# Veason-silverbullet/DIGAT

Hardware: AMD Instinct MI355X
Metric: MIND dev impressions scored/sec (AUC match not run) (higher is better)
Workload: dtype f32; 1 GPU; MIND-small default: --graph_encoder=DIGAT neighbors=3 hops=2 (N=10, U=67), d=400, graph_depth=3, fp32 dev inference; projection=auto -> fp16x3, N=10, U=67, d=400, graph_depth=3, news_num=65238, parallelism=dp1 (row shards, no data-path collective), ranks_in_process_group=1

## Files before the change

digat_amd/_lib.py:

```python
from __future__ import annotations

import ctypes as C
import os
from typing import Optional

import torch

_HERE = os.path.dirname(os.path.abspath(__file__))
LIB_PATH = os.environ.get("DIGAT_HIP_LIB") or os.path.join(_HERE, "lib", "libdigat_hip.so")
DIGAT_MAX_DEPTH = 16
DIGAT_MAX_NODES = 128
GEMM_BF16X6, GEMM_F16X3 = 0, 1
GEMM_F16F8C = 2
PARAMS_GEMM_F16X3 = 64
PARAMS_BD_TILED = 128
PARAMS_PQ_FP8 = 256
PARAMS_SIDE_STREAM_OFF, PARAMS_SIDE_STREAM_ON = 512, 1024
PARAMS_NO_LIVE_ROWS = 2048
PARAMS_PROJ_F16F8C = 4096

_f = C.c_void_p


class LayerParams(C.Structure):
    _fields_ = [(k, _f) for k in ("W", "bW", "F1", "F2", "F3", "b3", "a", "wsplit", "f3_wsplit")]


class MsaParams(C.Structure):
    _fields_ = ([(k, C.c_int32) for k in ("word_embedding_dim", "head_num", "head_dim", "attention_dim")]
                + [(k, C.c_void_p) for k in ("word_embedding", "W_Q", "b_Q", "W_K", "W_V", "b_V", "A1", "b1", "a2",
                                             "qkv_wsplit", "a1_wsplit")])


class CnnParams(C.Structure):
    _fields_ = ([(k, C.c_int32) for k in ("word_embedding_dim", "kernel_num", "taps", "attention_dim")]
                + [(k, C.c_void_p) for k in ("word_embedding", "W", "b", "A1", "b1", "a2", "w_split", "a1_wsplit")])


class SplitJob(C.Structure):
    _fields_ = [("w0", C.c_void_p), ("w1", C.c_void_p), ("w2", C.c_void_p), ("rows", C.c_int32), ("cols", C.c_int32), ("layout", C.c_int32),
                ("reserved", C.c_int32), ("image", C.c_void_p)]


class GatherJob(C.Structure):
    _fields_ = [("src", C.c_void_p), ("dst", C.c_void_p), ("row_bytes", C.c_int64), ("rows", C.c_int64),
                ("idx", C.c_void_p), ("idx2", C.c_void_p), ("inner", C.c_int64)]


class Params(C.Structure):
    _fields_ = ([("d", C.c_int32), ("depth", C.c_int32), ("category_num", C.c_int32), ("flags", C.c_int32)]
                + [(k, _f) for k in ("topic_node_embedding", "cand_K", "cand_Q", "cand_bQ",
                                     "news_graph_W", "news_graph_b", "user_news_K", "user_news_Q",
                                     "user_news_bQ", "featureAffine_W", "featureAffine_b",
                                     "userAtt_K", "userAtt_Q", "userAtt_bQ")]
                + [("news", LayerParams * DIGAT_MAX_DEPTH), ("user", LayerParams * DIGAT_MAX_DEPTH)]
                + [(k, _f) for k in ("cand_fold_W", "cand_fold_b", "user_news_fold_W", "user_news_fold_b",
                                     "userAtt_fold_W", "userAtt_fold_b", "featureAffine_wsplit", "cand_fold_wsplit", "gate_wsplit")]
                + [("ctx_wsplit", _f * (DIGAT_MAX_DEPTH + 1)), ("range_flag", _f), ("featureAffine_fsplit", _f)])


class DigatHipError(RuntimeError):
    pass


_lib: Optional[C.CDLL] = None

_SIGNATURES = {
    "digat_version": (C.c_int, []),
    "digat_error_string": (C.c_char_p, [C.c_int]),
    "digat_linear_f32": (C.c_int, [_f, C.c_int64, _f, _f, _f, C.c_int64, C.c_int, C.c_int, C.c_int, _f]),
    "digat_xattn_workspace_bytes": (C.c_size_t, [C.c_int] * 3),
    "digat_xattn_fwd": (C.c_int, [_f] * 12 + [C.c_int] * 3 + [_f, C.c_size_t, _f]),
    "digat_xattn_fwd_mode": (C.c_int, [_f] * 11 + [C.c_int] * 4 + [_f, C.c_size_t, _f]),
    "digat_xattn_fwd_lowprec": (C.c_int, [_f] * 11 + [C.c_int, _f] + [C.c_int] * 4 + [_f, C.c_size_t, _f]),
    "digat_xattn_pairwise_fwd": (C.c_int, [_f] * 8 + [C.c_int] * 3 + [_f]),
    "digat_news_ctx_workspace_bytes": (C.c_size_t, [C.c_int] * 3),
    "digat_news_ctx_fwd": (C.c_int, [_f] * 9 + [C.c_int] * 3 + [_f, C.c_size_t, _f]),
    "digat_user_ctx_workspace_bytes": (C.c_size_t, [C.c_int] * 5),
    "digat_user_ctx_fwd": (C.c_int, [_f] * 14 + [C.c_int] * 5 + [_f, C.c_size_t, _f]),
    "digat_topic_pool_fwd": (C.c_int, [_f] * 4 + [C.c_int] * 5 + [_f]),
    "digat_encoder_workspace_bytes": (C.c_size_t, [C.c_int] * 6),
    "digat_encoder_fwd": (C.c_int, [C.POINTER(Params)] + [_f] * 10 + [C.c_int] * 3 + [_f, C.c_size_t, _f]),
    "digat_row_logits": (C.c_int, [_f] * 3 + [C.c_int] * 2 + [_f]),
    "digat_profile_pause": (C.c_int, [C.c_int]),
    "digat_set_train_precision": (C.c_int, [C.c_int]),
    "digat_gather_tables": (C.c_int, [C.POINTER(GatherJob), C.c_int, _f]),
    "digat_profile_live_row_fraction": (C.c_double, []),
    "digat_rank_metrics": (C.c_int, [_f] * 3 + [C.c_int] + [_f] * 4),
    "digat_format_rank_file": (C.c_int64, [_f, _f, C.c_int64, _f, C.c_int64]),
    "digat_gat_workspace_bytes": (C.c_size_t, [C.c_int] * 3),
    "digat_gat_fwd": (C.c_int, [_f] * 7 + [C.c_int] * 3 + [_f, C.c_size_t, _f]),
    "digat_gat_train_save_bytes": (C.c_size_t, [C.c_int] * 3),
    "digat_gat_train_workspace_bytes": (C.c_size_t, [C.c_int] * 3),
    "digat_gat_fwd_train": (C.c_int, [_f] * 7 + [C.c_float, C.c_uint32] + [C.c_int] * 3 + [_f, C.c_size_t, _f, C.c_size_t, _f]),
    "digat_gat_bwd": (C.c_int, [_f] * 7 + [C.c_float, _f, C.c_size_t] + [_f] * 5 + [C.c_int] * 3 + [_f, C.c_size_t, _f]),
    "digat_sag_cos_topk_workspace_bytes": (C.c_size_t, [C.c_int64, C.c_int64, C.c_int]),
    "digat_sag_cos_topk": (C.c_int, [_f, _f, C.c_int64, _f, _f, C.c_int64, C.c_int, C.c_int, _f, _f, _f, C.c_size_t, _f]),
    "digat_sag_news_graph": (C.c_int, [_f, _f, _f, C.c_int64, C.c_int, C.c_int, C.c_int, C.c_float] + [_f] * 5),
    "digat_msa_split_bytes": (C.c_size_t, [C.c_int] * 3),
    "digat_split_msa_weights": (C.c_int, [_f] * 3 + [C.c_int] * 2 + [_f, _f]),
    "digat_msa_workspace_bytes": (C.c_size_t, [C.c_int] * 6),
    "digat_msa_fwd": (C.c_int, [C.POINTER(MsaParams), _f, _f, _f, C.c_int, C.c_int, _f, C.c_size_t, _f]),
    "digat_msa_train_save_bytes": (C.c_size_t, [C.c_int] * 6),
    "digat_msa_train_workspace_bytes": (C.c_size_t, [C.c_int] * 6),
    "digat_msa_fwd_train": (C.c_int, [C.POINTER(MsaParams), _f, _f, _f, C.c_float, C.c_uint32, C.c_int, C.c_int, _f, C.c_size_t, _f,
                                      C.c_size_t, _f]),
    "digat_msa_bwd": (C.c_int, [C.POINTER(MsaParams), _f, _f, _f, C.c_float, _f, C.c_size_t, _f, C.c_int64] + [_f] * 8
                      + [C.c_int, C.c_int, _f, C.c_size_t, _f]),
    "digat_msa_row_grad_ld": (C.c_int64, [C.c_int] * 3),
    "digat_cnn_split_bytes": (C.c_size_t, [C.c_int] * 3),
    "digat_split_cnn_weights": (C.c_int, [_f] + [C.c_int] * 3 + [_f, _f]),
    "digat_cnn_merge_group3": (C.c_int, [_f] * 6 + [C.c_int] * 2 + [_f] * 3),
    "digat_cnn_workspace_bytes": (C.c_size_t, [C.c_int] * 6),
    "digat_cnn_fwd": (C.c_int, [C.POINTER(CnnParams), _f, _f, _f, C.c_int, C.c_int, _f, C.c_size_t, _f]),
    "digat_cnn_train_save_bytes": (C.c_size_t, [C.c_int] * 6),
    "digat_cnn_train_workspace_bytes": (C.c_size_t, [C.c_int] * 6),
    "digat_cnn_fwd_train": (C.c_int, [C.POINTER(CnnParams), _f, _f, _f, C.c_float, C.c_uint32, C.c_int, C.c_int, _f, C.c_size_t, _f,
                                      C.c_size_t, _f]),
    "digat_cnn_bwd": (C.c_int, [C.POINTER(CnnParams), _f, _f, _f, C.c_float, C.c_uint32, _f, C.c_size_t, _f, C.c_int64] + [_f] * 5
                      + [C.c_int, C.c_int, _f, C.c_size_t, _f]),
    "digat_embedding_bwd_workspace_bytes": (C.c_size_t, [C.c_int64, C.c_int]),
    "digat_embedding_bwd": (C.c_int, [_f, C.c_int64, _f, _f, C.c_int64, C.c_int, _f, _f, C.c_size_t, _f]),
    "digat_embedding_bwd_unsorted_workspace_bytes": (C.c_size_t, [C.c_int64, C.c_int, C.c_int64]),
    "digat_embedding_bwd_unsorted": (C.c_int, [_f, _f, C.c_int64, C.c_int64, _f, _f, C.c_int64, C.c_int64, C.c_int, C.c_int64, _f, _f, C.c_size_t,
                                               _f]),
    "digat_encoder_grouped_workspace_bytes": (C.c_size_t, [C.c_int] * 6),
    "digat_encoder_fwd_grouped": (C.c_int, [C.POINTER(Params)] + [_f] * 11 + [C.c_int] * 4 + [_f, C.c_size_t, _f]),
    "digat_encoder_fwd_grouped_cached": (C.c_int, [C.POINTER(Params)] + [_f] * 14 + [C.c_int64] + [_f] * 2 + [C.c_int] * 4 + [_f, C.c_size_t, _f]),
    "digat_news_context_queries": (C.c_int, [C.POINTER(Params), _f, _f, C.c_int, _f]),
    "digat_user_project0": (C.c_int, [C.POINTER(Params), _f, _f, C.c_int, _f]),
    "digat_news_project0": (C.c_int, [C.POINTER(Params), _f, _f, C.c_int, C.c_int, _f]),
    "digat_split_weights_bytes": (C.c_size_t, [C.c_int, C.c_int]),
    "digat_split_weights_bytes_format": (C.c_size_t, [C.c_int, C.c_int, C.c_int]),
    "digat_forget_split_image": (C.c_int, [_f]),
    "digat_split_proj_weights": (C.c_int, [_f, _f, _f, C.c_int, _f, C.c_int, _f]),
    "digat_split_weights": (C.c_int, [_f, C.c_int, C.c_int, _f, C.c_int, _f]),
    "digat_linear_f32x3": (C.c_int, [_f, C.c_int64, _f, _f, _f, C.c_int64, C.c_int, C.c_int, C.c_int, _f, C.c_int, _f]),
    "digat_fold_workspace_bytes": (C.c_size_t, [C.c_int]),
    "digat_fold_attention": (C.c_int, [_f] * 5 + [C.c_int, _f, C.c_size_t, _f]),
    "digat_linear_bwd_input": (C.c_int, [_f, C.c_int64, _f, _f, C.c_int64, C.c_int, C.c_int, C.c_int, C.c_int, _f]),
    "digat_linear_bwd_input_x3": (C.c_int, [_f, C.c_int64, _f, _f, C.c_int64, C.c_int, C.c_int, C.c_int, C.c_int, _f, _f]),
    "digat_linear_bwd_weight_workspace": (C.c_size_t, [C.c_int] * 3),
    "digat_linear_bwd_weight": (C.c_int, [_f, C.c_int64, _f, C.c_int64, _f, _f, C.c_int, C.c_int, C.c_int, C.c_int, _f,
                                          C.c_size_t, _f]),
    "digat_colsum": (C.c_int, [_f, C.c_int64, _f, C.c_int, C.c_int, C.c_int, _f]),
    "digat_dropout_fwd": (C.c_int, [_f, _f, _f, C.c_int64, C.c_float, C.c_uint32, _f]),
    "digat_dropout_bwd": (C.c_int, [_f, _f, _f, C.c_int64, C.c_float, _f]),
    "digat_gate_fwd": (C.c_int, [_f, _f, C.c_int64, _f, _f, C.c_int, C.c_int, _f]),
    "digat_gate_bwd": (C.c_int, [_f, _f, _f, C.c_int64, _f, _f, _f, _f, C.c_int, C.c_int, _f]),
    "digat_relu_res_fwd": (C.c_int, [_f, _f, _f, C.c_int64, _f]),
    "digat_relu_mask": (C.c_int, [_f, _f, _f, C.c_int64, _f]),
    "digat_attn_pool_fwd": (C.c_int, [_f, C.c_int64, _f, _f, _f, _f, C.c_int, C.c_int, C.c_int, _f]),
    "digat_attn_pool_bwd": (C.c_int, [_f, C.c_int64, _f, _f, _f, _f, _f, C.c_int64, _f, C.c_int, C.c_int, C.c_int,
                                      C.c_int, _f]),
    "digat_topic_pool_fwd_train": (C.c_int, [_f] * 5 + [C.c_int] * 5 + [_f]),
    "digat_topic_pool_bwd": (C.c_int, [_f] * 7 + [C.c_int] * 5 + [_f]),
    "digat_xattn_project": (C.c_int, [_f] * 9 + [C.c_int] * 3 + [_f]),
    "digat_xattn_project_x3": (C.c_int, [_f] * 9 + [C.c_int] * 3 + [_f, _f]),
    "digat_xattn_pairwise_fwd_train": (C.c_int, [_f] * 11 + [C.c_float, C.c_uint32, C.c_int, C.c_int, C.c_int, _f]),
    "digat_xattn_pairwise_bwd_workspace": (C.c_size_t, [C.c_int] * 3),
    "digat_xattn_pairwise_bwd": (C.c_int, [_f] * 11 + [C.c_float] + [_f] * 4 + [C.c_int] * 4 + [_f, C.c_size_t, _f]),
    "digat_sum_nodes": (C.c_int, [_f, _f, C.c_int, C.c_int, C.c_int, _f]),
    "digat_xattn_train_save_bytes": (C.c_size_t, [C.c_int] * 3),
    "digat_xattn_train_workspace_bytes": (C.c_size_t, [C.c_int] * 3),
    "digat_xattn_fwd_train": (C.c_int, [_f] * 11 + [C.c_float, C.c_uint32, C.c_float, C.c_uint32] + [C.c_int] * 3 + [_f, C.c_size_t, _f, C.c_size_t, _f, C.c_int,
                                        _f]),
    "digat_xattn_bwd": (C.c_int, [_f] * 10 + [C.c_float, C.c_float, _f, C.c_size_t] + [_f] * 9 + [C.c_int] * 3 + [_f, C.c_size_t, _f, C.c_int, _f]),
    "digat_opt_chunk": (C.c_int, []),
    "digat_clip_adam_step": (C.c_int, [_f, _f, _f, C.c_int, _f] + [C.c_float] * 5 + [C.c_int, _f]),
    "digat_row_logits_bwd": (C.c_int, [_f] * 5 + [C.c_int, C.c_int, _f]),
    "digat_click_loss": (C.c_int, [_f, C.c_int, C.c_int, _f, _f, _f]),
    "digat_split_job_bytes": (C.c_size_t, [C.c_int] * 4),
# ... 150 lines not shown
```

digat_amd/csrc/digat_context.inc:

```

struct PoolArgs {
    const float* feat; long ld_b;
    const float* kq; const uint8_t* mask; const float* addend; float* out;
    int B, n, d; float sqrt_d;
    float* alpha_out;
    long ld_out;
    float* node0; long ld_node0;
};

__global__ void __launch_bounds__(256) attn_pool_kernel(const PoolArgs g) {
    __shared__ float sc[DIGAT_MAX_NODES];
    const int b = blockIdx.x, tid = threadIdx.x, lane = tid & 63, wave = tid >> 6;
    const int d4 = g.d >> 2, n = g.n;
    const float4* F4 = reinterpret_cast<const float4*>(g.feat + (long)b * g.ld_b);
    const float4* K4 = reinterpret_cast<const float4*>(g.kq + (long)b * g.d);
    for (int j = wave; j < n; j += 4) {
        float part = 0.f;
        for (int c4 = lane; c4 < d4; c4 += 64) {
            const float4 x = F4[(long)j * d4 + c4], k = K4[c4];
            part = fmaf(x.w, k.w, fmaf(x.z, k.z, fmaf(x.y, k.y, fmaf(x.x, k.x, part))));
        }
        part = wave_sum(part);
        if (lane == 0) sc[j] = g.mask[(long)b * n + j] == 0 ? -1e9f : part / g.sqrt_d;
    }
    __syncthreads();
    if (wave == 0) {
        const float v0 = lane < n ? sc[lane] : -INFINITY;
        const float v1 = lane + 64 < n ? sc[lane + 64] : -INFINITY;
        const float m = wave_max(fmaxf(v0, v1));
        const float e0 = lane < n ? expf(v0 - m) : 0.f;
        const float e1 = lane + 64 < n ? expf(v1 - m) : 0.f;
        const float s = wave_sum(e0 + e1);
        if (lane < n) sc[lane] = e0 / s;
        if (lane + 64 < n) sc[lane + 64] = e1 / s;
        if (g.alpha_out) {
            if (lane < n) g.alpha_out[(long)b * n + lane] = e0 / s;
            if (lane + 64 < n) g.alpha_out[(long)b * n + lane + 64] = e1 / s;
        }
    }
    __syncthreads();
    for (int c4 = tid; c4 < d4; c4 += 256) {
        float4 o = f4_zero();
        for (int j = 0; j < n; ++j) {
            const float al = sc[j];
            if (al == 0.f) continue;
            const float4 x = F4[(long)j * d4 + c4];
            o.x = fmaf(al, x.x, o.x); o.y = fmaf(al, x.y, o.y); o.z = fmaf(al, x.z, o.z); o.w = fmaf(al, x.w, o.w);
        }
        if (g.addend) o = f4_add(reinterpret_cast<const float4*>(g.addend + (long)b * g.d)[c4], o);
        reinterpret_cast<float4*>(g.out + (long)b * (g.ld_out ? g.ld_out : (long)g.d))[c4] = o;
        if (g.node0) reinterpret_cast<float4*>(g.node0 + (long)b * g.ld_node0)[c4] = F4[c4];
    }
}

template <int NPW, int U>
__global__ void __launch_bounds__(256) attn_pool_resident_kernel(const PoolArgs g) {
    __shared__ float sc[DIGAT_MAX_NODES];
    __shared__ float4 part[4][64 * U];
    const int b = blockIdx.x, tid = threadIdx.x, lane = tid & 63, wave = tid >> 6;
    const int d4 = g.d >> 2, n = g.n;
    const float4* F4 = reinterpret_cast<const float4*>(g.feat + (long)b * g.ld_b);
    const float4* K4 = reinterpret_cast<const float4*>(g.kq + (long)b * g.d);
    float4 x[NPW][U], k[U];
#pragma unroll
    for (int u = 0; u < U; ++u) {
        const int c4 = min(lane + 64 * u, d4 - 1);
        const float4 kv = K4[c4];
        k[u] = lane + 64 * u < d4 ? kv : f4_zero();
    }
    const unsigned long long mb0 = __ballot(lane < n && g.mask[(long)b * n + min(lane, n - 1)] != 0);
    const unsigned long long mb1 = __ballot(lane + 64 < n && g.mask[(long)b * n + min(lane + 64, n - 1)] != 0);
    const bool none = (mb0 | mb1) == 0ull;
#pragma unroll
    for (int t = 0; t < NPW; ++t) {
        const int j = min(wave + 4 * t, n - 1);
        const bool want = none || (((j < 64 ? mb0 : mb1) >> (j & 63)) & 1ull);
#pragma unroll
        for (int u = 0; u < U; ++u) x[t][u] = want ? F4[(long)j * d4 + min(lane + 64 * u, d4 - 1)] : f4_zero();
    }
#pragma unroll
    for (int t = 0; t < NPW; ++t) {
        const int j = wave + 4 * t;
        float p = 0.f;
#pragma unroll
        for (int u = 0; u < U; ++u) p = fmaf(x[t][u].w, k[u].w, fmaf(x[t][u].z, k[u].z, fmaf(x[t][u].y, k[u].y, fmaf(x[t][u].x, k[u].x, p))));
        p = wave_sum(p);
        if (lane == 0 && j < n) sc[j] = g.mask[(long)b * n + j] == 0 ? -1e9f : p / g.sqrt_d;
    }
    __syncthreads();
    {
        const float v0 = lane < n ? sc[lane] : -INFINITY;
        const float v1 = lane + 64 < n ? sc[lane + 64] : -INFINITY;
        const float m = wave_max(fmaxf(v0, v1));
        const float e0 = lane < n ? expf(v0 - m) : 0.f;
        const float e1 = lane + 64 < n ? expf(v1 - m) : 0.f;
        const float s = wave_sum(e0 + e1);
        const float a0 = e0 / s, a1 = e1 / s;
        if (wave == 0 && g.alpha_out) {
            if (lane < n) g.alpha_out[(long)b * n + lane] = a0;
            if (lane + 64 < n) g.alpha_out[(long)b * n + lane + 64] = a1;
        }
        float4 o[U];
#pragma unroll
        for (int u = 0; u < U; ++u) o[u] = f4_zero();
#pragma unroll
        for (int t = 0; t < NPW; ++t) {
            const int j = wave + 4 * t;
            const float al = j < n ? (j < 64 ? lane_bcast(a0, j & 63) : lane_bcast(a1, j & 63)) : 0.f;
            if (al != 0.f) {
#pragma unroll
                for (int u = 0; u < U; ++u) {
                    o[u].x = fmaf(al, x[t][u].x, o[u].x); o[u].y = fmaf(al, x[t][u].y, o[u].y);
                    o[u].z = fmaf(al, x[t][u].z, o[u].z); o[u].w = fmaf(al, x[t][u].w, o[u].w);
                }
            }
        }
#pragma unroll
        for (int u = 0; u < U; ++u) part[wave][lane + 64 * u] = o[u];
    }
    __syncthreads();
    for (int c4 = tid; c4 < d4; c4 += 256) {
        float4 o = f4_add(f4_add(part[0][c4], part[1][c4]), f4_add(part[2][c4], part[3][c4]));
        if (g.addend) o = f4_add(reinterpret_cast<const float4*>(g.addend + (long)b * g.d)[c4], o);
        reinterpret_cast<float4*>(g.out + (long)b * g.d)[c4] = o;
    }
}

static int launch_pool(const float* feat, long ld_b, const float* kq, const uint8_t* mask, const float* addend,
                       float* out, int B, int n, int d, hipStream_t st) {
    if (n > DIGAT_MAX_NODES || d % 4) return DIGAT_ERR_SHAPE;
    if (B == 0) return DIGAT_OK;
    PoolArgs g{feat, ld_b, kq, mask, addend, out, B, n, d, sqrtf((float)d), nullptr};
    ProfScope prof(DIGAT_KERNEL_POOL, (double)B * ((double)n * d * 4 + 2.0 * d * 4 + n), st);
    const int d4 = d / 4;
    if (d4 <= 128 && n <= 68) {
        if (d4 <= 64) {
            if (n <= 12) hipLaunchKernelGGL((attn_pool_resident_kernel<3, 1>), dim3(B), dim3(256), 0, st, g);
            else if (n <= 20) hipLaunchKernelGGL((attn_pool_resident_kernel<5, 1>), dim3(B), dim3(256), 0, st, g);
            else if (n <= 28) hipLaunchKernelGGL((attn_pool_resident_kernel<7, 1>), dim3(B), dim3(256), 0, st, g);
            else hipLaunchKernelGGL((attn_pool_resident_kernel<17, 1>), dim3(B), dim3(256), 0, st, g);
        } else {
            if (n <= 12) hipLaunchKernelGGL((attn_pool_resident_kernel<3, 2>), dim3(B), dim3(256), 0, st, g);
            else if (n <= 20) hipLaunchKernelGGL((attn_pool_resident_kernel<5, 2>), dim3(B), dim3(256), 0, st, g);
            else if (n <= 28) hipLaunchKernelGGL((attn_pool_resident_kernel<7, 2>), dim3(B), dim3(256), 0, st, g);
            else hipLaunchKernelGGL((attn_pool_resident_kernel<17, 2>), dim3(B), dim3(256), 0, st, g);
        }
        DIGAT_CHECK_LAUNCH();
        return DIGAT_OK;
    }
    hipLaunchKernelGGL(attn_pool_kernel, dim3(B), dim3(256), 0, st, g);
    DIGAT_CHECK_LAUNCH();
    return DIGAT_OK;
}

struct TopicArgs {
    const float* Xu; long ld_b; const float* kq; const int64_t* idx; float* out;
    int B, H, C1, d; float sqrt_d;
    float* alpha_out;
    const int* group;
    const uint8_t* live; int live_ld;
    const int* hlast;
};
constexpr int TOPIC_MAX_H = 256;
constexpr int TOPIC_MAX_CT = 4;

__global__ void __launch_bounds__(1024) topic_pool_kernel(const TopicArgs g) {
    extern __shared__ __attribute__((aligned(16))) unsigned char smem[];
    const int H = g.H, hs = H | 1;
    const int ct = (g.C1 + 15) >> 4;
    float* M = reinterpret_cast<float*>(smem);
    float* sa = M + ct * 16 * hs;
    int* sidx = reinterpret_cast<int*>(sa + H);
    const int b = blockIdx.x, tid = threadIdx.x, lane = tid & 63, wave = tid >> 6;
    const int nthreads = blockDim.x, nw = nthreads >> 6;
    const int d4 = g.d >> 2;
    const float* Xb = g.Xu + (long)(g.group ? g.group[b] : b) * g.ld_b;
    const float4* F4 = reinterpret_cast<const float4*>(Xb);
    const float4* K4 = reinterpret_cast<const float4*>(g.kq + (long)b * g.d);
    unsigned char* slive = reinterpret_cast<unsigned char*>(sidx + H);
    for (int t = tid; t < H; t += nthreads) {
        const long v = g.idx[(long)b * H + t];
        sidx[t] = (v >= 0 && v < g.C1) ? (int)v : -1;
        slive[t] = g.live ? g.live[(long)b * g.live_ld + t] : 1;
    }
    for (int i = tid; i < ct * 16 * hs; i += nthreads) M[i] = 0.f;
    __syncthreads();
    for (int t0 = wave; t0 < H; t0 += 4 * nw) {
        float part[4] = {0.f, 0.f, 0.f, 0.f};
        for (int c4 = lane; c4 < d4; c4 += 64) {
            const float4 k = K4[c4];
#pragma unroll
            for (int r = 0; r < 4; ++r) {
                const int t = t0 + r * nw;
                if (t < H && slive[t]) {
                    const float4 x = F4[(long)t * d4 + c4];
                    part[r] = fmaf(x.w, k.w, fmaf(x.z, k.z, fmaf(x.y, k.y, fmaf(x.x, k.x, part[r]))));
                }
            }
        }
#pragma unroll
        for (int r = 0; r < 4; ++r) {
            const int t = t0 + r * nw;
            const float s = wave_sum(part[r]);
            if (lane == 0 && t < H) sa[t] = s / g.sqrt_d;
        }
    }
    __syncthreads();
    for (int t = tid; t < H; t += nthreads) {
        const int s = sidx[t];
        float m = -INFINITY;
        for (int u = 0; u < H; ++u) if (sidx[u] == s) m = fmaxf(m, sa[u]);
        float den = 0.f;
        for (int u = 0; u < H; ++u) if (sidx[u] == s) den += expf(sa[u] - m);
        const float al = s >= 0 ? expf(sa[t] - m) / den : 0.f;
        if (s >= 0) M[s * hs + t] = al;
        if (g.alpha_out) g.alpha_out[(long)b * H + t] = al;
    }
    __syncthreads();

    const int lr = lane & 15, lq = lane >> 4;
    const int ch = wave * 64 + 4 * lr;
    const bool ch_ok = ch < g.d;
    const int nsteps = (H + 3) >> 2;
    auto load_x = [&](int step) -> float4 {
        const int j = step * 4 + lq;
        return (j < H && ch_ok && slive[j]) ? *reinterpret_cast<const float4*>(Xb + (long)j * g.d + ch) : f4_zero();
    };
    constexpr int PF = 4;
    v4f acc[TOPIC_MAX_CT][4];
#pragma unroll
    for (int it = 0; it < TOPIC_MAX_CT; ++it)
#pragma unroll
        for (int s = 0; s < 4; ++s) acc[it][s] = (v4f){0.f, 0.f, 0.f, 0.f};
    float4 xq[PF];
#pragma unroll
    for (int u = 0; u < PF; ++u) xq[u] = load_x(u);
    for (int step = 0; step < nsteps; step += PF) {
#pragma unroll
        for (int u = 0; u < PF; ++u) {
            const int st = step + u;
            if (st < nsteps) {
                const float4 xc = xq[u];
                xq[u] = load_x(st + PF);
                const int j = st * 4 + lq;
#pragma unroll
                for (int it = 0; it < TOPIC_MAX_CT; ++it) {
                    if (it < ct) {
                        const float av = j < H ? M[(it * 16 + lr) * hs + j] : 0.f;
                        acc[it][0] = __builtin_amdgcn_mfma_f32_16x16x4f32(av, xc.x, acc[it][0], 0, 0, 0);
                        acc[it][1] = __builtin_amdgcn_mfma_f32_16x16x4f32(av, xc.y, acc[it][1], 0, 0, 0);
                        acc[it][2] = __builtin_amdgcn_mfma_f32_16x16x4f32(av, xc.z, acc[it][2], 0, 0, 0);
                        acc[it][3] = __builtin_amdgcn_mfma_f32_16x16x4f32(av, xc.w, acc[it][3], 0, 0, 0);
                    }
                }
            }
        }
    }
    float* Ob = g.out + (long)b * g.C1 * g.d;
#pragma unroll
    for (int it = 0; it < TOPIC_MAX_CT; ++it) {
        if (it < ct) {
#pragma unroll
            for (int r = 0; r < 4; ++r) {
                const int c = it * 16 + 4 * lq + r;
                if (c < g.C1 && ch_ok)
                    *reinterpret_cast<float4*>(Ob + (long)c * g.d + ch) =
                        make_float4(acc[it][0][r], acc[it][1][r], acc[it][2][r], acc[it][3][r]);
            }
        }
    }
}


template <int TOPIC_RES_STEPS>
__global__ void __launch_bounds__(TOPIC_RES_STEPS > 13 ? 512 : 1024) topic_pool_resident_kernel(const TopicArgs g) {
    extern __shared__ __attribute__((aligned(16))) unsigned char smem[];
    const int H = g.H, hs = H | 1;
    const int ct = (g.C1 + 15) >> 4;
    const int tid = threadIdx.x, lane = tid & 63, wave = tid >> 6;
    const int nthreads = blockDim.x, nw = nthreads >> 6;
    float* M = reinterpret_cast<float*>(smem);
    float* part = M + ct * 16 * hs;
    float* sa = part + nw * 64;
    int* sidx = reinterpret_cast<int*>(sa + 64);
    int* slive = sidx + 64;
    int* cslot = slive + 64;
    int* scat = cslot + 64;
    const int b = blockIdx.x;
    const float* Xb = g.Xu + (long)(g.group ? g.group[b] : b) * g.ld_b;
    const int lr = lane & 15, lq = lane >> 4;
    const int ch = wave * 64 + 4 * lr;
    const bool ch_ok = ch < g.d;
    const int nsteps = (H + 3) >> 2;
    const int nl = (g.live && g.hlast) ? min(g.hlast[b], H) : H;

    float4 xq[TOPIC_RES_STEPS];
#pragma unroll
    for (int s = 0; s < TOPIC_RES_STEPS; ++s) {
        const int j = s * 4 + lq;
        const int jr = min(j, nl > 0 ? nl - 1 : 0);
        xq[s] = (s < nsteps && j < H && ch_ok) ? *reinterpret_cast<const float4*>(Xb + (long)jr * g.d + ch) : f4_zero();
    }
    const float4 k4 = ch_ok ? *reinterpret_cast<const float4*>(g.kq + (long)b * g.d + ch) : f4_zero();
    if (tid < 64) {
        long v = -1;
        if (tid < H) v = g.idx[(long)b * H + tid];
        const int cat = (v >= 0 && v < g.C1) ? (int)v : -1;
        sidx[tid] = cat;
        slive[tid] = (g.live && tid < H) ? (int)g.live[(long)b * g.live_ld + tid] : 1;
        unsigned long long present = 0ull;
        for (int c = 0; c < g.C1; ++c) present |= __ballot(cat == c) ? (1ull << c) : 0ull;
        const bool has = tid < g.C1 && ((present >> tid) & 1ull);
        const int slot = __popcll(present & ((1ull << tid) - 1ull));
        cslot[tid] = has ? slot : -1;
        if (has) scat[slot] = tid;
        if (tid == 0) scat[64] = __popcll(present);
    }
    for (int i = tid; i < ct * 16 * hs; i += nthreads) M[i] = 0.f;
    if (g.live) {
        __syncthreads();
#pragma unroll
        for (int s = 0; s < TOPIC_RES_STEPS; ++s) xq[s] = slive[min(s * 4 + lq, 63)] ? xq[s] : f4_zero();
    }

#pragma unroll
    for (int s = 0; s < TOPIC_RES_STEPS; ++s) {
        float p = fmaf(xq[s].w, k4.w, fmaf(xq[s].z, k4.z, fmaf(xq[s].y, k4.y, xq[s].x * k4.x)));
        p += dpp_mov<0xB1>(p); p += dpp_mov<0x4E>(p); p += dpp_mov<0x141>(p); p += dpp_mov<0x140>(p);
        if (lr == 0) part[wave * 64 + s * 4 + lq] = p;
    }
    __syncthreads();
    if (tid < 64) {
        float a = 0.f;
        for (int w = 0; w < nw; ++w) a += part[w * 64 + tid];
        sa[tid] = a / g.sqrt_d;
    }
    __syncthreads();
    {
        const int my = lane < H ? sidx[lane] : -2;
        const float v = lane < H ? sa[lane] : 0.f;
        const int nslots = scat[64];
        for (int sl = wave; sl < nslots; sl += nw) {
            const int c = scat[sl];
            const bool in = my == c;
            const float m = wave_max(in ? v : -INFINITY);
            const float e = in ? expf(v - m) : 0.f;
            const float den = wave_sum(e);
            if (in) {
                const float al = e / den;
                M[sl * hs + lane] = al;
                if (g.alpha_out) g.alpha_out[(long)b * H + lane] = al;
            }
        }
        if (wave == 0 && g.alpha_out && lane < H && my < 0) g.alpha_out[(long)b * H + lane] = 0.f;
    }
    __syncthreads();

    const int ct_eff = __builtin_amdgcn_readfirstlane((scat[64] + 15) >> 4);
    const int nslots_all = scat[64];
    float* Ob = g.out + (long)b * g.C1 * g.d;
    for (int it = 0; it < ct_eff; ++it) {
        v4f acc[4];
#pragma unroll
        for (int s = 0; s < 4; ++s) acc[s] = (v4f){0.f, 0.f, 0.f, 0.f};
#pragma unroll
        for (int s = 0; s < TOPIC_RES_STEPS; ++s) {
            if (s * 4 < nl) {
                const int j = s * 4 + lq;
                const float4 xc = xq[s];
                const float av = j < H ? M[(it * 16 + lr) * hs + j] : 0.f;
                acc[0] = __builtin_amdgcn_mfma_f32_16x16x4f32(av, xc.x, acc[0], 0, 0, 0);
                acc[1] = __builtin_amdgcn_mfma_f32_16x16x4f32(av, xc.y, acc[1], 0, 0, 0);
                acc[2] = __builtin_amdgcn_mfma_f32_16x16x4f32(av, xc.z, acc[2], 0, 0, 0);
                acc[3] = __builtin_amdgcn_mfma_f32_16x16x4f32(av, xc.w, acc[3], 0, 0, 0);
            }
        }
#pragma unroll
        for (int r = 0; r < 4; ++r) {
            const int sl = it * 16 + 4 * lq + r;
            if (sl < nslots_all && ch_ok)
                *reinterpret_cast<float4*>(Ob + (long)scat[sl] * g.d + ch) = make_float4(acc[0][r], acc[1][r], acc[2][r], acc[3][r]);
        }
    }
    for (int c = lq; c < g.C1; c += 4)
        if (cslot[c] < 0 && ch_ok) *reinterpret_cast<float4*>(Ob + (long)c * g.d + ch) = f4_zero();
}

static int launch_topic_args(TopicArgs g, hipStream_t st) {
    const int groups = (g.d + 63) / 64;
    const int ct = (g.C1 + 15) / 16;
    if (g.H > TOPIC_MAX_H || g.d % 4 || groups > 16 || ct > TOPIC_MAX_CT) return DIGAT_ERR_SHAPE;
    const size_t lds = ((size_t)ct * 16 * (g.H | 1) + 2 * (size_t)g.H) * 4 + align_up((size_t)g.H, 16);
    if (lds > 64 * 1024) {
        static int raised = 0;
        if (!raised) {
            if (hipFuncSetAttribute((const void*)topic_pool_kernel, hipFuncAttributeMaxDynamicSharedMemorySize,
                                    160 * 1024) != hipSuccess) return DIGAT_ERR_LAUNCH;
            raised = 1;
        }
    }
    if (g.H <= 64 && (g.H <= 52 || groups <= 8)) {
        const size_t ldsr = ((size_t)ct * 16 * (g.H | 1) + (size_t)groups * 64 + 192 + 64 + 68) * 4;
        if (g.H <= 52) hipLaunchKernelGGL(topic_pool_resident_kernel<13>, dim3(g.B), dim3(64 * groups), ldsr, st, g);
        else hipLaunchKernelGGL(topic_pool_resident_kernel<16>, dim3(g.B), dim3(64 * groups), ldsr, st, g);
    } else {
        hipLaunchKernelGGL(topic_pool_kernel, dim3(g.B), dim3(64 * groups), lds, st, g);
    }
    DIGAT_CHECK_LAUNCH();
    return DIGAT_OK;
}

static int launch_topic(const float* Xu, long ld_b, const float* kq, const int64_t* idx, float* out,
                        int B, int H, int C1, int d, hipStream_t st, const int* group = nullptr,
                        const uint8_t* live = nullptr, int live_ld = 0, const int* hlast = nullptr) {
    if (B == 0) return DIGAT_OK;
    TopicArgs g{Xu, ld_b, kq, idx, out, B, H, C1, d, sqrtf((float)d), nullptr, group, live, live_ld, hlast};
    ProfScope prof(DIGAT_KERNEL_TOPIC, (double)B * ((double)H * d * 4 + d * 4.0 + H * 8.0 + (double)C1 * d * 4), st);
    return launch_topic_args(g, st);
}
```

digat_amd/csrc/digat_gemm.inc:

```

#include "digat_gemm_plan.h"

template <int BM, int BN, int WAVES_M, int WAVES_N, int PF, int TAG>
__global__ void __launch_bounds__(256) gemm_f32_kernel(const GemmArgs g) {
    constexpr int BK4 = 8;
    constexpr int MT = BM / WAVES_M / 16;
    constexpr int NT = BN / WAVES_N / 16;
    static_assert(WAVES_M * WAVES_N == 4, "4 waves per workgroup");
    static_assert(BM % (WAVES_M * 16) == 0 && BN % (WAVES_N * 16) == 0, "wave tile");
    static_assert(BM % 8 == 0 && BN % 8 == 0, "xor swizzle needs 8-row groups");
    constexpr int A_PER_T = (BM * BK4 + 255) / 256;
    constexpr int B_PER_T = (BN * BK4 + 255) / 256;
    __shared__ float4 As[BK4 * BM];
    __shared__ float4 Bs[BK4 * BN];

    const int total = g.mtiles * g.ntiles;
    const int chunk = (total + 7) >> 3;
    const int tile = (int)(blockIdx.x & 7) * chunk + (int)(blockIdx.x >> 3);
    if (tile >= total) return;
    const int mtile = tile / g.ntiles, ntile = tile - mtile * g.ntiles;

    const int tid = threadIdx.x, lane = tid & 63, wave = tid >> 6;
    const int wm = wave / WAVES_N, wn = wave % WAVES_N;
    const int m0 = mtile * BM, n0 = ntile * BN;
// ... 43 lines not shown
        }
    };
    auto store_tiles = [&](const float4* ra, const float4* rb) {
#pragma unroll
        for (int u = 0; u < A_PER_T; ++u) {
            const int i = tid + u * 256;
            if (i < BM * BK4) {
                const int r = i / BK4, c4 = i % BK4;
                As[c4 * BM + (r ^ c4)] = ra[u];
            }
        }
#pragma unroll
        for (int u = 0; u < B_PER_T; ++u) {
            const int i = tid + u * 256;
            if (i < BN * BK4) {
                const int r = g.transW ? i % BN : i / BK4;
                const int c4 = g.transW ? i / BN : i % BK4;
                Bs[c4 * BN + (r ^ c4)] = rb[u];
            }
        }
    };

    v4f acc[MT][NT];
#pragma unroll
    for (int mt = 0; mt < MT; ++mt)
#pragma unroll
        for (int nt = 0; nt < NT; ++nt) acc[mt][nt] = (v4f){0.f, 0.f, 0.f, 0.f};

    auto compute_tile = [&]() {
#pragma unroll
        for (int kk = 0; kk < 2; ++kk) {
            const int k4 = kk * 4 + (lane >> 4);
            float4 af[MT], bf[NT];
#pragma unroll
            for (int mt = 0; mt < MT; ++mt) {
                const int r = wm * (MT * 16) + mt * 16 + (lane & 15);
                af[mt] = As[k4 * BM + (r ^ k4)];
            }
#pragma unroll
            for (int nt = 0; nt < NT; ++nt) {
                const int r = wn * (NT * 16) + nt * 16 + (lane & 15);
                bf[nt] = Bs[k4 * BN + (r ^ k4)];
            }
#pragma unroll
            for (int s = 0; s < 4; ++s)
#pragma unroll
                for (int mt = 0; mt < MT; ++mt)
#pragma unroll
                    for (int nt = 0; nt < NT; ++nt)
                        acc[mt][nt] = __builtin_amdgcn_mfma_f32_16x16x4f32(
                            f4_comp(af[mt], s), f4_comp(bf[nt], s), acc[mt][nt], 0, 0, 0);
        }
    };

    if (PF == 1) {
        load_tiles(0, ra0, rb0);
        store_tiles(ra0, rb0);
        __syncthreads();
        for (int kt = 0; kt < ktiles; ++kt) {
            const bool more = kt + 1 < ktiles;
            if (more) load_tiles(kt + 1, ra0, rb0);
            compute_tile();
            __syncthreads();
            if (more) {
                store_tiles(ra0, rb0);
                __syncthreads();
            }
        }
    } else {
        load_tiles(0, ra0, rb0);
        if (ktiles > 1) load_tiles(1, ra1, rb1);
        store_tiles(ra0, rb0);
        __syncthreads();
        for (int kt = 0; kt < ktiles; kt += 2) {
            if (kt + 2 < ktiles) load_tiles(kt + 2, ra0, rb0);
            compute_tile();
            __syncthreads();
            if (kt + 1 >= ktiles) break;
            store_tiles(ra1, rb1);
            __syncthreads();
            if (kt + 3 < ktiles) load_tiles(kt + 3, ra1, rb1);
            compute_tile();
            __syncthreads();
            if (kt + 2 < ktiles) {
                store_tiles(ra0, rb0);
                __syncthreads();
            }
        }
    }

#pragma unroll
    for (int mt = 0; mt < MT; ++mt) {
#pragma unroll
        for (int nt = 0; nt < NT; ++nt) {
            const int nn = nbase + wn * (NT * 16) + nt * 16 + (lane & 15);
            if (nn >= g.nseg) continue;
            const float* bp = g.bias[seg];
            float* yp = g.y[seg];
            const float bv = bp ? bp[nn] : 0.f;
            const float* radd = seg == g.radd_seg ? g.radd : nullptr;
#pragma unroll
            for (int r = 0; r < 4; ++r) {
                const int gm = m0 + wm * (MT * 16) + mt * 16 + (lane >> 4) * 4 + r;
                if (gm >= g.M) continue;
                float v = acc[mt][nt][r] + bv;
                if (radd) v = radd[(long)(gm / g.rows_per_b) * g.nseg + nn] + v;
                if (g.epi == EPI_RELU_RES) {
                    v = fmaxf(v, 0.f) + g.e0[(long)gm * g.lde0 + nn];
                } else if (g.epi == EPI_GATE) {
                    const float gate = 1.f / (1.f + expf(-v));
                    const float loc = g.e0[(long)gm * g.lde0 + nn];
                    const float glo = g.e1[(long)gm * g.lde1 + nn];
                    v = gate * loc + (1.f - gate) * glo;
                    if (g.e2) v = g.e2[(long)gm * g.lde2 + nn] + v;
                } else if (g.epi == EPI_ACCUM) {
                    v = yp[(long)gm * g.ldy + nn] + v;
                }
                yp[(long)gm * g.ldy + nn] = v;
            }
        }
    }
}

typedef __bf16 bf16x8 __attribute__((ext_vector_type(8)));

struct Split3f { float a, b, c; };
__device__ __forceinline__ Split3f split3f(float v) {
    Split3f o;
    o.a = __builtin_bit_cast(float, __builtin_bit_cast(unsigned, v) & 0xffff0000u);
    const float r1 = v - o.a;
    o.b = __builtin_bit_cast(float, __builtin_bit_cast(unsigned, r1) & 0xffff0000u);
    o.c = r1 - o.b;
    return o;
}
__device__ __forceinline__ unsigned pack_bf16_rne(float lo, float hi) {
    unsigned a = __builtin_bit_cast(unsigned, lo), b = __builtin_bit_cast(unsigned, hi);
    a += 0x7fffu + ((a >> 16) & 1u);
    b += 0x7fffu + ((b >> 16) & 1u);
    return (a >> 16) | (b & 0xffff0000u);
}
__device__ __forceinline__ unsigned pack_hi16(float lo, float hi) {
    return __builtin_amdgcn_perm(__builtin_bit_cast(unsigned, hi), __builtin_bit_cast(unsigned, lo), 0x07060302u);
}
constexpr float F16_WEIGHT_SCALE = 1024.f;
constexpr float F16_ACT_SCALE = 16.f;
typedef _Float16 half8 __attribute__((ext_vector_type(8)));
typedef __fp16 fp16x2 __attribute__((ext_vector_type(2)));
__device__ __forceinline__ unsigned pack_half_rtz(float lo, float hi) { return __builtin_bit_cast(unsigned, __builtin_amdgcn_cvt_pkrtz(lo, hi)); }
__device__ __forceinline__ unsigned half_bits_rtz(float v) { return pack_half_rtz(v, 0.f) & 0xffffu; }
__device__ __forceinline__ float half_bits_to_float(unsigned bits) {
    const fp16x2 h = __builtin_bit_cast(fp16x2, bits);
    return (float)h[0];
}
struct Split3 { unsigned short a, b, c; };
__device__ __forceinline__ Split3 split3(float v) {
    const Split3f f = split3f(v);
    Split3 o;
    o.a = (unsigned short)(__builtin_bit_cast(unsigned, f.a) >> 16);
    o.b = (unsigned short)(__builtin_bit_cast(unsigned, f.b) >> 16);
    o.c = (unsigned short)(__builtin_bit_cast(unsigned, f.c) >> 16);
    return o;
}

constexpr int WS_SLOTS = 960;

__device__ __forceinline__ void split_weights_tiled_body(const float* w0, const float* w1, const float* w2,
                                                         int nseg, int nsegs, int K, unsigned short* out, int transposed, int planes) {
    const int KT = (K + 31) >> 5, Kp = KT * 32;
    const int Ntot = nseg * nsegs;
    const int strips = (Ntot + 79) / 80;
    const long total = (long)strips * 80 * Kp;
    for (long i = (long)blockIdx.x * 256 + threadIdx.x; i < total; i += (long)gridDim.x * 256) {
        const int n = (int)(i / Kp), k = (int)(i - (long)n * Kp);
        float v = 0.f;
        if (n < Ntot && k < K) {
            const int seg = n / nseg;
            const float* w = seg == 0 ? w0 : (seg == 1 ? w1 : w2);
            if (transposed == 2) {
                const int kseg = K / 3, ks = k / kseg;
                const float* wk = ks == 0 ? w0 : (ks == 1 ? w1 : w2);
                v = wk[(long)(k - ks * kseg) * nseg + n];
            } else
            v = transposed ? w[(long)k * nseg + n] : w[(long)(n - seg * nseg) * K + k];
        }
        const int strip = n / 80, r = n - strip * 80, kt = k >> 5, kq = (k >> 3) & 3, e = k & 7;
        const long base = ((long)strip * KT + kt) * (planes * 320) * 8;
        if (planes == 3) {
            const Split3 sp = split3(v);
            out[base + ((0 * 4 + kq) * 80 + r) * 8 + e] = sp.a;
            out[base + ((1 * 4 + kq) * 80 + r) * 8 + e] = sp.b;
            out[base + ((2 * 4 + kq) * 80 + r) * 8 + e] = sp.c;
        } else {
            const float vs = v * F16_WEIGHT_SCALE;
            const _Float16 h = (_Float16)vs;
            const _Float16 l = (_Float16)(vs - (float)h);
            const unsigned hi = __builtin_bit_cast(unsigned short, h), lo = __builtin_bit_cast(unsigned short, l);
            out[base + ((0 * 4 + kq) * 80 + r) * 8 + e] = (unsigned short)hi;
            out[base + ((1 * 4 + kq) * 80 + r) * 8 + e] = (unsigned short)lo;
        }
    }
}
__global__ void __launch_bounds__(256) split_weights_tiled_kernel(const float* w0, const float* w1, const float* w2,
                                                                  int nseg, int nsegs, int K, unsigned short* out, int transposed, int planes) {
    split_weights_tiled_body(w0, w1, w2, nseg, nsegs, K, out, transposed, planes);
}
constexpr int SPLIT_MAX_JOBS = 24;
struct SplitJobDev { const float *w0, *w1, *w2; unsigned short* out; int nseg, nsegs, K, transposed; };
struct SplitJobsDev { SplitJobDev j[SPLIT_MAX_JOBS]; };
__device__ __forceinline__ void split_weights_slots_body(const float* w0, const float* w1, const float* w2, int nseg, int nsegs, int K,
                                                         unsigned short* out, int transposed) {
    const int KT = (K + 31) >> 5;
    const int Ntot = nseg * nsegs;
    const int strips = (Ntot + 79) / 80;
    const int k8s = KT * 4;
    const long total = (long)strips * 80 * k8s;
    for (long i = (long)blockIdx.x * 256 + threadIdx.x; i < total; i += (long)gridDim.x * 256) {
        const int n = transposed ? (int)(i % (strips * 80)) : (int)(i / k8s);
        const int k8 = transposed ? (int)(i / (strips * 80)) : (int)(i - (long)n * k8s);
        const int k0 = k8 * 8;
        float v[8];
#pragma unroll
        for (int e = 0; e < 8; ++e) v[e] = 0.f;
        if (n < Ntot) {
            if (!transposed) {
                const int seg = n / nseg;
                const float* row = (seg == 0 ? w0 : (seg == 1 ? w1 : w2)) + (long)(n - seg * nseg) * K;
                if (k0 + 8 <= K && ((uintptr_t)(row + k0) & 15) == 0) {
                    const float4 a = *reinterpret_cast<const float4*>(row + k0), b = *reinterpret_cast<const float4*>(row + k0 + 4);
                    v[0] = a.x; v[1] = a.y; v[2] = a.z; v[3] = a.w; v[4] = b.x; v[5] = b.y; v[6] = b.z; v[7] = b.w;
                } else {
#pragma unroll
                    for (int e = 0; e < 8; ++e) if (k0 + e < K) v[e] = row[k0 + e];
                }
            } else if (transposed == 2) {
                const int kseg = K / 3;
#pragma unroll
                for (int e = 0; e < 8; ++e) {
                    const int k = k0 + e;
                    if (k < K) {
                        const int ks = k / kseg;
                        v[e] = (ks == 0 ? w0 : (ks == 1 ? w1 : w2))[(long)(k - ks * kseg) * nseg + n];
                    }
                }
            } else {
#pragma unroll
                for (int e = 0; e < 8; ++e) if (k0 + e < K) v[e] = w0[(long)(k0 + e) * nseg + n];
            }
        }
        const int strip = n / 80, r = n - strip * 80, kt = k8 >> 2, kq = k8 & 3;
        const long base = ((long)strip * KT + kt) * (3 * 320) * 8;
        unsigned pa[4], pb[4], pc[4];
#pragma unroll
        for (int h = 0; h < 4; ++h) {
            const Split3 s0 = split3(v[2 * h]), s1 = split3(v[2 * h + 1]);
            pa[h] = (unsigned)s0.a | ((unsigned)s1.a << 16);
            pb[h] = (unsigned)s0.b | ((unsigned)s1.b << 16);
            pc[h] = (unsigned)s0.c | ((unsigned)s1.c << 16);
        }
        *reinterpret_cast<uint4*>(out + base + ((0 * 4 + kq) * 80 + r) * 8) = make_uint4(pa[0], pa[1], pa[2], pa[3]);
        *reinterpret_cast<uint4*>(out + base + ((1 * 4 + kq) * 80 + r) * 8) = make_uint4(pb[0], pb[1], pb[2], pb[3]);
        *reinterpret_cast<uint4*>(out + base + ((2 * 4 + kq) * 80 + r) * 8) = make_uint4(pc[0], pc[1], pc[2], pc[3]);
    }
}
__global__ void __launch_bounds__(256) split_weights_jobs_kernel(const SplitJobsDev a) {
    const SplitJobDev& j = a.j[blockIdx.y];
    split_weights_slots_body(j.w0, j.w1, j.w2, j.nseg, j.nsegs, j.K, j.out, j.transposed);
}

#ifdef DIGAT_GEMM_TIMERS
__device__ unsigned long long g_gemm_timers[8];
#define GT_NOW() __builtin_amdgcn_s_memtime()
#else
#define GT_NOW() 0ull
#endif
template <int NSUB, bool F16, int MT, bool FULL>
__global__ void __launch_bounds__(256, MT == 1 ? 3 : 2) gemm_bf16x6s_kernel(const GemmArgs g) {
    static_assert(MT == 1 || MT == 2, "wave tiles of 16 or 32 rows");
    constexpr int NT = 5;
    constexpr int WROWS = 16 * MT, TROWS = 4 * WROWS;
    constexpr int APW = 2 * MT;
    constexpr int RING = 3;
    constexpr int ABUF = NSUB == 1 ? 2 : 1;
    constexpr int PL = F16 ? 2 : 3;
    constexpr int WS_SLOTS = PL * 320;
    constexpr int PIECES = WS_SLOTS / 64;
    constexpr int IMG_I = (PIECES + 3) / 4;
    __shared__ uint4 Bs[RING][WS_SLOTS];
    __shared__ uint4 As[ABUF][TROWS * 8];

    const int Mv = g.nrows_dev ? __builtin_amdgcn_readfirstlane(*g.nrows_dev) : g.M;
    if (g.exec_rows && blockIdx.x == 0 && threadIdx.x == 0) atomicAdd(g.exec_rows, (unsigned long long)Mv);
    const int total = ((Mv + TROWS - 1) / TROWS) * g.ntiles;
    const int chunk = (total + 7) >> 3;
    if ((int)(blockIdx.x >> 3) >= chunk) return;
    const int tile = (int)(blockIdx.x & 7) * chunk + (int)(blockIdx.x >> 3);
    if (tile >= total) return;
    const int mtile = tile / g.ntiles, ntile = tile - mtile * g.ntiles;

    const int tid = threadIdx.x, lane = tid & 63, wm = tid >> 6;
    const int kg = lane >> 4, lr = lane & 15;
    const int m0 = mtile * TROWS;
    const int strip0 = ntile * NSUB;
#ifdef DIGAT_GEMM_TIMERS
    const unsigned long long gt_enter = GT_NOW();
    unsigned long long gt_wait = 0, gt_bar = 0, gt_body = 0, gt_steps = 0, gt_last = 0;
#endif
    const int KT = (g.K + 31) >> 5;
    const int nsteps = KT * NSUB;
    const unsigned ldsB = (unsigned)(uintptr_t)(__attribute__((address_space(3))) unsigned char*)&Bs[0][0];
    const unsigned ldsA = (unsigned)(uintptr_t)(__attribute__((address_space(3))) unsigned char*)&As[0][0];
    const char* const wimg = reinterpret_cast<const char*>(g.wsplit);
    const unsigned wlane = (unsigned)lane * 16u;
    const int wu = __builtin_amdgcn_readfirstlane(wm);

    auto issue_b = [&](int step) {
        const int kt = step / NSUB, s = step - kt * NSUB;
        const int buf = step % RING;
        const char* src = wimg + ((long)(strip0 + s) * KT + kt) * (WS_SLOTS * 16);
#pragma unroll
        for (int k = 0; k < IMG_I; ++k) {
            int q = wu + 4 * k;
            q = q < PIECES ? q : PIECES - 1;
            lds_dma16_s(src + q * 1024, wlane, ldsB + (unsigned)((buf * WS_SLOTS + q * 64) * 16));
        }
    };
    const long arow0 = g.rowidx ? 0 : (long)(m0 < Mv ? m0 : Mv - 1);
    const char* const abase = reinterpret_cast<const char*>(g.a0 + arow0 * g.lda0);
    unsigned aoff[APW];
    int ac4[APW];
#pragma unroll
    for (int k = 0; k < APW; ++k) {
        const int sl = (wm + 4 * k) * 64 + lane;
        const int r = sl >> 3, c4 = (sl & 7) ^ ((r >> 1) & 7);
        int gm = m0 + r;
        gm = gm < Mv ? gm : Mv - 1;
        if (g.rowidx) gm = g.rowidx[gm];
        aoff[k] = (unsigned)((((long)gm - arow0) * g.lda0 + c4 * 4) * 4);
        ac4[k] = c4 * 4;
    }
    auto issue_a_piece = [&](int kt, int abuf, int k) {
        unsigned vo = aoff[k];
        long sk = (long)kt * 128;
        if (kt * 32 + 32 > g.K) { vo += kt * 32 + ac4[k] < g.K ? (unsigned)kt * 128u : 0u; sk = 0; }
        lds_dma16_s(abase + sk, vo, ldsA + (unsigned)((abuf * (TROWS * 8) + (wu + 4 * k) * 64) * 16));
    };
    auto issue_a = [&](int kt, int abuf) {
#pragma unroll
        for (int k = 0; k < APW; ++k) issue_a_piece(kt, abuf, k);
    };
    auto split_half = [&](const float4& v, unsigned (&o)[3][2]) {
        const Split3f s0 = split3f(v.x), s1 = split3f(v.y), s2 = split3f(v.z), s3 = split3f(v.w);
        o[0][0] = pack_hi16(s0.a, s1.a); o[0][1] = pack_hi16(s2.a, s3.a);
        o[1][0] = pack_hi16(s0.b, s1.b); o[1][1] = pack_hi16(s2.b, s3.b);
        o[2][0] = pack_hi16(s0.c, s1.c); o[2][1] = pack_hi16(s2.c, s3.c);
    };
    float amax = 0.f;
    auto split_mt = [&](int mt, int abuf, bf16x8 (&dst)[3][MT]) {
        const int r = wm * WROWS + mt * 16 + lr;
        const int sw = (r >> 1) & 7;
        const float4 v0 = __builtin_bit_cast(float4, As[abuf][r * 8 + ((kg * 2) ^ sw)]);
        const float4 v1 = __builtin_bit_cast(float4, As[abuf][r * 8 + ((kg * 2 + 1) ^ sw)]);
        if constexpr (F16) {
            constexpr float xs = F16_ACT_SCALE;
            const float raw[8] = {v0.x, v0.y, v0.z, v0.w, v1.x, v1.y, v1.z, v1.w};
            const float v[8] = {v0.x * xs, v0.y * xs, v0.z * xs, v0.w * xs, v1.x * xs, v1.y * xs, v1.z * xs, v1.w * xs};
            amax = fmaxf(fmaxf(amax, fabsf(v[0])), fabsf(v[1])); amax = fmaxf(fmaxf(amax, fabsf(v[2])), fabsf(v[3]));
            amax = fmaxf(fmaxf(amax, fabsf(v[4])), fabsf(v[5])); amax = fmaxf(fmaxf(amax, fabsf(v[6])), fabsf(v[7]));
            unsigned hi[4], lo[4];
#pragma unroll
            for (int e = 0; e < 4; ++e) {
                hi[e] = pack_half_rtz(v[2 * e], v[2 * e + 1]);
                const fp16x2 h = __builtin_bit_cast(fp16x2, hi[e]);
                const _Float16 l0 = (_Float16)__builtin_fmaf(raw[2 * e], xs, -(float)h[0]), l1 = (_Float16)__builtin_fmaf(raw[2 * e + 1], xs, -(float)h[1]);
                lo[e] = (unsigned)__builtin_bit_cast(unsigned short, l0) | ((unsigned)__builtin_bit_cast(unsigned short, l1) << 16);
            }
            dst[0][mt] = __builtin_bit_cast(bf16x8, make_uint4(hi[0], hi[1], hi[2], hi[3]));
            dst[1][mt] = __builtin_bit_cast(bf16x8, make_uint4(lo[0], lo[1], lo[2], lo[3]));
        } else {
            unsigned lo[3][2], hi[3][2];
            split_half(v0, lo);
            split_half(v1, hi);
#pragma unroll
            for (int p = 0; p < 3; ++p) dst[p][mt] = __builtin_bit_cast(bf16x8, make_uint4(lo[p][0], lo[p][1], hi[p][0], hi[p][1]));
        }
    };
    auto mma = [&](const bf16x8 w, const bf16x8 a, const v4f c) -> v4f {
        if constexpr (F16) return __builtin_amdgcn_mfma_f32_16x16x32_f16(__builtin_bit_cast(half8, w), __builtin_bit_cast(half8, a), c, 0, 0, 0);
        else return __builtin_amdgcn_mfma_f32_16x16x32_bf16(w, a, c, 0, 0, 0);
    };

    int lite[NSUB];
#pragma unroll
    for (int s = 0; s < NSUB; ++s) {
        const int seg = ((strip0 + s) * 80) / g.nseg;
        lite[s] = FULL ? 0 : __builtin_amdgcn_readfirstlane(((g.x1_segs >> seg) & 1) ? 2 : ((g.x3_segs >> seg) & 1));
    }
    v4f acc[NSUB][MT][NT];
#pragma unroll
    for (int s = 0; s < NSUB; ++s)
#pragma unroll
        for (int mt = 0; mt < MT; ++mt)
#pragma unroll
            for (int nt = 0; nt < NT; ++nt) acc[s][mt][nt] = (v4f){0.f, 0.f, 0.f, 0.f};

    bf16x8 af[3][MT], afn[3][MT];
    if constexpr (NSUB == 1) {
#pragma unroll
        for (int j = 0; j < ABUF; ++j) if (j < KT) issue_a(j, j);
#pragma unroll
        for (int j = 0; j < RING - 1; ++j) if (j < nsteps) issue_b(j);
    } else {
        issue_a(0, 0);
        issue_b(0);
        if (nsteps > 1) issue_b(1);
    }
    asm volatile("s_waitcnt vmcnt(0)" ::: "memory");
    __builtin_amdgcn_s_barrier();
#pragma unroll
    for (int mt = 0; mt < MT; ++mt) split_mt(mt, 0, af);

    for (int kt = 0; kt < KT; ++kt) {
        const bool more = kt + 1 < KT;
#pragma unroll
        for (int s = 0; s < NSUB; ++s) {
            const int step = kt * NSUB + s;
            const int buf = step % RING;
#ifdef DIGAT_GEMM_TIMERS
            const unsigned long long gt0 = GT_NOW();
            if (step > 0) gt_body += gt0 - gt_last;
#endif
            if constexpr (NSUB == 1) {
                constexpr int L = (RING - 1 < ABUF - 1 ? RING - 1 : ABUF - 1) - 1;
                constexpr int KEEP = (APW + IMG_I) * (L < 0 ? 0 : L) + ((ABUF - 1 < RING - 1) ? IMG_I : 0);
                static_assert(KEEP <= 63, "vmcnt is six bits");
                if (kt + (RING - 1 > ABUF ? RING - 1 : ABUF) < KT) wait_vmcnt_imm<KEEP>();
                else asm volatile("s_waitcnt vmcnt(0)" ::: "memory");
            } else if (step + 1 < nsteps) {
                if constexpr (IMG_I == 4) asm volatile("s_waitcnt vmcnt(4)" ::: "memory");
                else asm volatile("s_waitcnt vmcnt(3)" ::: "memory");
            } else asm volatile("s_waitcnt vmcnt(0)" ::: "memory");
#ifdef DIGAT_GEMM_TIMERS
            const unsigned long long gt1 = GT_NOW();
#endif
            __builtin_amdgcn_s_barrier();
#ifdef DIGAT_GEMM_TIMERS
            gt_last = GT_NOW();
            gt_wait += gt1 - gt0; gt_bar += gt_last - gt1; ++gt_steps;
#endif
            if (NSUB == 1) {
                if (kt + ABUF < KT) issue_a(kt + ABUF, kt % ABUF);
                if (step + RING - 1 < nsteps) issue_b(step + RING - 1);
            } else {
                if (s == 0 && more) issue_a(kt + 1, 0);
                if (step + 2 < nsteps) issue_b(step + 2);
            }
            const uint4* Bi = Bs[buf];
            const int lslot = kg * 80 + lr;
            bf16x8 bq[2][3];
#pragma unroll
            for (int p = 0; p < PL; ++p) bq[0][p] = __builtin_bit_cast(bf16x8, Bi[p * 320 + lslot]);
#pragma unroll
            for (int nt = 0; nt < NT; ++nt) {
                if (nt + 1 < NT) {
#pragma unroll
                    for (int p = 0; p < PL; ++p) bq[(nt + 1) & 1][p] = __builtin_bit_cast(bf16x8, Bi[p * 320 + lslot + (nt + 1) * 16]);
                }
                const bf16x8 b1 = bq[nt & 1][0], b2 = bq[nt & 1][1], b3 = bq[nt & 1][PL - 1];
                v4f c[MT];
#pragma unroll
                for (int mt = 0; mt < MT; ++mt) c[mt] = acc[s][mt][nt];
                if (!F16 && (FULL || !lite[s])) {
#pragma unroll
                    for (int mt = 0; mt < MT; ++mt) c[mt] = mma(b1, af[2][mt], c[mt]);
#pragma unroll
                    for (int mt = 0; mt < MT; ++mt) c[mt] = mma(b2, af[1][mt], c[mt]);
#pragma unroll
                    for (int mt = 0; mt < MT; ++mt) c[mt] = mma(b3, af[0][mt], c[mt]);
                }
                if (FULL || lite[s] < 2) {
#pragma unroll
                    for (int mt = 0; mt < MT; ++mt) c[mt] = mma(b1, af[1][mt], c[mt]);
#pragma unroll
                    for (int mt = 0; mt < MT; ++mt) c[mt] = mma(b2, af[0][mt], c[mt]);
                }
#pragma unroll
                for (int mt = 0; mt < MT; ++mt) c[mt] = mma(b1, af[0][mt], c[mt]);
#pragma unroll
                for (int mt = 0; mt < MT; ++mt) acc[s][mt][nt] = c[mt];
                if (NSUB > 1) {
                    if (s == 1 && nt == 0) split_mt(0, 0, afn);
                    if constexpr (MT > 1) { if (s == 1 && nt == 2) split_mt(1, 0, afn); }
                } else {
                    if (nt == 0) split_mt(0, (kt + 1) % ABUF, afn);
                    if constexpr (MT > 1) { if (nt == 2) split_mt(1, (kt + 1) % ABUF, afn); }
                }
            }
            if (NSUB == 1 || s == 1) {
#pragma unroll
                for (int i = 0; i < 56; ++i) {
                    __builtin_amdgcn_sched_group_barrier(0x008, 1, 0);
                    __builtin_amdgcn_sched_group_barrier(0x002, 2, 0);
                }
            }
        }
        if (more) {
#pragma unroll
            for (int p = 0; p < 3; ++p)
#pragma unroll
                for (int mt = 0; mt < MT; ++mt) af[p][mt] = afn[p][mt];
        }
    }

#ifdef DIGAT_GEMM_TIMERS
    const unsigned long long gt_loop_end = GT_NOW();
    gt_body += gt_loop_end - gt_last;
#endif
    if constexpr (F16) {
        if (g.range_flag && __builtin_amdgcn_ballot_w64(!(amax < 65504.f)) != 0 && lane == 0) atomicOr(g.range_flag, 1u);
    }
    int gmv[MT];
    bool rok[MT];
    {
        const int* const ri = (g.rowidx && !g.gather_only) ? g.rowidx : nullptr;
#pragma unroll
        for (int mt = 0; mt < MT; ++mt) {
            const int gv = m0 + wm * WROWS + mt * 16 + lr;
            rok[mt] = gv < Mv;
            const int gvc = rok[mt] ? gv : Mv - 1;
            gmv[mt] = ri ? ri[gvc] : gvc;
        }
    }
    const bool has_e0 = g.epi == EPI_RELU_RES || g.epi == EPI_ADD_E0;
#pragma unroll
    for (int s = 0; s < NSUB; ++s) {
        const int ncol0 = (strip0 + s) * 80;
        const int seg = ncol0 / g.nseg;
        const int nbase = ncol0 - seg * g.nseg + kg * 4;
        const float* const bp = g.bias[seg];
        const bool radd_here = g.radd && seg == g.radd_seg;
        const bool y16 = (g.bf16_segs >> seg) & 1;
        const bool y8 = (g.fp8_segs >> seg) & 1;
        float4 bv[NT];
        if (bp) {
#pragma unroll
            for (int nt = 0; nt < NT; ++nt) bv[nt] = *reinterpret_cast<const float4*>(bp + nbase + nt * 16);
        }
#pragma unroll
        for (int mt = 0; mt < MT; ++mt) {
            const int gm = gmv[mt];
            float* const yrow = g.y[seg] + (long)gm * g.ldy;
            float4 rv[NT], ev[NT];
            if (radd_here) {
                const float* rrow = g.radd + (long)(gm / g.rows_per_b) * g.nseg + nbase;
#pragma unroll
                for (int nt = 0; nt < NT; ++nt) rv[nt] = *reinterpret_cast<const float4*>(rrow + nt * 16);
            }
            if (y8) {
                float4 vv[NT];
                float amx = 0.f;
#pragma unroll
                for (int nt = 0; nt < NT; ++nt) {
                    const v4f a = acc[s][mt][nt];
                    float4 v = make_float4(a[0], a[1], a[2], a[3]);
                    if constexpr (F16) {
                        constexpr float u = 1.f / (F16_WEIGHT_SCALE * F16_ACT_SCALE);
                        v = make_float4(v.x * u, v.y * u, v.z * u, v.w * u);
                    }
                    if (bp) v = f4_add(v, bv[nt]);
                    if (radd_here) v = f4_add(rv[nt], v);
                    vv[nt] = v;
                    amx = fmaxf(fmaxf(amx, fmaxf(fabsf(v.x), fabsf(v.y))), fmaxf(fabsf(v.z), fabsf(v.w)));
                }
                amx = fmaxf(amx, __shfl_xor(amx, 16, 64));
                amx = fmaxf(amx, __shfl_xor(amx, 32, 64));
                const float scale = amx > 0.f ? amx * (1.f / 448.f) : 1.f;
                const float inv = 1.f / scale;
                unsigned char* const row8 = reinterpret_cast<unsigned char*>(g.y[seg]) + (long)gm * g.ldy8;
                if (rok[mt]) {
#pragma unroll
                    for (int nt = 0; nt < NT; ++nt) {
                        int w = 0;
                        w = __builtin_amdgcn_cvt_pk_fp8_f32(vv[nt].x * inv, vv[nt].y * inv, w, false);
                        w = __builtin_amdgcn_cvt_pk_fp8_f32(vv[nt].z * inv, vv[nt].w * inv, w, true);
                        *reinterpret_cast<int*>(row8 + nbase + nt * 16) = w;
                    }
                    if (kg == 0) *reinterpret_cast<float*>(row8 + g.nseg + 4 * ((ncol0 - seg * g.nseg) / 80)) = scale;
                }
                continue;
            }
            if (has_e0) {
                const float* erow = g.e0 + (long)gm * g.lde0 + nbase;
#pragma unroll
                for (int nt = 0; nt < NT; ++nt) ev[nt] = *reinterpret_cast<const float4*>(erow + nt * 16);
            } else if (g.epi == EPI_ACCUM) {
#pragma unroll
                for (int nt = 0; nt < NT; ++nt) ev[nt] = *reinterpret_cast<const float4*>(yrow + nbase + nt * 16);
            }
#pragma unroll
            for (int nt = 0; nt < NT; ++nt) {
                const int nn = nbase + nt * 16;
                const v4f a = acc[s][mt][nt];
                float4 v = make_float4(a[0], a[1], a[2], a[3]);
                if constexpr (F16) {
                    constexpr float u = 1.f / (F16_WEIGHT_SCALE * F16_ACT_SCALE);
                    v = make_float4(v.x * u, v.y * u, v.z * u, v.w * u);
                }
                if (bp) v = f4_add(v, bv[nt]);
                if (radd_here) v = f4_add(rv[nt], v);
                if (y16) {
                    if (rok[mt])
                        *reinterpret_cast<uint2*>(reinterpret_cast<unsigned short*>(g.y[seg]) + (long)gm * g.ldy + nn) =
                            make_uint2(pack_bf16_rne(v.x, v.y), pack_bf16_rne(v.z, v.w));
                    continue;
                }
                if (g.epi == EPI_RELU_RES) {
                    const float4 x = ev[nt];
                    v = make_float4(fmaxf(v.x, 0.f) + x.x, fmaxf(v.y, 0.f) + x.y, fmaxf(v.z, 0.f) + x.z, fmaxf(v.w, 0.f) + x.w);
                }
                if (g.epi == EPI_ACCUM || g.epi == EPI_ADD_E0) v = f4_add(ev[nt], v);
                if constexpr (!F16) {
                    if (g.dmask && rok[mt] && (g.dmask_cols == 0 || nn < g.dmask_cols)) {
                        const unsigned mk = *reinterpret_cast<const unsigned*>(g.dmask + (long)gm * g.lddm + nn);
                        v = make_float4((mk & 0xffu) ? v.x * g.dscale : 0.f, (mk & 0xff00u) ? v.y * g.dscale : 0.f,
                                        (mk & 0xff0000u) ? v.z * g.dscale : 0.f, (mk & 0xff000000u) ? v.w * g.dscale : 0.f);
                    }
                }
                if (rok[mt]) *reinterpret_cast<float4*>(yrow + nn) = v;
            }
        }
    }
#ifdef DIGAT_GEMM_TIMERS
    if (lane == 0 && (blockIdx.x & 15) < 8) {
        const unsigned long long gt_end = GT_NOW();
        atomicAdd(&g_gemm_timers[0], gt_wait); atomicAdd(&g_gemm_timers[1], gt_bar); atomicAdd(&g_gemm_timers[2], gt_body);
        atomicAdd(&g_gemm_timers[3], gt_steps); atomicAdd(&g_gemm_timers[5], gt_end - gt_loop_end);
        atomicAdd(&g_gemm_timers[6], 1ull); atomicAdd(&g_gemm_timers[7], gt_end - gt_enter);
    }
#endif
}

template <int MT, bool KTAIL, bool TW = false>
__global__ void __launch_bounds__(256) gemm_skinny_kernel(const GemmArgs g) {
    __shared__ float red[4][MT * 20][64];
    const int tile = blockIdx.x;
    const int mtile = tile / g.ntiles, ntile = tile - mtile * g.ntiles;
    const int tid = threadIdx.x, lane = tid & 63, wave = tid >> 6;
    const int lr = lane & 15, lq = lane >> 4;
    const int m0 = mtile * (MT * 16), n0 = ntile * 80;
    const int seg = n0 / g.nseg;
    const int nbase = n0 - seg * g.nseg;
    const float* const wseg = g.w[seg];
    const int nkb = (g.K + 15) >> 4;

    const float* arow[MT][2];
    bool aok[MT];
#pragma unroll
    for (int mt = 0; mt < MT; ++mt) {
        const int gm = m0 + mt * 16 + lr;
        aok[mt] = gm < g.M;
        arow[mt][0] = g.a0 + (long)(aok[mt] ? gm : 0) * g.lda0;
        arow[mt][1] = g.a1 ? g.a1 + (long)(aok[mt] ? gm : 0) * g.lda1 : arow[mt][0];
    }
    const float* brow[5];
    bool bok[5];
#pragma unroll
    for (int nt = 0; nt < 5; ++nt) {
        const int nn = nbase + nt * 16 + lr;
        bok[nt] = nn < g.nseg;
        brow[nt] = TW ? wseg + (bok[nt] ? nn : 0) : wseg + (long)(bok[nt] ? nn : 0) * g.K;
    }
    auto load_block = [&](int kb, float4* a, float4* b) {
        const int k = kb * 16 + 4 * lq;
        const int kc = (KTAIL && k >= g.K) ? g.K - 4 : k;
        const float mk = (KTAIL && k >= g.K) ? 0.f : 1.f;
#pragma unroll
        for (int mt = 0; mt < MT; ++mt) {
            const float* p = kc < g.k0 ? arow[mt][0] + kc : arow[mt][1] + (kc - g.k0);
            const float4 v = *reinterpret_cast<const float4*>(p);
            a[mt] = KTAIL ? make_float4(v.x * mk, v.y * mk, v.z * mk, v.w * mk) : v;
        }
#pragma unroll
        for (int nt = 0; nt < 5; ++nt) {
            float4 v;
            if constexpr (TW) {
                const float* c = brow[nt] + (long)kc * g.nseg;
                v = make_float4(c[0], c[g.nseg], c[2 * (long)g.nseg], c[3 * (long)g.nseg]);
            } else {
                v = *reinterpret_cast<const float4*>(brow[nt] + kc);
            }
            b[nt] = KTAIL ? make_float4(v.x * mk, v.y * mk, v.z * mk, v.w * mk) : v;
        }
    };

    v4f acc[MT][5];
#pragma unroll
    for (int mt = 0; mt < MT; ++mt)
#pragma unroll
        for (int nt = 0; nt < 5; ++nt) acc[mt][nt] = (v4f){0.f, 0.f, 0.f, 0.f};

    auto blk = [&](int q) { return 8 * (q >> 1) + 2 * wave + (q & 1); };
    float4 a0[MT], b0[5], a1[MT], b1[5];
    int q = 0;
    if (blk(0) < nkb) load_block(blk(0), a0, b0);
    while (blk(q) < nkb) {
        if (blk(q + 1) < nkb) load_block(blk(q + 1), a1, b1);
#pragma unroll
        for (int s = 0; s < 4; ++s)
#pragma unroll
            for (int mt = 0; mt < MT; ++mt)
#pragma unroll
                for (int nt = 0; nt < 5; ++nt)
                    acc[mt][nt] = __builtin_amdgcn_mfma_f32_16x16x4f32(f4_comp(a0[mt], s), f4_comp(b0[nt], s), acc[mt][nt], 0, 0, 0);
        ++q;
        if (blk(q) >= nkb) break;
        if (blk(q + 1) < nkb) load_block(blk(q + 1), a0, b0);
#pragma unroll
        for (int s = 0; s < 4; ++s)
#pragma unroll
            for (int mt = 0; mt < MT; ++mt)
#pragma unroll
                for (int nt = 0; nt < 5; ++nt)
                    acc[mt][nt] = __builtin_amdgcn_mfma_f32_16x16x4f32(f4_comp(a1[mt], s), f4_comp(b1[nt], s), acc[mt][nt], 0, 0, 0);
        ++q;
    }
#pragma unroll
    for (int mt = 0; mt < MT; ++mt)
#pragma unroll
        for (int nt = 0; nt < 5; ++nt)
#pragma unroll
            for (int r = 0; r < 4; ++r) red[wave][(mt * 5 + nt) * 4 + r][lane] = acc[mt][nt][r];
    __syncthreads();
    const float* bp = g.bias[seg];
    float* yp = g.y[seg];
    for (int q = 0; q < MT * 5; ++q) {
        const int reg = wave * (MT * 5) + q;
        const int mt = reg / 20, nt = (reg / 4) % 5, r = reg & 3;
        const int gm = m0 + mt * 16 + lq * 4 + r;
        const int nn = nbase + nt * 16 + lr;
        if (gm >= g.M || nn >= g.nseg) continue;
        float v = ((red[0][reg][lane] + red[1][reg][lane]) + red[2][reg][lane]) + red[3][reg][lane];
        v += bp ? bp[nn] : 0.f;
        if (g.epi == EPI_RELU_RES) {
            v = fmaxf(v, 0.f) + g.e0[(long)gm * g.lde0 + nn];
        } else if (g.epi == EPI_GATE) {
            const float gate = 1.f / (1.f + expf(-v));
            const float loc = g.e0[(long)gm * g.lde0 + nn];
            const float glo = g.e1[(long)gm * g.lde1 + nn];
            v = gate * loc + (1.f - gate) * glo;
            if (g.e2) v = g.e2[(long)gm * g.lde2 + nn] + v;
        } else if (g.epi == EPI_ACCUM) {
            v = yp[(long)gm * g.ldy + nn] + v;
        }
        yp[(long)gm * g.ldy + nn] = v;
    }
}

template <int MT, bool F16>
__global__ void __launch_bounds__(256) gemm_skinny_split_kernel(const GemmArgs g) {
    constexpr int PL = F16 ? 2 : 3;
    constexpr int IMG_BYTES = PL * 320 * 16;
    __shared__ v4f red[4][MT * 5][64];
    const int tile = blockIdx.x;
    const int mtile = tile / g.ntiles, strip = tile - mtile * g.ntiles;
    const int tid = threadIdx.x, lane = tid & 63, wave = tid >> 6;
    const int kg = lane >> 4, lr = lane & 15;
    const int m0 = mtile * (MT * 16), n0 = strip * 80;
    const int seg = n0 / g.nseg;
    const int nbase = n0 - seg * g.nseg;
    const int KT = (g.K + 31) >> 5;
    const char* const wimg = reinterpret_cast<const char*>(g.wsplit) + (long)strip * KT * IMG_BYTES + (long)(kg * 80 + lr) * 16;

    const float* arow[MT][2];
#pragma unroll
    for (int mt = 0; mt < MT; ++mt) {
        const int gm = min(m0 + mt * 16 + lr, g.M - 1);
        arow[mt][0] = g.a0 + (long)gm * g.lda0;
        arow[mt][1] = g.a1 ? g.a1 + (long)gm * g.lda1 : arow[mt][0];
    }
    auto load_tile = [&](int kt, uint4 (&b)[PL][5], float4 (&a)[MT][2]) {
        const char* src = wimg + (long)kt * IMG_BYTES;
#pragma unroll
        for (int p = 0; p < PL; ++p)
#pragma unroll
            for (int nt = 0; nt < 5; ++nt) b[p][nt] = *reinterpret_cast<const uint4*>(src + (p * 320 + nt * 16) * 16);
        const int k = kt * 32 + kg * 8;
        const bool in = k < g.K;
#pragma unroll
        for (int mt = 0; mt < MT; ++mt) {
            const float* pa = !in ? arow[mt][0] : (k < g.k0 ? arow[mt][0] + k : arow[mt][1] + (k - g.k0));
            a[mt][0] = *reinterpret_cast<const float4*>(pa);
            a[mt][1] = *reinterpret_cast<const float4*>(pa + (in ? 4 : 0));
// ... 316 lines not shown
        xsc = ((w >> sh) & 0xff) | (((w >> (16 + sh)) & 0xff) << 8);
    };

    v4f acc[NSUB][NT];
#pragma unroll
    for (int s = 0; s < NSUB; ++s)
#pragma unroll
        for (int nt = 0; nt < NT; ++nt) acc[s][nt] = (v4f){0.f, 0.f, 0.f, 0.f};

    load_x(0);
    issue_b(0);
    for (int kt = 0; kt < KT; ++kt) {
        const int krel = g.K - kt * 128;
        const int nks = krel >= 32 ? 4 : (krel + 7) >> 3;
#pragma unroll
        for (int s = 0; s < NSUB; ++s) {
            const int step = kt * NSUB + s;
            asm volatile("s_waitcnt vmcnt(0)" ::: "memory");
            __builtin_amdgcn_s_barrier();
            if (s == 0) split_x();
            if (step + 1 < nsteps) issue_b(step + 1);
            if (s == NSUB - 1 && kt + 1 < KT) load_x(kt + 1);
            const uint4* Bi = Bs[step & 1];
            const int lslot = kg * 80 + lr;
            const uint2 sch = *reinterpret_cast<const uint2*>(reinterpret_cast<const unsigned char*>(Bi) + 40960 + ((0 * 4 + kg) * 16 + lr) * 8);
            const uint2 scl = *reinterpret_cast<const uint2*>(reinterpret_cast<const unsigned char*>(Bi) + 40960 + ((1 * 4 + kg) * 16 + lr) * 8);
#pragma unroll
            for (int nt = 0; nt < NT; ++nt) {
                const int sl = lslot + nt * 16;
                const uint4 q1a = Bi[1280 + sl], q1b = Bi[1280 + 320 + sl];
                const uint4 q2a = Bi[1920 + sl], q2b = Bi[1920 + 320 + sl];
                const v8i wq1 = (v8i){(int)q1a.x, (int)q1a.y, (int)q1a.z, (int)q1a.w, (int)q1b.x, (int)q1b.y, (int)q1b.z, (int)q1b.w};
                const v8i wq2 = (v8i){(int)q2a.x, (int)q2a.y, (int)q2a.z, (int)q2a.w, (int)q2b.x, (int)q2b.y, (int)q2b.z, (int)q2b.w};
                const int sh = (int)(nt < 4 ? sch.x : sch.y), sl8 = (int)(nt < 4 ? scl.x : scl.y);
                v4f c = acc[s][nt];
                c = f8c_mma<0>(nt & 3, wq2, xq1, c, sl8, xsc);
                c = f8c_mma<1>(nt & 3, wq1, xq2, c, sh, xsc);
#pragma unroll
                for (int ks = 0; ks < 4; ++ks) {
                    if (ks < nks) {
                        const bf16x8 wh = __builtin_bit_cast(bf16x8, Bi[ks * 320 + sl]);
                        c = __builtin_amdgcn_mfma_f32_16x16x32_f16(__builtin_bit_cast(half8, wh), __builtin_bit_cast(half8, xh[ks]), c, 0, 0, 0);
                    }
                }
                acc[s][nt] = c;
            }
        }
    }

    if (g.range_flag && __builtin_amdgcn_ballot_w64(!(amax < 65504.f)) != 0 && lane == 0) atomicOr(g.range_flag, 1u);
    const int gv = m0 + wm * 16 + lr;
    const bool rok = gv < Mv;
    const int gvc = rok ? gv : Mv - 1;
    const int gm = (g.rowidx && !g.gather_only) ? g.rowidx[gvc] : gvc;
    const bool has_e0 = g.epi == EPI_RELU_RES || g.epi == EPI_ADD_E0;
    constexpr float u = 1.f / (F16_WEIGHT_SCALE * F16_ACT_SCALE);
#pragma unroll
    for (int s = 0; s < NSUB; ++s) {
        const int ncol0 = (strip0 + s) * 80;
        const int seg = ncol0 / g.nseg;
        const int nbase = ncol0 - seg * g.nseg + kg * 4;
        const float* const bp = g.bias[seg];
        const bool radd_here = g.radd && seg == g.radd_seg;
        float* const yrow = g.y[seg] + (long)gm * g.ldy;
        float4 bv[NT], rv[NT], ev[NT];
        if (bp) {
#pragma unroll
            for (int nt = 0; nt < NT; ++nt) bv[nt] = *reinterpret_cast<const float4*>(bp + nbase + nt * 16);
        }
        if (radd_here) {
            const float* rrow = g.radd + (long)(gm / g.rows_per_b) * g.nseg + nbase;
#pragma unroll
            for (int nt = 0; nt < NT; ++nt) rv[nt] = *reinterpret_cast<const float4*>(rrow + nt * 16);
        }
        if (has_e0) {
            const float* erow = g.e0 + (long)gm * g.lde0 + nbase;
#pragma unroll
            for (int nt = 0; nt < NT; ++nt) ev[nt] = *reinterpret_cast<const float4*>(erow + nt * 16);
        } else if (g.epi == EPI_ACCUM) {
#pragma unroll
            for (int nt = 0; nt < NT; ++nt) ev[nt] = *reinterpret_cast<const float4*>(yrow + nbase + nt * 16);
        }
#pragma unroll
        for (int nt = 0; nt < NT; ++nt) {
            const v4f a = acc[s][nt];
            float4 v = make_float4(a[0] * u, a[1] * u, a[2] * u, a[3] * u);
            if (bp) v = f4_add(v, bv[nt]);
            if (radd_here) v = f4_add(rv[nt], v);
            if (g.epi == EPI_RELU_RES) {
                const float4 x = ev[nt];
                v = make_float4(fmaxf(v.x, 0.f) + x.x, fmaxf(v.y, 0.f) + x.y, fmaxf(v.z, 0.f) + x.z, fmaxf(v.w, 0.f) + x.w);
            }
            if (g.epi == EPI_ACCUM || g.epi == EPI_ADD_E0) v = f4_add(ev[nt], v);
            if (rok) *reinterpret_cast<float4*>(yrow + nbase + nt * 16) = v;
        }
    }
}

static std::mutex g_wsplit_mu;
static std::unordered_map<const void*, int> g_wsplit_format;
static void wsplit_note(const void* image, int format) {
    std::lock_guard<std::mutex> lock(g_wsplit_mu);
    g_wsplit_format[image] = format;
}
static int wsplit_forget(const void* image) {
    std::lock_guard<std::mutex> lock(g_wsplit_mu);
    return g_wsplit_format.erase(image) ? 1 : 0;
}
static int wsplit_format_of(const void* image) {
    std::lock_guard<std::mutex> lock(g_wsplit_mu);
    const auto it = g_wsplit_format.find(image);
    return it == g_wsplit_format.end() ? -1 : it->second;
}
static double gemm_row_bytes(const GemmArgs& g) {
    double out = 0.0;
    for (int sgm = 0; sgm < g.nsegs; ++sgm)
        out += ((g.fp8_segs >> sgm) & 1) ? (double)g.nseg + 4.0 * (g.nseg / 80) : (((g.bf16_segs >> sgm) & 1) ? 2.0 * g.nseg : 4.0 * g.nseg);
    double in = 4.0 * g.K;
    if (g.epi == EPI_RELU_RES || g.epi == EPI_ADD_E0 || g.epi == EPI_ACCUM) in += 4.0 * g.nseg;
    if (g.epi == EPI_GATE) in += 4.0 * g.nseg * (g.e2 ? 3 : 2);
    if (g.radd) in += 4.0 * g.nseg / (g.rows_per_b > 0 ? g.rows_per_b : 1);
    return in + out;
}

static int launch_gemm(GemmArgs g, hipStream_t st, int kind = DIGAT_KERNEL_LINEAR) {
    if (g.M <= 0) return DIGAT_OK;
    const GemmPlan p = gemm_plan(g, kind);
    if (p.status) return p.status;
    if (p.kernel == GEMM_PER_SEGMENT) {
        for (int sgm = 0; sgm < g.nsegs; ++sgm) {
            GemmArgs one = g;
            one.w[0] = g.w[sgm]; one.bias[0] = g.bias[sgm]; one.y[0] = g.y[sgm]; one.nsegs = 1;
            if (sgm == g.radd_seg) one.radd_seg = 0; else one.radd = nullptr;
            const int rc = launch_gemm(one, st, kind);
            if (rc) return rc;
        }
        return DIGAT_OK;
    }
    if (p.image_format >= 0) {
        const int made_as = wsplit_format_of(g.wsplit);
        if (made_as >= 0 && made_as != p.image_format) return DIGAT_ERR_ARG;
    }
    const int Ntot = g.nseg * g.nsegs;
    const bool listed = g.rowidx != nullptr && !g.gather_only;
    if (listed && g_prof.enabled) {
        g.exec_rows = g_prof.rows_dev + kind;
        g_prof.flops_per_row[kind] = 2.0 * (double)Ntot * g.K; g_prof.rows_nominal[kind] += g.M;
        g_prof.bytes_per_row[kind] = gemm_row_bytes(g);
    }
    ProfScope prof(kind, listed ? 0.0 : 2.0 * g.M * (double)Ntot * g.K, st, listed ? 0.0 : (double)g.M * gemm_row_bytes(g));
    g.mtiles = p.mtiles; g.ntiles = p.ntiles;
    switch (p.kernel) {
#define DIGAT_GEMM_LAUNCH(id, ...) case GEMM_##id: hipLaunchKernelGGL((__VA_ARGS__), dim3(p.grid), dim3(p.block), 0, st, g); break;
        DIGAT_GEMM_KERNELS(DIGAT_GEMM_LAUNCH)
#undef DIGAT_GEMM_LAUNCH
        default: return DIGAT_ERR_ARG;
    }
    DIGAT_CHECK_LAUNCH();
    return DIGAT_OK;
}

static GemmArgs gemm_plain(const float* x, long ldx, const float* w, const float* b, float* y, long ldy,
                           int M, int N, int K, int transW) {
    GemmArgs g;
    memset(&g, 0, sizeof(g));
    g.a0 = x; g.lda0 = ldx; g.k0 = K; g.a1 = nullptr; g.lda1 = 0;
    g.w[0] = w; g.bias[0] = b; g.y[0] = y; g.ldy = ldy;
    g.nseg = N; g.nsegs = 1; g.M = M; g.K = K; g.transW = transW; g.epi = EPI_NONE;
    return g;
}
```

digat_amd/csrc/digat_gemm_plan.h:

```cpp
#pragma once
#include <stdint.h>
#include "../../include/digat_hip.h"

enum { EPI_NONE = 0, EPI_RELU_RES = 1, EPI_GATE = 2, EPI_ACCUM = 3,
       EPI_ADD_E0 = 4 };

struct GemmArgs {
    const float* a0; long lda0; int k0;
    const float* a1; long lda1;
    const float* w[3]; const float* bias[3]; float* y[3]; long ldy;
    int nseg, nsegs, M, K, transW;
    int epi;
    const float* e0; long lde0; const float* e1; long lde1; const float* e2; long lde2;
    int mtiles, ntiles;
    const unsigned short* wsplit;
    const float* radd; int radd_seg, rows_per_b;
    unsigned long long* exec_rows;
    const int* rowidx; const int* nrows_dev;
    int gather_only;
    int m_dispatch;
    int x3_segs;
    int x1_segs;
    int bf16_segs;
    int fp8_segs; long ldy8;
    int format;
    unsigned* range_flag;
    const uint8_t* dmask; long lddm; float dscale;
    int dmask_cols;
};

#define DIGAT_GEMM_KERNELS(X)                                        \
    X(F16F8C_3, gemm_f16f8c_kernel<3>)                               \
    X(F16F8C_1, gemm_f16f8c_kernel<1>)                               \
    X(SKINNY_TW_2, gemm_skinny_kernel<2, false, true>)               \
    X(SKINNY_TW_1, gemm_skinny_kernel<1, false, true>)               \
    X(SKINNY_SPLIT_F16_2, gemm_skinny_split_kernel<2, true>)         \
    X(SKINNY_SPLIT_F16_1, gemm_skinny_split_kernel<1, true>)         \
    X(SKINNY_SPLIT_BF16_2, gemm_skinny_split_kernel<2, false>)       \
    X(SKINNY_SPLIT_BF16_1, gemm_skinny_split_kernel<1, false>)       \
    X(SKINNY_2_KTAIL, gemm_skinny_kernel<2, true, false>)            \
    X(SKINNY_2, gemm_skinny_kernel<2, false, false>)                 \
    X(SKINNY_1_KTAIL, gemm_skinny_kernel<1, true, false>)            \
    X(SKINNY_1, gemm_skinny_kernel<1, false, false>)                 \
    X(STRIP_3_F16_64, gemm_bf16x6s_kernel<3, true, 1, false>)        \
    X(STRIP_1_F16_64, gemm_bf16x6s_kernel<1, true, 1, false>)        \
    X(STRIP_3_BF16_64, gemm_bf16x6s_kernel<3, false, 1, false>)      \
    X(STRIP_1_BF16_64, gemm_bf16x6s_kernel<1, false, 1, false>)      \
    X(STRIP_3_F16_FULL, gemm_bf16x6s_kernel<3, true, 2, true>)       \
    X(STRIP_3_F16, gemm_bf16x6s_kernel<3, true, 2, false>)           \
    X(STRIP_3_BF16, gemm_bf16x6s_kernel<3, false, 2, false>)         \
    X(STRIP_1_F16, gemm_bf16x6s_kernel<1, true, 2, false>)           \
    X(STRIP_1_BF16, gemm_bf16x6s_kernel<1, false, 2, false>)         \
    X(F32_128_PROJ, gemm_f32_kernel<128, 80, 4, 1, 1, 1>)            \
    X(F32_128, gemm_f32_kernel<128, 80, 4, 1, 1, 0>)                 \
    X(F32_64, gemm_f32_kernel<64, 80, 4, 1, 2, 0>)                   \
    X(F32_32, gemm_f32_kernel<32, 64, 1, 4, 2, 0>)

enum GemmKernel {
    GEMM_NONE,
    GEMM_PER_SEGMENT,
#define DIGAT_GEMM_ENUM(id, ...) GEMM_##id,
    DIGAT_GEMM_KERNELS(DIGAT_GEMM_ENUM)
#undef DIGAT_GEMM_ENUM
};

static inline const char* gemm_kernel_name(int kernel) {
#define DIGAT_GEMM_NAME(id, ...) if (kernel == GEMM_##id) return #__VA_ARGS__;
    DIGAT_GEMM_KERNELS(DIGAT_GEMM_NAME)
#undef DIGAT_GEMM_NAME
    return kernel == GEMM_PER_SEGMENT ? "per segment" : "none";
}

struct GemmPlan {
    int status;
    int kernel;
    int mtiles, ntiles;
    unsigned grid, block;
    int image_format;
};

static inline bool gemm_kernel_takes_row_list(int kernel) {
    return kernel == GEMM_F16F8C_3 || kernel == GEMM_F16F8C_1 || (kernel >= GEMM_STRIP_3_F16_64 && kernel <= GEMM_STRIP_1_BF16);
}

static inline GemmPlan gemm_plan(const GemmArgs& g, int kind = DIGAT_KERNEL_LINEAR) {
    GemmPlan p = {DIGAT_OK, GEMM_NONE, 0, 0, 0, 256, -1};
    const int Ntot = g.nseg * g.nsegs;
    const int Md = g.m_dispatch > 0 ? g.m_dispatch : g.M;
    const auto tiles = [&](int kernel, int mtiles, int ntiles, bool round8) {
        p.kernel = kernel; p.mtiles = mtiles; p.ntiles = ntiles;
        p.grid = round8 ? (unsigned)(((mtiles * ntiles + 7) / 8) * 8) : (unsigned)(mtiles * ntiles);
        if (g.rowidx && !gemm_kernel_takes_row_list(kernel)) p.status = DIGAT_ERR_ARG;
        return p;
    };

    if (g.format == DIGAT_GEMM_F16F8C && g.wsplit) {
        const bool ok = g.nseg % 80 == 0 && g.K % 4 == 0 && g.k0 == g.K && !g.a1 && !g.transW && g.lda0 % 4 == 0 &&
                        ((uintptr_t)g.a0 & 15) == 0 && g.ldy % 4 == 0 && g.lde0 % 4 == 0 &&
                        (g.epi == EPI_NONE || g.epi == EPI_RELU_RES || g.epi == EPI_ACCUM || g.epi == EPI_ADD_E0) &&
                        !g.x1_segs && !g.x3_segs && !g.bf16_segs && !g.fp8_segs && !g.dmask;
        if (!ok) { p.status = DIGAT_ERR_ARG; return p; }
        const int strips = Ntot / 80;
        p.image_format = DIGAT_GEMM_F16F8C;
        p.block = 512;
        return strips % 3 == 0 ? tiles(GEMM_F16F8C_3, (g.M + 127) / 128, strips / 3, true)
                               : tiles(GEMM_F16F8C_1, (g.M + 127) / 128, strips, true);
    }
    if (Md < 2048 && g.nseg % 80 == 0 && g.transW && g.nsegs == 1 && g.K % 16 == 0 && g.k0 == g.K && !g.radd && !g.a1) {
        const int ntiles = Ntot / 80;
        if (((g.M + 31) / 32) * ntiles >= 480 || g.K >= 800) return tiles(GEMM_SKINNY_TW_2, (g.M + 31) / 32, ntiles, false);
        return tiles(GEMM_SKINNY_TW_1, (g.M + 15) / 16, ntiles, false);
    }
    if (Md < 2048 && g.wsplit && g.nseg % 80 == 0 && !g.transW && g.K % 8 == 0 && g.k0 % 8 == 0 && !g.radd && !g.rowidx &&
        g.ldy % 4 == 0 && g.lda0 % 4 == 0 && (!g.a1 || g.lda1 % 4 == 0) && g.lde0 % 4 == 0 && g.lde1 % 4 == 0 && g.lde2 % 4 == 0 &&
        (g.epi == EPI_NONE || g.epi == EPI_RELU_RES || g.epi == EPI_GATE || g.epi == EPI_ACCUM)) {
        if (g.format != DIGAT_GEMM_BF16X6 && g.format != DIGAT_GEMM_F16X3) p.status = DIGAT_ERR_ARG;
        p.image_format = g.format;
        const int ntiles = Ntot / 80;
        const bool mt2 = ((g.M + 31) / 32) * ntiles >= 320;
        const bool f16 = g.format == DIGAT_GEMM_F16X3;
        return tiles(mt2 ? (f16 ? GEMM_SKINNY_SPLIT_F16_2 : GEMM_SKINNY_SPLIT_BF16_2) : (f16 ? GEMM_SKINNY_SPLIT_F16_1 : GEMM_SKINNY_SPLIT_BF16_1),
                     mt2 ? (g.M + 31) / 32 : (g.M + 15) / 16, ntiles, false);
    }
    if (Md < 2048 && g.nseg % 80 == 0 && !g.transW && g.K % 4 == 0 && g.k0 % 16 == 0 && !g.radd) {
        const int ntiles = Ntot / 80;
        const bool ktail = (g.K & 15) != 0;
        if (((g.M + 31) / 32) * ntiles >= 480 || g.K >= 800)
            return tiles(ktail ? GEMM_SKINNY_2_KTAIL : GEMM_SKINNY_2, (g.M + 31) / 32, ntiles, false);
        return tiles(ktail ? GEMM_SKINNY_1_KTAIL : GEMM_SKINNY_1, (g.M + 15) / 16, ntiles, false);
    }
    const int cfg = Md >= 2048 ? 0 : ((g.nsegs > 1 && g.nseg % 80 == 0) ? 1 : 2);
    const int bn = cfg == 2 ? 64 : 80;
    if (g.nsegs > 1 && g.nseg % bn != 0) return tiles(GEMM_PER_SEGMENT, 0, 0, false);
    if (g.wsplit && cfg == 0 && g.nseg % 80 == 0 && g.K % 4 == 0 && g.K >= 32 && g.ldy % 4 == 0 && g.lde0 % 4 == 0 &&
        (g.epi == EPI_NONE || g.epi == EPI_RELU_RES || g.epi == EPI_ACCUM || g.epi == EPI_ADD_E0) && g.k0 == g.K && !g.transW) {
        if (g.format != DIGAT_GEMM_BF16X6 && g.format != DIGAT_GEMM_F16X3) p.status = DIGAT_ERR_ARG;
        else if (g.rowidx && (unsigned long long)g.M * (unsigned long long)g.lda0 * 4ull >= (1ull << 32)) p.status = DIGAT_ERR_SHAPE;
        p.image_format = g.format;
        const bool f16 = g.format == DIGAT_GEMM_F16X3;
        const int strips = Ntot / 80;
        const bool three = strips % 3 == 0;
        const int ntiles = three ? strips / 3 : strips;
        if (((g.M + 127) / 128) * ntiles < 400 && (f16 || !g.rowidx)) {
            const int k = f16 ? (three ? GEMM_STRIP_3_F16_64 : GEMM_STRIP_1_F16_64) : (three ? GEMM_STRIP_3_BF16_64 : GEMM_STRIP_1_BF16_64);
            return tiles(k, (g.M + 63) / 64, ntiles, true);
        }
        const int k = three ? (f16 ? (!g.x1_segs && !g.x3_segs ? GEMM_STRIP_3_F16_FULL : GEMM_STRIP_3_F16) : GEMM_STRIP_3_BF16)
                            : (f16 ? GEMM_STRIP_1_F16 : GEMM_STRIP_1_BF16);
        return tiles(k, (g.M + 127) / 128, ntiles, true);
    }
    const int bm = cfg == 0 ? 128 : (cfg == 1 ? 64 : 32);
    const int k = cfg == 0 ? (kind == DIGAT_KERNEL_PROJ ? GEMM_F32_128_PROJ : GEMM_F32_128) : (cfg == 1 ? GEMM_F32_64 : GEMM_F32_32);
    return tiles(k, (g.M + bm - 1) / bm, (Ntot + bn - 1) / bn, true);
}

static inline bool gemm_takes_row_list(const GemmArgs& g) { return gemm_kernel_takes_row_list(gemm_plan(g).kernel); }
```

digat_amd/csrc/digat_kernels.hip:

```cpp
#include <hip/hip_runtime.h>
#include <stdint.h>
#include <string.h>
#include <stdlib.h>
#include <atomic>
#include <initializer_list>
#include <mutex>
#include <unordered_map>
#include <utility>

#include "../../include/digat_hip.h"

typedef float v4f __attribute__((ext_vector_type(4)));

#define DIGAT_CHECK_LAUNCH()                                   \
    do {                                                       \
        if (hipGetLastError() != hipSuccess) return DIGAT_ERR_LAUNCH; \
    } while (0)

static inline size_t align_up(size_t v, size_t a) { return (v + a - 1) / a * a; }
struct Arena {
    char* base; size_t cap, used; bool ok;
    Arena() : base(nullptr), cap(SIZE_MAX), used(0), ok(true) {}
    Arena(void* p, size_t n) : base((char*)p), cap(n), used(0), ok(p != nullptr) {}
    template <class T> T* take(size_t count) {
// ... 414 lines not shown

int digat_split_weights(const float* W, int N, int K, void* wsplit, int format, void* stream) {
    if (!W || !wsplit || N <= 0 || K <= 0) return DIGAT_ERR_ARG;
    return launch_split(W, W, W, N, 1, K, wsplit, (hipStream_t)stream, 0, format);
}

#ifdef DIGAT_CF_TIMERS
extern "C" int digat_debug_cf_timers(double* out16) {
    unsigned long long h[16];
    if (hipDeviceSynchronize() != hipSuccess || hipMemcpyFromSymbol(h, HIP_SYMBOL(g_cf_timers), sizeof(h)) != hipSuccess) return DIGAT_ERR_LAUNCH;
    for (int k = 0; k < 16; ++k) { out16[k] = (double)h[k]; h[k] = 0; }
    return hipMemcpyToSymbol(HIP_SYMBOL(g_cf_timers), h, sizeof(h)) == hipSuccess ? DIGAT_OK : DIGAT_ERR_LAUNCH;
}
#endif
#ifdef DIGAT_GEMM_TIMERS
int digat_debug_gemm_timers(double* out8) {
    unsigned long long h[8];
    if (hipDeviceSynchronize() != hipSuccess || hipMemcpyFromSymbol(h, HIP_SYMBOL(g_gemm_timers), sizeof(h)) != hipSuccess) return DIGAT_ERR_LAUNCH;
    for (int k = 0; k < 8; ++k) { out8[k] = (double)h[k]; h[k] = 0; }
    return hipMemcpyToSymbol(HIP_SYMBOL(g_gemm_timers), h, sizeof(h)) == hipSuccess ? DIGAT_OK : DIGAT_ERR_LAUNCH;
}
#endif

static std::atomic<int> g_train_bf16{0};
int digat_set_train_precision(int bf16) { return g_train_bf16.exchange(bf16 ? 1 : 0); }

int digat_linear_f32x3(const float* x, int64_t ldx, const float* w, const float* b, float* y, int64_t ldy,
                       int M, int N, int K, void* wsplit, int format, void* stream) {
    if (!x || !w || !y || !wsplit || M < 0 || N <= 0 || K <= 0) return DIGAT_ERR_ARG;
    if (K % 8 || ldx % 4 || N % 80) return DIGAT_ERR_SHAPE;
    const int rcs = launch_split(w, w, w, N, 1, K, wsplit, (hipStream_t)stream, 0, format);
    if (rcs) return rcs;
    GemmArgs g = gemm_plain(x, ldx, w, b, y, ldy, M, N, K, 0);
    g.wsplit = (const unsigned short*)wsplit; g.format = format;
    if (g_train_bf16 && format != DIGAT_GEMM_F16F8C) g.x1_segs = 7;
    return launch_gemm(g, (hipStream_t)stream, DIGAT_KERNEL_PROJ);
}

struct NewsCtxWs { float *qv, *kq, *glob; };
static NewsCtxWs news_ctx_carve(Arena& a, int B, int d) {
    const size_t bd = (size_t)B * d;
    return NewsCtxWs{a.take<float>(bd), a.take<float>(bd), a.take<float>(bd)};
}
size_t digat_news_ctx_workspace_bytes(int B, int N, int d) { (void)N; Arena a; news_ctx_carve(a, B, d); return a.used; }

int digat_news_ctx_fwd(const float* X, const uint8_t* mask, const float* Kc, const float* Qc, const float* bQc,
                       const float* Wg, const float* bg, const float* addend, float* out, int B, int N, int d,
                       void* workspace, size_t workspace_bytes, void* stream) {
    if (!X || !mask || !Kc || !Qc || !Wg || !out || !workspace || B < 0 || N <= 0 || d <= 0) return DIGAT_ERR_ARG;
    if (d % 4 || N > DIGAT_MAX_NODES) return DIGAT_ERR_SHAPE;
    Arena ar(workspace, workspace_bytes);
    const NewsCtxWs w = news_ctx_carve(ar, B, d);
    if (!ar.ok) return DIGAT_ERR_WORKSPACE;
    if (B == 0) return DIGAT_OK;
    hipStream_t st = (hipStream_t)stream;
    float *qv = w.qv, *kq = w.kq, *glob = w.glob;
    const long ldx = (long)N * d;
    int rc;
    rc = launch_gemm(gemm_plain(X, ldx, Qc, bQc, qv, d, B, d, d, 0), st);
    if (rc) return rc;
    rc = launch_gemm(gemm_plain(qv, d, Kc, nullptr, kq, d, B, d, d, 1), st);
    if (rc) return rc;
    rc = launch_pool(X, ldx, kq, mask, nullptr, glob, B, N, d, st);
    if (rc) return rc;
    GemmArgs g = gemm_plain(X, ldx, Wg, bg, out, d, B, d, 2 * d, 0);
    g.k0 = d; g.a1 = glob; g.lda1 = d;
    g.epi = EPI_GATE; g.e0 = X; g.lde0 = ldx; g.e1 = glob; g.lde1 = d; g.e2 = addend; g.lde2 = d;
    return launch_gemm(g, st);
}

struct UserCtxWs { float *qv, *kq, *T, *T2; };
static UserCtxWs user_ctx_carve(Arena& a, int B, int C1, int d) {
    const size_t bd = (size_t)B * d, bcd = (size_t)B * C1 * d;
    return UserCtxWs{a.take<float>(bd), a.take<float>(bd), a.take<float>(bcd), a.take<float>(bcd)};
}
size_t digat_user_ctx_workspace_bytes(int B, int U, int H, int C1, int d) { (void)U; (void)H; Arena a; user_ctx_carve(a, B, C1, d); return a.used; }

int digat_topic_pool_fwd(const float* Xu, const float* kq, const int64_t* cat_idx, float* out,
                         int B, int U, int H, int C1, int d, void* stream) {
    if (!Xu || !kq || !cat_idx || !out || B < 0 || H < 0 || U < H || C1 <= 0 || d <= 0) return DIGAT_ERR_ARG;
    return launch_topic(Xu, (long)U * d, kq, cat_idx, out, B, H, C1, d, (hipStream_t)stream);
}

int digat_user_ctx_fwd(const float* Xu, const uint8_t* cat_mask, const int64_t* cat_idx, const float* c_n,
                       const float* Ku, const float* Qu, const float* bQu, const float* Fa, const float* bFa,
                       const float* Kua, const float* Qua, const float* bQua, const float* addend, float* out,
                       int B, int U, int H, int C1, int d, void* workspace, size_t workspace_bytes, void* stream) {
    if (!Xu || !cat_mask || !cat_idx || !c_n || !Ku || !Qu || !Fa || !Kua || !Qua || !out || !workspace)
        return DIGAT_ERR_ARG;
    if (B < 0 || H < 0 || U < H || C1 <= 0 || d <= 0) return DIGAT_ERR_ARG;
    if (d % 4 || C1 > DIGAT_MAX_NODES || H > TOPIC_MAX_H) return DIGAT_ERR_SHAPE;
    Arena ar(workspace, workspace_bytes);
    const UserCtxWs w = user_ctx_carve(ar, B, C1, d);
    if (!ar.ok) return DIGAT_ERR_WORKSPACE;
    if (B == 0) return DIGAT_OK;
    hipStream_t st = (hipStream_t)stream;
    float *qv = w.qv, *kq = w.kq, *T = w.T, *T2 = w.T2;
    int rc;
    rc = launch_gemm(gemm_plain(c_n, d, Qu, bQu, qv, d, B, d, d, 0), st);
    if (rc) return rc;
    rc = launch_gemm(gemm_plain(qv, d, Ku, nullptr, kq, d, B, d, d, 1), st);
    if (rc) return rc;
    rc = launch_topic(Xu, (long)U * d, kq, cat_idx, T, B, H, C1, d, st);
    if (rc) return rc;
    GemmArgs g = gemm_plain(T, d, Fa, bFa, T2, d, B * C1, d, d, 0);
    g.epi = EPI_RELU_RES; g.e0 = T; g.lde0 = d;
    rc = launch_gemm(g, st);
    if (rc) return rc;
    rc = launch_gemm(gemm_plain(c_n, d, Qua, bQua, qv, d, B, d, d, 0), st);
    if (rc) return rc;
    rc = launch_gemm(gemm_plain(qv, d, Kua, nullptr, kq, d, B, d, d, 1), st);
    if (rc) return rc;
    return launch_pool(T2, (long)C1 * d, kq, cat_mask, addend, out, B, C1, d, st);
}

__global__ void __launch_bounds__(256) transpose_kernel(const float* __restrict__ in, float* __restrict__ out, int d) {
    __shared__ float tile[32][33];
    const int bx = blockIdx.x * 32, by = blockIdx.y * 32;
    for (int r = threadIdx.y; r < 32; r += 8) {
        const int y = by + r, x = bx + threadIdx.x;
        if (y < d && x < d) tile[r][threadIdx.x] = in[(long)y * d + x];
    }
    __syncthreads();
    for (int r = threadIdx.y; r < 32; r += 8) {
        const int y = bx + r, x = by + threadIdx.x;
        if (y < d && x < d) out[(long)y * d + x] = tile[threadIdx.x][r];
    }
}

size_t digat_fold_workspace_bytes(int d) { return 2 * align_up((size_t)d * d * 4, 256); }

int digat_fold_attention(const float* K, const float* Q, const float* bQ, float* Wf, float* bf, int d,
                         void* workspace, size_t workspace_bytes, void* stream) {
    if (!K || !Q || !Wf || !bf || !workspace || d <= 0) return DIGAT_ERR_ARG;
    if (d % 4) return DIGAT_ERR_SHAPE;
    if (workspace_bytes < digat_fold_workspace_bytes(d)) return DIGAT_ERR_WORKSPACE;
    hipStream_t st = (hipStream_t)stream;
    float* Kt = (float*)workspace;
    float* Qt = (float*)((char*)workspace + align_up((size_t)d * d * 4, 256));
    const dim3 grid((d + 31) / 32, (d + 31) / 32), block(32, 8);
    hipLaunchKernelGGL(transpose_kernel, grid, block, 0, st, K, Kt, d);
    hipLaunchKernelGGL(transpose_kernel, grid, block, 0, st, Q, Qt, d);
    DIGAT_CHECK_LAUNCH();
    int rc = launch_gemm(gemm_plain(Kt, d, Qt, nullptr, Wf, d, d, d, d, 0), st);
    if (rc) return rc;
    if (bQ) return launch_gemm(gemm_plain(bQ, d, Kt, nullptr, bf, d, 1, d, d, 0), st);
    return hipMemsetAsync(bf, 0, (size_t)d * 4, st) == hipSuccess ? DIGAT_OK : DIGAT_ERR_LAUNCH;
}

static size_t max_sz(size_t a, size_t b) { return a > b ? a : b; }


enum { ENC_PLAIN, ENC_GROUPED, ENC_SHARED };
struct FoldCtxWs { float *T, *T2, *glob; };
struct EncoderWs {
    float *Xu[2], *Xn[2];
    char* xws; size_t xws_bytes;
    XattnWs xu;
    char* cws; size_t cws_bytes;
    FoldCtxWs fc;
    float *kq_t, *kq_u, *r_user[2], *r_news;
    char* xws_news; size_t xws_news_bytes;
    XattnWs xn;
    int *cnt, *off, *idx, *cnt2, *off2, *idx2, *entries, *flag, *hlast;
    uint8_t *flags1, *flags2;
    int *cnt_n, *off_n, *idx_n; uint8_t* flags_n;
    int *l0_gs, *l0_off; uint8_t* l0_lead; int* l0_idx;
    unsigned* tw_word; int* tw_list; uint8_t* tw_flags; int *tw_cnt, *tw_off;
    int *gl_off, *gl_idx;
    int* idx32;
    uint8_t *Au, *cm; int64_t* ci;
    uint8_t *fg, *tfg; unsigned* twg; uint8_t* bfg; int *cg, *eg, *hg, *bcg, *tcg;
    uint8_t *same, *is_leader, *lead; int* leader_of;
};
static bool encoder_carve(Arena& a, int B, int N, int H, int C, int d, int variant, EncoderWs& e) {
    const int U = H + C, C1 = C + 1, nmax = N > U ? N : U;
    const size_t b = (size_t)B, bd = b * d, bu = b * U;
    e = EncoderWs();
    for (float*& x : e.Xu) x = a.take<float>(bu * d);
    for (float*& x : e.Xn) x = a.take<float>(b * N * d);
    Arena xa = a.sub(digat_xattn_workspace_bytes(B, nmax, d));
    e.xws = xa.base; e.xws_bytes = xa.cap;
    e.xu = xattn_carve(xa, B, U, d);
    Arena ca = a.sub(max_sz(digat_news_ctx_workspace_bytes(B, N, d), digat_user_ctx_workspace_bytes(B, U, H, C1, d)));
    e.cws = ca.base; e.cws_bytes = ca.cap;
    e.fc = FoldCtxWs{ca.take<float>(b * C1 * d), ca.take<float>(b * C1 * d), ca.take<float>(bd)};
    e.kq_t = a.take<float>(bd); e.kq_u = a.take<float>(bd);
    e.r_user[0] = a.take<float>(bd); e.r_news = a.take<float>(bd); e.r_user[1] = a.take<float>(bd);
    Arena na = a.sub(digat_xattn_workspace_bytes(B, N, d));
    e.xws_news = na.base; e.xws_news_bytes = na.cap;
    e.xn = xattn_carve(na, B, N, d);
    e.cnt = a.take<int>(b); e.off = a.take<int>(b + 1); e.idx = a.take<int>(bu);
    e.cnt2 = a.take<int>(b); e.off2 = a.take<int>(b + 1); e.idx2 = a.take<int>(b * C1);
    e.entries = a.take<int>(b); e.flag = a.take<int>(64); e.hlast = a.take<int>(b);
    e.flags1 = a.take<uint8_t>(bu); e.flags2 = a.take<uint8_t>(b * C1);
    e.cnt_n = a.take<int>(b); e.off_n = a.take<int>(b + 1); e.idx_n = a.take<int>(b * N); e.flags_n = a.take<uint8_t>(b * N);
    e.l0_gs = a.take<int>(b + 64); e.l0_off = a.take<int>(b + 64); e.l0_lead = a.take<uint8_t>(b); e.l0_idx = a.take<int>(bu);
    e.tw_word = a.take<unsigned>(bu); e.tw_list = a.take<int>(bu); e.tw_flags = a.take<uint8_t>(bu);
    e.tw_cnt = a.take<int>(b + 64); e.tw_off = a.take<int>(b + 64);
    e.gl_off = a.take<int>(b + 64); e.gl_idx = a.take<int>(bu);
    e.idx32 = a.take<int>(b);
    if (variant == ENC_GROUPED) {
        const size_t g = b / 4 + 1;
        e.Au = a.take<uint8_t>(bu * U); e.cm = a.take<uint8_t>(b * C1); e.ci = a.take<int64_t>(b * H);
        e.fg = a.take<uint8_t>(g * U); e.tfg = a.take<uint8_t>(g * U); e.twg = a.take<unsigned>(g * U); e.bfg = a.take<uint8_t>(g * C1);
        for (int** x : {&e.cg, &e.eg, &e.hg, &e.bcg, &e.tcg}) *x = a.take<int>(g);
    } else if (variant == ENC_SHARED) {
        e.same = a.take<uint8_t>(b); e.is_leader = a.take<uint8_t>(b); e.lead = a.take<uint8_t>(b); e.leader_of = a.take<int>(b);
    }
    return a.ok && xa.ok && ca.ok && na.ok;
}
static size_t encoder_ws_bytes(int B, int N, int H, int C, int d, int variant) { Arena a; EncoderWs e; encoder_carve(a, B, N, H, C, d, variant, e); return a.used; }

struct EncoderCall {
    const digat_params* p;
    const float* Xn_in; const uint8_t *An, *Mn;
    const float* ue;
    const uint8_t *Au, *cat_mask; const int64_t* cat_idx;
    const float* c_n0; float *out_news, *out_user;
    int B, N, H;
    void* workspace; size_t workspace_bytes; hipStream_t st;
    int variant;
    const int* row_group; int G;
    const uint8_t *Au_g, *cm_g; const int64_t* ci_g;
    const float *news_hpq0, *hist_hpq0, *topic_hpq0, *ctxq0; const int64_t* news_index; int64_t news_rows;
    const uint8_t *run_leader, *run_lead;
    EncoderWs ws;
};
struct SideStream { hipStream_t s; hipEvent_t fork, join, early; int ok; };
constexpr int SPARSE_PER_NODE = 20;
static SideStream* side_stream(hipStream_t caller) {
    struct Entry { int dev; hipStream_t caller; SideStream side; int state; };
    static Entry tab[64];
    static int used = 0;
    static std::mutex mu;
    int dev = 0;
    if (hipGetDevice(&dev) != hipSuccess) return nullptr;
    std::lock_guard<std::mutex> lock(mu);
    for (int i = 0; i < used; ++i)
        if (tab[i].dev == dev && tab[i].caller == caller) return tab[i].state == 1 ? &tab[i].side : nullptr;
    if (used == 64) return nullptr;
    Entry& e = tab[used++];
    e.dev = dev; e.caller = caller;
    SideStream& x = e.side;
    const bool ok = hipStreamCreateWithFlags(&x.s, hipStreamNonBlocking) == hipSuccess &&
                    hipEventCreateWithFlags(&x.fork, hipEventDisableTiming) == hipSuccess &&
                    hipEventCreateWithFlags(&x.join, hipEventDisableTiming) == hipSuccess &&
                    hipEventCreateWithFlags(&x.early, hipEventDisableTiming) == hipSuccess;
    e.state = ok ? 1 : -1;
    return ok ? &x : nullptr;
}

static int encoder_fwd_folded(const EncoderCall& c, const float* Xg0) {
    const digat_params* p = c.p;
    const EncoderWs& w = c.ws;
    const int B = c.B, N = c.N, H = c.H, G = c.G;
    const uint8_t *An = c.An, *Mn = c.Mn, *Au = c.Au, *cat_mask = c.cat_mask, *run_leader = c.run_leader, *run_lead = c.run_lead;
    const int64_t* cat_idx = c.cat_idx;
    const int* row_group = c.row_group;
    const float *news_hpq0 = c.news_hpq0, *ctxq0 = c.ctxq0;
    float *c_n = c.out_news, *c_u = c.out_user;
    hipStream_t st = c.st;
    const bool shared = run_leader != nullptr && run_lead != nullptr && row_group != nullptr;
    const float* c_n_src = c.c_n0 && p->depth > 0 ? c.c_n0 : c_n;
    const bool xu0_grouped = Xg0 != nullptr;
    const int d = p->d, C = p->category_num, L = p->depth, U = H + C, C1 = C + 1;
    const int fmt = (p->flags & DIGAT_PARAMS_GEMM_F16X3) ? 1 : 0;
    unsigned* const rflag = fmt ? (unsigned*)p->range_flag : nullptr;
    const int lfmt = (p->flags & DIGAT_PARAMS_PROJ_F16F8C) ? DIGAT_GEMM_F16F8C : fmt;
    const int bd_disp = (p->flags & DIGAT_PARAMS_BD_TILED) ? (1 << 30) : 1;
    float *T = w.fc.T, *T2 = w.fc.T2, *glob = w.fc.glob;
    const int* bucket_idx = nullptr;
    const int* nbuckets_dev = nullptr;
    const int* hist_last = nullptr;
    int rc;
    auto from_c_n = [&](int next_layer, hipStream_t sq) -> int {
        GemmArgs g = gemm_plain(next_layer == 0 ? c_n_src : c_n, d, p->user_news_fold_W, p->user_news_fold_b, w.kq_t, d, B, d, d, 0);
        g.w[1] = p->userAtt_fold_W; g.bias[1] = p->userAtt_fold_b; g.y[1] = w.kq_u;
        g.nsegs = 2;
        if (next_layer < L) {
            g.w[2] = p->user[next_layer].F3; g.bias[2] = p->user[next_layer].b3; g.y[2] = w.r_user[next_layer & 1];
            g.nsegs = 3;
        }
        g.wsplit = (const unsigned short*)p->ctx_wsplit[next_layer]; g.format = fmt; g.range_flag = rflag;
        g.m_dispatch = bd_disp;
        return launch_gemm(g, sq);
    };
    auto user_ctx_tail = [&](const float* Xu_cur, const float* addend, hipStream_t sq, const int* xgroup = nullptr,
                             const uint8_t* live = nullptr, const float* kq_topic = nullptr, const float* kq_user = nullptr) -> int {
        if (!kq_topic) { kq_topic = w.kq_t; kq_user = w.kq_u; }
        if (p->featureAffine_fsplit && fmt == 1 && ctxfused_ok(H, C1, d)) {
            const CtxFusedArgs fa{Xu_cur, (long)U * d, xgroup, live, U, live ? hist_last : nullptr, kq_topic, kq_user, cat_idx, cat_mask, addend, c_u,
                                  (const uint4*)p->featureAffine_fsplit, p->featureAffine_b, rflag, B, H, C1, d, sqrtf((float)d)};
            return launch_user_ctx_fused(fa, sq);
        }
        int e = launch_topic(Xu_cur, (long)U * d, kq_topic, cat_idx, T, B, H, C1, d, sq, xgroup, live, U, live ? hist_last : nullptr);
        if (e) return e;
        GemmArgs g = gemm_plain(T, d, p->featureAffine_W, p->featureAffine_b, T2, d, B * C1, d, d, 0);
        g.epi = EPI_RELU_RES; g.e0 = T; g.lde0 = d;
        g.wsplit = (const unsigned short*)p->featureAffine_wsplit;
        g.format = fmt; g.range_flag = rflag;
        if (bucket_idx && gemm_takes_row_list(g)) { g.rowidx = bucket_idx; g.nrows_dev = nbuckets_dev; }
        e = launch_gemm(g, sq);
        if (e) return e;
        return launch_pool(T2, (long)C1 * d, kq_user, cat_mask, addend, c_u, B, C1, d, sq);
    };
    auto news_ctx = [&](const float* Xn_cur, hipStream_t sq, bool first) -> int {
        const long ldx = (long)N * d;
        float* kq = w.kq_t;
        GemmArgs gq = gemm_plain(Xn_cur, ldx, p->cand_fold_W, p->cand_fold_b, kq, d, B, d, d, 0);
        gq.wsplit = (const unsigned short*)p->cand_fold_wsplit; gq.format = fmt; gq.range_flag = rflag;
        gq.m_dispatch = bd_disp;
        int e = launch_gemm(gq, sq);
        if (e) return e;
        e = launch_pool(Xn_cur, ldx, kq, Mn, nullptr, glob, B, N, d, sq);
        if (e) return e;
        GemmArgs g = gemm_plain(Xn_cur, ldx, p->news_graph_W, p->news_graph_b, c_n, d, B, d, 2 * d, 0);
        g.k0 = d; g.a1 = glob; g.lda1 = d;
        g.epi = EPI_GATE; g.e0 = Xn_cur; g.lde0 = ldx; g.e1 = glob; g.lde1 = d; g.e2 = first ? c_n_src : c_n; g.lde2 = d;
        g.wsplit = (const unsigned short*)p->gate_wsplit; g.format = fmt; g.range_flag = rflag;
        g.m_dispatch = 1;
        return launch_gemm(g, sq);
    };

    const bool want_live = L > 0 && !(p->flags & DIGAT_PARAMS_NO_LIVE_ROWS);
    int sparse_mode = p->flags & 3;
    if (sparse_mode == 3 || (sparse_mode == DIGAT_XATTN_AUTO && L == 0)) sparse_mode = DIGAT_XATTN_DENSE;
    const int* sparse_flag = nullptr;
    const int pq_x3 = (p->flags & DIGAT_PROJ_PQ_X3) ? 1 : 0;
    const int pq_mode = ((p->flags & DIGAT_PQ_BF16) ? 1 : 0) | ((p->flags & DIGAT_PQ_X1) ? 2 : 0) | ((p->flags & DIGAT_PQ_FP8) ? 4 : 0);
    const bool want_scan = want_live || sparse_mode == DIGAT_XATTN_AUTO;
    const int* rowidx = nullptr;
    const int* nrows_dev = nullptr;
    uint8_t* live_flags = nullptr;
    const int *pend_rowidx = nullptr, *pend_nrows = nullptr, *pend_bidx = nullptr, *pend_nb = nullptr, *pend_hlast = nullptr;

    uint8_t* pend_flags = nullptr;
    const bool l0_chunked = row_group && (Xg0 || shared) && want_live &&
                            sparse_mode == DIGAT_XATTN_SPARSE && d / 4 <= 128 && U <= 128;
    const uint8_t* const l0_lead = shared ? run_lead : w.l0_lead;
    const bool twins = want_live && sparse_mode == DIGAT_XATTN_SPARSE && d / 4 <= 128 && U <= 128 && L > 1;
    unsigned* const tw_word = w.tw_word; uint8_t* const tw_flags = w.tw_flags;
    int *const tw_list = w.tw_list, *const tw_cnt = w.tw_cnt, *const tw_off = w.tw_off;
    int *const gl_off = w.gl_off, *const gl_idx = w.gl_idx, *const l0_gs = w.l0_gs, *const l0_off = w.l0_off, *const l0_idx = w.l0_idx;
    TwinLists tw_pub{nullptr, nullptr, nullptr};
    auto find_live_rows = [&](hipStream_t sq) -> int {
        int *cnt = w.cnt, *off = w.off, *idx = w.idx, *cnt2 = w.cnt2, *off2 = w.off2, *idx2 = w.idx2, *entries = w.entries, *flag = w.flag;
        int* hlast = w.hlast; uint8_t *flags1 = w.flags1, *flags2 = w.flags2;
        ProfScope prof(DIGAT_KERNEL_GLUE, (double)B * ((double)U * U + 2.0 * C1 + H * 8.0) + (double)B * (U + C1) * 6, sq);
        if (l0_chunked && !shared) {
            hipLaunchKernelGGL(sparse_l0_chunks_kernel, dim3(1), dim3(1024), 0, sq, row_group, B, G, SPARSE_L0_ROWS, l0_gs, w.l0_lead);
            DIGAT_CHECK_LAUNCH();
        }
        if (shared) {
            const bool want_entries = sparse_mode == DIGAT_XATTN_AUTO;
            hipLaunchKernelGGL(user_live_flags_kernel, dim3((B + 3) / 4), dim3(256), (size_t)4 * ((U * U + 63) & ~63), sq, Au, cat_mask, cat_idx, B, U, H, C1,
                               flags1, cnt, want_entries ? entries : (int*)nullptr, hlast, flags2, cnt2,
                               twins ? tw_word : (unsigned*)nullptr, twins ? tw_flags : (uint8_t*)nullptr, twins ? tw_cnt : (int*)nullptr,
                               run_leader);
            DIGAT_CHECK_LAUNCH();
            const LiveExpand le{flags1, twins ? tw_word : nullptr, tw_flags, flags2, cnt, entries, hlast, cnt2, tw_cnt,
                                flags1, twins ? tw_word : nullptr, tw_flags, flags2,
                                cnt, want_entries ? entries : nullptr, hlast, cnt2, twins ? tw_cnt : nullptr};
            hipLaunchKernelGGL(live_expand_kernel, dim3((B + 3) / 4), dim3(256), 0, sq, le, row_group, B, U, C1);
            DIGAT_CHECK_LAUNCH();
        } else if (c.variant == ENC_GROUPED) {
            uint8_t *fg = w.fg, *tfg = w.tfg, *bfg = w.bfg; unsigned* twg = w.twg;
            int *cg = w.cg, *eg = w.eg, *hg = w.hg, *bcg = w.bcg, *tcg = w.tcg;
            const bool want_entries = sparse_mode == DIGAT_XATTN_AUTO;
            hipLaunchKernelGGL(user_live_flags_kernel, dim3((G + 3) / 4), dim3(256), (size_t)4 * ((U * U + 63) & ~63), sq, c.Au_g, c.cm_g, c.ci_g, G, U, H, C1,
                               fg, cg, want_entries ? eg : (int*)nullptr, hg, bfg, bcg,
                               twins ? twg : (unsigned*)nullptr, twins ? tfg : (uint8_t*)nullptr, twins ? tcg : (int*)nullptr);
            DIGAT_CHECK_LAUNCH();
            const LiveExpand le{fg, twins ? twg : nullptr, tfg, bfg, cg, eg, hg, bcg, tcg,
                                flags1, twins ? tw_word : nullptr, tw_flags, flags2,
                                cnt, want_entries ? entries : nullptr, hlast, cnt2, twins ? tw_cnt : nullptr};
            hipLaunchKernelGGL(live_expand_kernel, dim3((B + 3) / 4), dim3(256), 0, sq, le, row_group, B, U, C1);
            DIGAT_CHECK_LAUNCH();
        } else {
            hipLaunchKernelGGL(user_live_flags_kernel, dim3((B + 3) / 4), dim3(256), (size_t)4 * ((U * U + 63) & ~63), sq, Au, cat_mask, cat_idx, B, U, H, C1,
                               flags1, cnt, sparse_mode == DIGAT_XATTN_AUTO ? entries : (int*)nullptr, hlast, flags2, cnt2,
                               twins ? tw_word : (unsigned*)nullptr, twins ? tw_flags : (uint8_t*)nullptr, twins ? tw_cnt : (int*)nullptr);
            DIGAT_CHECK_LAUNCH();
        }
        if (sparse_mode == DIGAT_XATTN_AUTO) {
            hipLaunchKernelGGL(sparse_decide_kernel, dim3(1), dim3(1024), 0, sq, (const int*)entries, B, U, SPARSE_PER_NODE, flag);
            DIGAT_CHECK_LAUNCH();
            sparse_flag = flag;
        }
        ScanPair sp{{cnt, cnt2}, {off, off2}, {nullptr, nullptr}};
        ListPair lp{{flags1, flags2}, {off, off2}, {U, C1, U, U, U, U}, {idx, idx2}, {nullptr, nullptr}};
        int jobs = 2;
        if (l0_chunked) {
            sp.cnt[jobs] = cnt; sp.off[jobs] = l0_off; sp.rowmask[jobs] = l0_lead;
            lp.flags[jobs] = flags1; lp.off[jobs] = l0_off; lp.out[jobs] = l0_idx; lp.rowmask[jobs] = l0_lead;
            ++jobs;
        }
        if (twins) {
            sp.cnt[jobs] = tw_cnt; sp.off[jobs] = tw_off;
            lp.flags[jobs] = tw_flags; lp.off[jobs] = tw_off; lp.out[jobs] = tw_list;
            lp.width[jobs] = U;
            ++jobs;
        }
        if (shared) {
            sp.cnt[jobs] = cnt; sp.off[jobs] = gl_off; sp.rowmask[jobs] = run_leader;
            lp.flags[jobs] = flags1; lp.off[jobs] = gl_off; lp.out[jobs] = gl_idx; lp.rowmask[jobs] = run_leader;
            lp.width[jobs] = U;
            ++jobs;
        }
        hipLaunchKernelGGL(exclusive_scan2_kernel, dim3(jobs), dim3(1024), 0, sq, sp, B);
        DIGAT_CHECK_LAUNCH();
        hipLaunchKernelGGL(live_list2_kernel, dim3((B + 3) / 4, jobs), dim3(256), 0, sq, lp, B);
        DIGAT_CHECK_LAUNCH();
        pend_rowidx = idx; pend_nrows = off + B; pend_bidx = idx2; pend_nb = off2 + B; pend_flags = flags1; pend_hlast = hlast;
        return DIGAT_OK;
    };
    auto publish_live_rows = [&]() {
        rowidx = pend_rowidx; nrows_dev = pend_nrows; bucket_idx = pend_bidx; nbuckets_dev = pend_nb; live_flags = pend_flags;
        hist_last = pend_hlast;
        if (twins) tw_pub = TwinLists{tw_word, tw_list, tw_off + B};
    };
    const int side_mode = (p->flags & DIGAT_PARAMS_SIDE_STREAM_OFF) ? 0 : ((p->flags & DIGAT_PARAMS_SIDE_STREAM_ON) ? 1 : 2);
    SideStream* side = (side_mode == 0 || (side_mode == 2 && B >= 2048)) ? nullptr : side_stream(st);
    const bool news_early = L > 0 && N <= 16 && d / 4 <= 256;
    const bool news_lists_on = L > 0 && d / 4 <= 256 && !(p->flags & DIGAT_PARAMS_NO_LIVE_ROWS);
    const bool news_lists = news_lists_on && ((!news_early && (p->flags & DIGAT_NEWS_XATTN_SPARSE) && N > 16) || (news_early && L > 1 && B >= 2048));
    const int* news_rowidx = nullptr; const int* news_nrows = nullptr; const uint8_t* news_flags = nullptr;
    auto news_project = [&](int layer, const float* Xn_cur, hipStream_t sq) -> int {
        const digat_layer_params& ln = p->news[layer];
        GemmArgs gp = gemm_plain(Xn_cur, d, ln.W, ln.bW, w.xn.h, d, B * N, d, d, 0);
        gp.w[1] = ln.F1; gp.bias[1] = nullptr; gp.y[1] = w.xn.P;
        gp.w[2] = ln.F2; gp.bias[2] = nullptr; gp.y[2] = w.xn.Q;
        gp.nsegs = 3;
        gp.x3_segs = pq_x3 ? 6 : 0;
        gp.m_dispatch = 1 << 30;
        gp.wsplit = (const unsigned short*)ln.wsplit;
        gp.format = lfmt; gp.range_flag = rflag;
        if (news_rowidx && gemm_takes_row_list(gp)) { gp.rowidx = news_rowidx; gp.nrows_dev = news_nrows; }
        return launch_gemm(gp, sq, DIGAT_KERNEL_PROJ);
    };
    auto group_project = [&](hipStream_t sq) -> int {
        const digat_layer_params& lu = p->user[0];
        if (shared) {
            GemmArgs gs = gemm_plain(w.Xu[0], d, lu.W, lu.bW, w.xu.h, d, B * U, d, d, 0);
            gs.w[1] = lu.F1; gs.bias[1] = nullptr; gs.y[1] = w.xu.P;
            gs.w[2] = lu.F2; gs.bias[2] = nullptr; gs.y[2] = w.xu.Q;
            gs.nsegs = 3;
            gs.x3_segs = pq_x3 ? 6 : 0;
            gs.wsplit = (const unsigned short*)lu.wsplit;
            gs.format = lfmt; gs.range_flag = rflag;
            gs.m_dispatch = B * U;
            if (want_live && gemm_takes_row_list(gs)) { gs.rowidx = gl_idx; gs.nrows_dev = gl_off + B; }
            return launch_gemm(gs, sq, DIGAT_KERNEL_PROJ);
        }
        const size_t ndg = (size_t)G * U * d;
        float* Xg = xu0_grouped ? const_cast<float*>(Xg0) : w.Xu[1];
        float* h0 = w.xu.h;
        float* P0 = h0 + ndg;
        float* Q0 = w.xu.Q;
        const long total4 = (long)ndg / 4;
        int blocks = (int)((total4 + 255) / 256);
        if (blocks > 2048) blocks = 2048;
        if (!xu0_grouped) {
            hipLaunchKernelGGL(build_user_nodes_kernel, dim3(blocks), dim3(256), 0, sq, (const float4*)c.ue,
                               (const float4*)p->topic_node_embedding, (float4*)Xg, (long)G, H, C, d / 4, (const int*)nullptr);
            DIGAT_CHECK_LAUNCH();
        }
        if (c.hist_hpq0 && c.topic_hpq0 && (long)B * U >= 2048) {
            float* dst[3] = {h0, P0, Q0};
            UserNodes3 un3;
            for (int t = 0; t < 3; ++t) {
                un3.hist[t] = (const float4*)(c.hist_hpq0 + (size_t)t * G * H * d);
                un3.topic[t] = (const float4*)(c.topic_hpq0 + (size_t)t * C * d);
                un3.dst[t] = (float4*)dst[t];
            }
            hipLaunchKernelGGL(build_user_nodes3_kernel, dim3(blocks, 3), dim3(256), 0, sq, un3, (long)G, H, C, d / 4);
            DIGAT_CHECK_LAUNCH();
            return DIGAT_OK;
        }
        GemmArgs gg = gemm_plain(Xg, d, lu.W, lu.bW, h0, d, G * U, d, d, 0);
        gg.w[1] = lu.F1; gg.bias[1] = nullptr; gg.y[1] = P0;
        gg.w[2] = lu.F2; gg.bias[2] = nullptr; gg.y[2] = Q0;
        gg.nsegs = 3;
        gg.x3_segs = pq_x3 ? 6 : 0;
        gg.wsplit = (const unsigned short*)lu.wsplit;
        gg.format = lfmt; gg.range_flag = rflag;
        gg.m_dispatch = B * U;
        return launch_gemm(gg, sq, DIGAT_KERNEL_PROJ);
    };
    const bool group_early = side && L > 0 && row_group;
    const bool live_early = side && want_scan;
    if (side && (news_early || group_early || live_early)) {
        if (hipEventRecord(side->fork, st) != hipSuccess || hipStreamWaitEvent(side->s, side->fork, 0) != hipSuccess)
            return DIGAT_ERR_LAUNCH;
    }
    if (live_early) {
        rc = find_live_rows(side->s);
        if (rc) return rc;
    }
    if (group_early) {
        rc = group_project(side->s);
        if (rc) return rc;
    }
    if (group_early || live_early) {
        if (hipEventRecord(side->early, side->s) != hipSuccess) return DIGAT_ERR_LAUNCH;
    }
    if (news_early && !news_hpq0) {
        rc = news_project(0, c.Xn_in, side ? side->s : st);
        if (rc) return rc;
    }
    const size_t bd = (size_t)B * d;
    if (!ctxq0) {
        rc = from_c_n(0, st);
        if (rc) return rc;
    }
    const bool xu0_shared = shared && sparse_mode == DIGAT_XATTN_SPARSE;
    rc = user_ctx_tail(xu0_grouped ? Xg0 : w.Xu[0], nullptr, st, (xu0_grouped || xu0_shared) ? row_group : nullptr, nullptr,
                       ctxq0 ? ctxq0 : nullptr, ctxq0 ? ctxq0 + bd : nullptr);
    if (rc) return rc;
    const float* xn_cur = c.Xn_in;
    int un = 0, nn = 0;
    for (int i = 0; i < L; ++i) {
        const digat_layer_params& ln = p->news[i];
        const digat_layer_params& lu = p->user[i];
        const float* r_user = (i == 0 && ctxq0 && L > 0) ? ctxq0 + 2 * bd : w.r_user[i & 1];
        hipStream_t sn = side ? side->s : st;
        if (side && i == 0) {
            if (hipEventRecord(side->fork, st) != hipSuccess || hipStreamWaitEvent(sn, side->fork, 0) != hipSuccess)
                return DIGAT_ERR_LAUNCH;
        }
        if (side && i > 0) {
            if (hipStreamWaitEvent(st, side->join, 0) != hipSuccess) return DIGAT_ERR_LAUNCH;
        }
        if (i == 0 && want_scan && !live_early) {
            rc = find_live_rows(st);
            if (rc) return rc;
        }
        if (i == 0 && side && (group_early || live_early)) {
            if (hipStreamWaitEvent(st, side->early, 0) != hipSuccess) return DIGAT_ERR_LAUNCH;
        }
        if (i == 0 && want_live) publish_live_rows();
        if (i == 0 && row_group) {
            const size_t ndg = shared ? (size_t)B * U * d : (size_t)G * U * d;
            float* h0 = w.xu.h;
            float* P0 = h0 + ndg;
            float* P = w.xu.P;
            float* Q0 = w.xu.Q;
            if (!group_early) {
                rc = group_project(st);
                if (rc) return rc;
            }
            rc = DIGAT_OK;
            if (sparse_mode != DIGAT_XATTN_DENSE && d / 4 <= 256) {
                const bool l0_live = want_live && live_flags;
                SparseArgs sg{P0, Q0, h0, xu0_grouped ? Xg0 : w.Xu[0], lu.a, Au, w.Xu[1], r_user, row_group, l0_live ? live_flags : nullptr,
                                    sparse_mode == DIGAT_XATTN_AUTO ? sparse_flag : nullptr, B, U, d / 4, (xu0_grouped || xu0_shared) ? 1 : 0,
                                    (!l0_live && xu0_grouped && want_live) ? (const uint8_t*)pend_flags : nullptr, w.Xu[0],
                                    l0_live ? rowidx : nullptr, l0_live ? nrows_dev : nullptr, G, nullptr, 0, 0};
                if (l0_chunked && l0_live && sparse_l0_ok(sg)) {
                    rc = launch_sparse_l0(sg, l0_lead, l0_idx, l0_off + B, shared ? (B + SPARSE_L0_ROWS - 1) / SPARSE_L0_ROWS : G, st);
                } else
                rc = launch_sparse(sg, st);
            }
            if (!rc && !(sparse_mode == DIGAT_XATTN_SPARSE && d / 4 <= 256)) {
                const int* skip_if = sparse_mode == DIGAT_XATTN_AUTO && d / 4 <= 256 ? sparse_flag : nullptr;
                const size_t nd = (size_t)B * U * d;
                float* alpha = w.xu.alpha;
                {
                    const long total4 = (long)nd / 4;
                    int blocks = (int)((total4 + 255) / 256);
                    if (blocks > 4096) blocks = 4096;
                    ProfScope prof(DIGAT_KERNEL_GLUE, skip_if ? 0.0 : (double)nd * 4, st);
                    hipLaunchKernelGGL(expand_proj_kernel, dim3(blocks), dim3(256), 0, st, (const float4*)P0, (const float4*)r_user,
                                       row_group, (float4*)P, (long)B, U, d / 4, skip_if);
                    DIGAT_CHECK_LAUNCH();
                }
                rc = launch_xattn_pairwise(P, Q0, h0, w.Xu[0], lu.a, Au, w.Xu[1], alpha, B, U, d, st, nullptr, row_group, nullptr, true,
                                           skip_if);
            }
        } else {
            XattnOpts o;
            o.wsplit = lu.wsplit; o.rowidx = rowidx; o.nrows_dev = nrows_dev; o.live = live_flags;
            o.sparse_mode = sparse_mode; o.sparse_flag = sparse_flag; o.pq_x3 = pq_x3; o.pq_mode = i > 0 ? pq_mode : 0;
            o.centre_limit = (i > 0 && i == L - 1 && sparse_mode == DIGAT_XATTN_SPARSE) ? H : 0;
            o.gemm_format = lfmt; o.range_flag = rflag;
            o.tw = (i > 0 && tw_pub.word) ? &tw_pub : nullptr;
            rc = xattn_core(w.Xu[un], Au, r_user, lu.W, lu.bW, lu.F1, lu.F2, lu.a, w.Xu[un ^ 1], nullptr, B, U, d, w.xws, w.xws_bytes, st, o);
        }
        if (rc) return rc;
        if (side && hipEventRecord(side->fork, st) != hipSuccess) return DIGAT_ERR_LAUNCH;
        {
            GemmArgs g3 = gemm_plain(c_u, d, ln.F3, ln.b3, w.r_news, d, B, d, d, 0);
            g3.wsplit = (const unsigned short*)ln.f3_wsplit; g3.format = fmt; g3.range_flag = rflag;
            g3.m_dispatch = bd_disp;
            rc = launch_gemm(g3, sn);
        }
        if (rc) return rc;
        if (i == 0 && news_lists) {
            int *cnt_n = w.cnt_n, *off_n = w.off_n, *idx_n = w.idx_n; uint8_t* flags_n = w.flags_n;
            ProfScope prof(DIGAT_KERNEL_GLUE, (double)B * ((double)N * N + 6.0 * N), sn);
            hipLaunchKernelGGL(news_live_flags_kernel, dim3((B + 3) / 4), dim3(256), (size_t)4 * ((N * N + 15) & ~15), sn, An, Mn, B, N, flags_n, cnt_n);
            DIGAT_CHECK_LAUNCH();
            ScanPair sp{{cnt_n}, {off_n}, {nullptr}};
            ListPair lp{{flags_n}, {off_n}, {N, N, N, N, N, N}, {idx_n}, {nullptr}};
            hipLaunchKernelGGL(exclusive_scan2_kernel, dim3(1), dim3(1024), 0, sn, sp, B);
            DIGAT_CHECK_LAUNCH();
            hipLaunchKernelGGL(live_list2_kernel, dim3((B + 3) / 4, 1), dim3(256), 0, sn, lp, B);
            DIGAT_CHECK_LAUNCH();
            news_rowidx = idx_n; news_nrows = off_n + B; news_flags = flags_n;
        }
        if (news_early) {
            const size_t ndn = (size_t)B * N * d;
            const float* hn = (i == 0 && news_hpq0) ? news_hpq0 : w.xn.h;
            const bool tab = i == 0 && news_hpq0 && c.news_index;
            const size_t plane = tab ? (size_t)c.news_rows * N * d : ndn;
            rc = launch_xattn_pairwise(hn + plane, hn + 2 * plane, hn, xn_cur, ln.a, An, w.Xn[nn], w.xn.alpha, B, N, d, sn, nullptr, nullptr,
                                       w.r_news, false, nullptr, tab ? c.news_index : nullptr);
        } else if (i == 0 && news_hpq0 && c.news_index) {
            const size_t plane = (size_t)c.news_rows * N * d;
            hipLaunchKernelGGL(index_to_i32_kernel, dim3((B + 255) / 256), dim3(256), 0, sn, c.news_index, w.idx32, B);
            DIGAT_CHECK_LAUNCH();
            SparseArgs sgn{news_hpq0 + plane, news_hpq0 + 2 * plane, news_hpq0, xn_cur, ln.a, An, w.Xn[nn], w.r_news, w.idx32, news_flags,
                           nullptr, B, N, d / 4, 1, nullptr, nullptr, news_rowidx, news_nrows, B, nullptr, 0, 0};
            if (news_rowidx) sgn.prof_part = XPART_NEWS + 1;
            rc = launch_sparse(sgn, sn);
        } else {
            XattnOpts o;
            o.wsplit = ln.wsplit; o.rowidx = news_rowidx; o.nrows_dev = news_nrows; o.live = news_flags;
            o.sparse_mode = (p->flags & DIGAT_NEWS_XATTN_SPARSE) ? DIGAT_XATTN_SPARSE : DIGAT_XATTN_DENSE;
            o.pq_x3 = pq_x3;
            o.pq_mode = pq_mode;
            o.gemm_format = lfmt; o.range_flag = rflag;
            o.prof_part = news_rowidx ? XPART_NEWS + 1 : 0;
            rc = xattn_core(xn_cur, An, w.r_news, ln.W, ln.bW, ln.F1, ln.F2, ln.a, w.Xn[nn], nullptr, B, N, d, w.xws_news, w.xws_news_bytes, sn, o);
        }
        if (rc) return rc;
        xn_cur = w.Xn[nn]; nn ^= 1; un ^= 1;
        rc = news_ctx(xn_cur, sn, i == 0);
        if (rc) return rc;
        rc = from_c_n(i + 1, sn);
        if (rc) return rc;
        if (side && hipEventRecord(side->join, sn) != hipSuccess) return DIGAT_ERR_LAUNCH;
        if (news_early && i + 1 < L) {
            rc = news_project(i + 1, xn_cur, sn);
            if (rc) return rc;
        }
        if (side && hipStreamWaitEvent(sn, side->fork, 0) != hipSuccess) return DIGAT_ERR_LAUNCH;
        rc = user_ctx_tail(w.Xu[un], c_u, sn, nullptr, live_flags);
        if (rc) return rc;
    }
    if (side && L > 0) {
        if (hipEventRecord(side->join, side->s) != hipSuccess || hipStreamWaitEvent(st, side->join, 0) != hipSuccess)
            return DIGAT_ERR_LAUNCH;
    }
    return DIGAT_OK;
}

size_t digat_encoder_workspace_bytes(int B, int N, int H, int C, int d, int depth) { (void)depth; return encoder_ws_bytes(B, N, H, C, d, ENC_PLAIN); }

static int encoder_fwd_impl(EncoderCall& c) {
    const digat_params* p = c.p;
    const bool grouped = c.variant == ENC_GROUPED;
    if (!p || !c.Xn_in || !c.An || !c.Mn || !c.ue || !c.out_news || !c.out_user || !c.workspace) return DIGAT_ERR_ARG;
    if (grouped ? (!c.Au_g || !c.cm_g || !c.ci_g || !c.row_group || c.G <= 0) : (!c.Au || !c.cat_mask || !c.cat_idx)) return DIGAT_ERR_ARG;
    const int B = c.B, N = c.N, H = c.H;
    if (B < 0 || N <= 0 || H < 0) return DIGAT_ERR_ARG;
    const int d = p->d, C = p->category_num, L = p->depth, U = H + C;
    const bool folded = p->cand_fold_W && p->user_news_fold_W && p->userAtt_fold_W;
    if (grouped && !folded) return DIGAT_ERR_ARG;
    if (d <= 0 || d % 4 || L < 0 || L > DIGAT_MAX_DEPTH || N > DIGAT_MAX_NODES || U > DIGAT_MAX_NODES || C < 0)
        return DIGAT_ERR_SHAPE;
    if (grouped && (size_t)4 * c.G > (size_t)B) return DIGAT_ERR_SHAPE;
    Arena ar(c.workspace, c.workspace_bytes);
    if (!encoder_carve(ar, B, N, H, C, d, c.variant, c.ws)) return DIGAT_ERR_WORKSPACE;
    if (B == 0) return DIGAT_OK;
    if (c.news_index && !(c.c_n0 && c.news_hpq0 && L > 0 && d / 4 <= 256 && c.news_rows > 0 && c.news_rows <= 0x7fffffffLL &&
                          (N <= 16 || ((p->flags & DIGAT_NEWS_XATTN_SPARSE) && N <= DIGAT_MAX_NODES)) && folded)) return DIGAT_ERR_ARG;
    hipStream_t st = c.st;
    const EncoderWs& w = c.ws;
    int rc;
    if (grouped) {
        const GatherJobs jobs{{c.Au_g, c.cm_g, (const uint8_t*)c.ci_g}, {w.Au, w.cm, (uint8_t*)w.ci}, {(long)U * U, (long)(C + 1), (long)H * 8}};
        hipLaunchKernelGGL(gather_rows_kernel, dim3(B), dim3(256), 0, st, jobs, c.row_group, (long)B);
        DIGAT_CHECK_LAUNCH();
        c.Au = w.Au; c.cat_mask = w.cm; c.cat_idx = w.ci;
    } else if (c.variant == ENC_SHARED) {
        ProfScope prof(DIGAT_KERNEL_GLUE, (double)B * ((double)H * d * 4 + (double)U * U + (C + 1) + 8.0 * H), st);
// ... 304 lines not shown
```

digat_amd/graphEncoders.py:

```python
from __future__ import annotations

import contextlib
import math
import threading

import torch
import torch.nn as nn

from . import _lib
from .layers import ScaledDotProductAttention

_TLS = threading.local()


class GraphEncoder(nn.Module):
    def __init__(self, config, news_embedding_dim: int):
        super().__init__()
        self.news_graph_size = config.news_graph_size
        self.user_graph_size = config.max_history_num + config.category_num
        self.max_history_num = config.max_history_num
        self.category_num = config.category_num + 1
        self.news_embedding_dim = news_embedding_dim
        self.graph_depth = config.graph_depth
        self.dropout_rate = float(config.dropout_rate)
        self.attention_scalar = math.sqrt(float(self.news_embedding_dim))
        self.topic_node_embedding = nn.Parameter(torch.zeros([config.category_num, self.news_embedding_dim]))

    def initialize(self):
        nn.init.zeros_(self.topic_node_embedding)

    def forward(self, news_graph_embeddings, news_graph, news_graph_mask, user_news_embedding, user_graph,
                user_category_mask, user_category_indices):
        raise Exception('Function forward must be implemented at sub-class')

    def inference(self, news_graph_embeddings, news_graph, news_graph_mask, user_news_embedding, user_graph,
                  user_category_mask, user_category_indices, news_graph_context):
        raise Exception('Function inference must be implemented at sub-class')


class DIGAT(GraphEncoder):
    def __init__(self, config, news_embedding_dim: int):
        super().__init__(config, news_embedding_dim)
        d, L = self.news_embedding_dim, self.graph_depth
        if d % 4 != 0:
            raise ValueError("digat_amd needs news_embedding_dim % 4 == 0 (float4 rows)")
        if L > _lib.DIGAT_MAX_DEPTH or max(self.news_graph_size, self.user_graph_size) > _lib.DIGAT_MAX_NODES:
            raise ValueError("graph_depth <= %d and graph sizes <= %d are supported"
                             % (_lib.DIGAT_MAX_DEPTH, _lib.DIGAT_MAX_NODES))
        self.candidate_attention = ScaledDotProductAttention(d, d, d)
        self.news_graph_W = nn.Linear(d * 2, d, bias=True)
        self.user_news_K = nn.Linear(d, d, bias=False)
        self.user_news_Q = nn.Linear(d, d, bias=True)
        self.featureAffine = nn.Linear(d, d, bias=True)
        self.userAttention = ScaledDotProductAttention(d, d, d)
        for g in ("news", "user"):
            setattr(self, f"{g}_graph_attention_W", nn.ModuleList([nn.Linear(d, d, bias=True) for _ in range(L)]))
            setattr(self, f"{g}_graph_attention_ffn1", nn.ModuleList([nn.Linear(d, d, bias=False) for _ in range(L)]))
            setattr(self, f"{g}_graph_attention_ffn2", nn.ModuleList([nn.Linear(d, d, bias=False) for _ in range(L)]))
            setattr(self, f"{g}_graph_attention_ffn3", nn.ModuleList([nn.Linear(d, d, bias=True) for _ in range(L)]))
            setattr(self, f"{g}_graph_attention_a", nn.ModuleList([nn.Linear(d, 1, bias=False) for _ in range(L)]))
        self._param_block = None
        self.projection_mode = "auto"
        self._resolved_pm = None
        self._range_flag = None
        self.range_fallback = False
        self.corpus_activation_max = None
        self.pass_rows = 4096
        self.user_xattn_mode = "auto"
        self.news_xattn_mode = "auto"
        self.corpus_xattn_hint = {}
        self.side_stream = "auto"
        self.live_rows = True
        self.fused_user_context = False

    def initialize(self):
        super().initialize()
        relu_gain = nn.init.calculate_gain('relu')
        leaky_gain = nn.init.calculate_gain('leaky_relu', 0.2)
        for g in ("news", "user"):
            for i in range(self.graph_depth):
                nn.init.xavier_uniform_(getattr(self, f"{g}_graph_attention_W")[i].weight)
                nn.init.zeros_(getattr(self, f"{g}_graph_attention_W")[i].bias)
                nn.init.xavier_uniform_(getattr(self, f"{g}_graph_attention_a")[i].weight, gain=leaky_gain)
                for f in ("ffn1", "ffn2", "ffn3"):
                    nn.init.xavier_uniform_(getattr(self, f"{g}_graph_attention_{f}")[i].weight, gain=relu_gain)
                nn.init.zeros_(getattr(self, f"{g}_graph_attention_ffn3")[i].bias)
        self.candidate_attention.initialize()
        nn.init.xavier_uniform_(self.news_graph_W.weight)
        nn.init.zeros_(self.news_graph_W.bias)
        nn.init.xavier_uniform_(self.user_news_K.weight)
        nn.init.xavier_uniform_(self.user_news_Q.weight)
        nn.init.zeros_(self.user_news_Q.bias)
        nn.init.xavier_uniform_(self.featureAffine.weight, gain=relu_gain)
        nn.init.zeros_(self.featureAffine.bias)
        self.userAttention.initialize()

    @contextlib.contextmanager
    def launch_options(self, side_stream=None, live_rows=None, shared_users=None):
        table = _TLS.__dict__.setdefault("opts", {})
        prev = table.get(id(self))
        cur = dict(prev or {})
        if side_stream is not None:
            if side_stream not in ("auto", "on", "off"):
                raise ValueError("side_stream must be 'auto', 'on' or 'off'")
            cur["side_stream"] = side_stream
        if live_rows is not None:
            cur["live_rows"] = bool(live_rows)
        if shared_users is not None:
            cur["detect_shared_users"] = bool(shared_users)
        table[id(self)] = cur
        try:
            yield self
        finally:
            if prev is None:
                table.pop(id(self), None)
            else:
                table[id(self)] = prev

    def _launch_option(self, name):
        return _TLS.__dict__.get("opts", {}).get(id(self), {}).get(name, getattr(self, name))

    def resolved_xattn_mode(self, g: str) -> str:
        mode = getattr(self, f"{g}_xattn_mode", "auto")
        return self.corpus_xattn_hint.get(g, "auto") if mode == "auto" else mode

    def _apply(self, fn, *args, **kwargs):
        self._param_block = None
        return super()._apply(fn, *args, **kwargs)

    def _params(self) -> "_lib.Params":
        pm = self.resolved_projection_mode()
        fmt = self.gemm_format()
        ptrs = tuple(p.data_ptr() for p in self.parameters())
        if self._param_block is not None and self._param_block[0] == ptrs and self._param_block[2] == self._fold_key():
            return self._call_block(self._param_block[1])
        for p in self.parameters():
            if p.device.type != "cuda" or p.dtype != torch.float32 or not p.is_contiguous():
                raise _lib.DigatHipError("DIGAT parameters must be contiguous float32 CUDA tensors "
                                         "(call model.cuda()); there is no CPU path")
        P = _lib.Params()
        P.d, P.depth, P.category_num = self.news_embedding_dim, self.graph_depth, self.category_num - 1
        P.flags = self._flags()
        P.topic_node_embedding = self.topic_node_embedding.data_ptr()
        P.cand_K = self.candidate_attention.K.weight.data_ptr()
        P.cand_Q = self.candidate_attention.Q.weight.data_ptr()
        P.cand_bQ = self.candidate_attention.Q.bias.data_ptr()
        P.news_graph_W = self.news_graph_W.weight.data_ptr()
        P.news_graph_b = self.news_graph_W.bias.data_ptr()
        P.user_news_K = self.user_news_K.weight.data_ptr()
        P.user_news_Q = self.user_news_Q.weight.data_ptr()
        P.user_news_bQ = self.user_news_Q.bias.data_ptr()
        P.featureAffine_W = self.featureAffine.weight.data_ptr()
        P.featureAffine_b = self.featureAffine.bias.data_ptr()
        P.userAtt_K = self.userAttention.K.weight.data_ptr()
        P.userAtt_Q = self.userAttention.Q.weight.data_ptr()
        P.userAtt_bQ = self.userAttention.Q.bias.data_ptr()
        for g, arr in (("news", P.news), ("user", P.user)):
            for i in range(self.graph_depth):
                lp = arr[i]
                W = getattr(self, f"{g}_graph_attention_W")[i]
                lp.W, lp.bW = W.weight.data_ptr(), W.bias.data_ptr()
                lp.F1 = getattr(self, f"{g}_graph_attention_ffn1")[i].weight.data_ptr()
                lp.F2 = getattr(self, f"{g}_graph_attention_ffn2")[i].weight.data_ptr()
                F3 = getattr(self, f"{g}_graph_attention_ffn3")[i]
                lp.F3, lp.b3 = F3.weight.data_ptr(), F3.bias.data_ptr()
                lp.a = getattr(self, f"{g}_graph_attention_a")[i].weight.data_ptr()
        P._splits = []
        if pm in ("bf16x6", "bf16x6-pq3", "pq-bf16", "pq-bf16-x1", "pq-fp8", "fp16x3", "fp16-fp8c") and self.news_embedding_dim % 80 == 0:
            L_ = _lib.lib()
            d = self.news_embedding_dim
            lfmt = _lib.GEMM_F16F8C if pm == "fp16-fp8c" else fmt
            nbytes = L_.digat_split_weights_bytes_format(3 * d, d, lfmt)
            for g, arr in (("news", P.news), ("user", P.user)):
                for i in range(self.graph_depth):
                    buf = _lib.split_buffer(nbytes, self.topic_node_embedding.device)
                    _lib.check(L_.digat_split_proj_weights(
                        getattr(self, f"{g}_graph_attention_W")[i].weight.data_ptr(),
                        getattr(self, f"{g}_graph_attention_ffn1")[i].weight.data_ptr(),
                        getattr(self, f"{g}_graph_attention_ffn2")[i].weight.data_ptr(), d, buf.data_ptr(), lfmt,
                        _lib.stream_ptr()), "digat_split_proj_weights")
                    arr[i].wsplit = buf.data_ptr()
                    P._splits.append(buf)
            buf = _lib.split_buffer(L_.digat_split_weights_bytes(d, d), self.topic_node_embedding.device)
            _lib.check(L_.digat_split_weights(self.featureAffine.weight.data_ptr(), d, d, buf.data_ptr(), fmt, _lib.stream_ptr()),
                       "digat_split_weights")
            P.featureAffine_wsplit = buf.data_ptr()
            P._splits.append(buf)
            if fmt == _lib.GEMM_F16X3:
                P.range_flag = self.range_flag().data_ptr()
        P._folds = None
        if not self.training:
            P._folds = self._fold_attention()
            (P.cand_fold_W, P.cand_fold_b, P.user_news_fold_W, P.user_news_fold_b,
             P.userAtt_fold_W, P.userAtt_fold_b) = (t.data_ptr() for t in P._folds)
            if P._splits:
                L_, d, dev = _lib.lib(), self.news_embedding_dim, self.topic_node_embedding.device

                def image(rows, K, fn, *args):
                    buf = _lib.split_buffer(L_.digat_split_weights_bytes(rows, K), dev)
                    _lib.check(fn(*args, buf.data_ptr(), fmt, _lib.stream_ptr()), "split")
                    P._splits.append(buf)
                    return buf.data_ptr()
                for i in range(self.graph_depth):
                    P.news[i].f3_wsplit = image(d, d, L_.digat_split_weights, self.news_graph_attention_ffn3[i].weight.data_ptr(), d, d)
                P.cand_fold_wsplit = image(d, d, L_.digat_split_weights, P.cand_fold_W, d, d)
                P.gate_wsplit = image(d, 2 * d, L_.digat_split_weights, self.news_graph_W.weight.data_ptr(), d, 2 * d)
                for l in range(self.graph_depth + 1):
                    third = self.user_graph_attention_ffn3[l].weight.data_ptr() if l < self.graph_depth else P.userAtt_fold_W
                    P.ctx_wsplit[l] = image(3 * d, d, L_.digat_split_proj_weights, P.user_news_fold_W, P.userAtt_fold_W, third, d)
                if fmt == _lib.GEMM_F16X3 and self.fused_user_context:
                    buf = _lib.split_buffer(L_.digat_split_ctx_fused_bytes(d), dev)
                    _lib.check(L_.digat_split_ctx_fused_weights(self.featureAffine.weight.data_ptr(), d, buf.data_ptr(), _lib.stream_ptr()),
                               "digat_split_ctx_fused_weights")
                    P._splits.append(buf)
                    P.featureAffine_fsplit = buf.data_ptr()
        self._param_block = (ptrs, P, self._fold_key())
        return self._call_block(P)

    def _call_block(self, P):
        Q = _lib.Params.from_buffer_copy(P)
        Q.flags = self._flags()
        return Q

    def resolved_projection_mode(self) -> str:
        return self._auto_base() if self.projection_mode == "auto" else self.projection_mode

    def gemm_format(self) -> int:
        pm = self.projection_mode
        if pm in ("fp16x3", "fp16-fp8c") or (pm in ("auto", "pq-bf16", "pq-fp8") and self._auto_base() == "fp16x3"):
            return _lib.GEMM_F16X3
        return _lib.GEMM_BF16X6

    def _auto_base(self) -> str:
        if self.news_embedding_dim % 80 != 0:
            return "bf16x6"
        ws = [m.weight for g in ("news", "user") for f in ("W", "ffn1", "ffn2") for m in getattr(self, f"{g}_graph_attention_{f}")]
        ws.append(self.featureAffine.weight)
        key = tuple((w.data_ptr(), w._version) for w in ws + [self.topic_node_embedding])
        key += (self.corpus_activation_max, self.range_fallback)
        if self._resolved_pm is None or self._resolved_pm[0] != key:
            amax = self.corpus_activation_max
            ok = amax is not None and not self.range_fallback
            if ok:
                wmax = float(torch.stack([w.detach().abs().max() for w in ws]).max())
                tmax = float(self.topic_node_embedding.detach().abs().max())
                ok = wmax < 32.0 and amax < 256.0 and tmax < 256.0
            self._resolved_pm = (key, "fp16x3" if ok else "bf16x6")
        return self._resolved_pm[1]

    def range_flag(self) -> torch.Tensor:
        dev = self.topic_node_embedding.device
        if self._range_flag is None or self._range_flag.device != dev:
            self._range_flag = torch.zeros(1, dtype=torch.int32, device=dev)
        return self._range_flag

    def range_overflowed(self, reset: bool = True) -> bool:
        if self._range_flag is None:
            return False
        hit = bool(int(self._range_flag.item()))
        if reset and hit:
            self._range_flag.zero_()
        return hit

    def _flags(self) -> int:
        pm = self.projection_mode
        return ({"auto": 0, "dense": 1, "sparse": 2}[self.resolved_xattn_mode("user")]
                | (4 if pm in ("bf16x6-pq3", "pq-bf16", "pq-fp8") else 0)
                | (8 if self.resolved_xattn_mode("news") == "sparse" else 0)
                | (16 if pm in ("pq-bf16", "pq-bf16-x1") else 0)
                | (32 if pm == "pq-bf16-x1" else 0)
                | (256 if pm == "pq-fp8" else 0)
                | (_lib.PARAMS_GEMM_F16X3 if self.gemm_format() == _lib.GEMM_F16X3 else 0)
                | (_lib.PARAMS_PROJ_F16F8C if pm == "fp16-fp8c" else 0)
                | (_lib.PARAMS_BD_TILED if self.pass_rows >= 2048 else 0)
                | {"auto": 0, "off": _lib.PARAMS_SIDE_STREAM_OFF, "on": _lib.PARAMS_SIDE_STREAM_ON}[self._launch_option("side_stream")]
                | (0 if self._launch_option("live_rows") else _lib.PARAMS_NO_LIVE_ROWS))

    def _fold_sources(self):
        ca, ua = self.candidate_attention, self.userAttention
        return ((ca.K.weight, ca.Q.weight, ca.Q.bias), (self.user_news_K.weight, self.user_news_Q.weight,
                                                        self.user_news_Q.bias), (ua.K.weight, ua.Q.weight, ua.Q.bias))

    def _fold_key(self):
        key = (self.training, self.resolved_projection_mode(), self.gemm_format()) + tuple(t._version for trio in self._fold_sources() for t in trio)
        for g in ("news", "user"):
            for f in ("W", "ffn1", "ffn2"):
                key += tuple(m.weight._version for m in getattr(self, f"{g}_graph_attention_{f}"))
        return key + (self.featureAffine.weight._version, bool(self.fused_user_context))

    def _fold_attention(self):
        L = _lib.lib()
        d = self.news_embedding_dim
        dev = self.topic_node_embedding.device
        nbytes = L.digat_fold_workspace_bytes(d)
        ws = _lib.workspace(nbytes, dev, "fold")
        out = []
        for K, Q, b in self._fold_sources():
            Wf = torch.empty((d, d), dtype=torch.float32, device=dev)
            bf = torch.empty((d,), dtype=torch.float32, device=dev)
            _lib.check(L.digat_fold_attention(K.data_ptr(), Q.data_ptr(), b.data_ptr(), Wf.data_ptr(), bf.data_ptr(), d,
                                              ws.data_ptr(), nbytes, _lib.stream_ptr()), "digat_fold_attention")
            out += [Wf, bf]
        return out

    def _eval_only(self, what: str):
        if self.training and self.dropout_rate > 0 and torch.is_grad_enabled():
            raise NotImplementedError(
                f"{what}: the HIP path implements eval-mode semantics (dropout = identity); "
                "call model.eval() / torch.no_grad(), or train through digat_amd.training")

    def compute_news_graph_context(self, news_graph_embeddings, news_graph_mask):
        X = _lib.f32(news_graph_embeddings)
        dev = _lib.require_device(X, news_graph_mask)
        B, N, d = X.shape
        mask = _lib.as_bytes(news_graph_mask)
        out = torch.empty((B, d), dtype=torch.float32, device=dev)
        if B == 0:
            return out
        L = _lib.lib()
        nbytes = L.digat_news_ctx_workspace_bytes(B, N, d)
        ws = _lib.workspace(nbytes, dev, "ctx")
        ca, g = self.candidate_attention, self.news_graph_W
        _lib.check(L.digat_news_ctx_fwd(X.data_ptr(), mask.data_ptr(), ca.K.weight.data_ptr(), ca.Q.weight.data_ptr(),
                                        ca.Q.bias.data_ptr(), g.weight.data_ptr(), g.bias.data_ptr(), None,
                                        out.data_ptr(), B, N, d, ws.data_ptr(), nbytes, _lib.stream_ptr()),
                   "digat_news_ctx_fwd")
        return out

    def compute_user_graph_context(self, user_graph_embeddings, user_category_mask, user_category_indices,
                                   news_graph_context):
        Xu = _lib.f32(user_graph_embeddings)
        c_n = _lib.f32(news_graph_context)
        dev = _lib.require_device(Xu, user_category_mask, user_category_indices, c_n)
        B, U, d = Xu.shape
        H, C1 = self.max_history_num, self.category_num
        mask = _lib.as_bytes(user_category_mask)
        idx = user_category_indices.to(torch.int64).contiguous()
        out = torch.empty((B, d), dtype=torch.float32, device=dev)
        if B == 0:
            return out
        L = _lib.lib()
        nbytes = L.digat_user_ctx_workspace_bytes(B, U, H, C1, d)
        ws = _lib.workspace(nbytes, dev, "ctx")
        ua = self.userAttention
        _lib.check(L.digat_user_ctx_fwd(Xu.data_ptr(), mask.data_ptr(), idx.data_ptr(), c_n.data_ptr(),
                                        self.user_news_K.weight.data_ptr(), self.user_news_Q.weight.data_ptr(),
                                        self.user_news_Q.bias.data_ptr(), self.featureAffine.weight.data_ptr(),
                                        self.featureAffine.bias.data_ptr(), ua.K.weight.data_ptr(),
                                        ua.Q.weight.data_ptr(), ua.Q.bias.data_ptr(), None, out.data_ptr(),
                                        B, U, H, C1, d, ws.data_ptr(), nbytes, _lib.stream_ptr()),
                   "digat_user_ctx_fwd")
        return out

    def _xattn(self, g: str, index: int, X, A, ctx, return_alpha: bool = False):
        X, ctx = _lib.f32(X), _lib.f32(ctx)
        dev = _lib.require_device(X, A, ctx)
        B, n, d = X.shape
        adj = _lib.as_bytes(A)
        out = torch.empty_like(X)
        alpha = torch.empty((B, n, n), dtype=torch.float32, device=dev) if return_alpha else None
        if B == 0:
            return (out, alpha) if return_alpha else out
        L = _lib.lib()
        nbytes = L.digat_xattn_workspace_bytes(B, n, d)
        ws = _lib.workspace(nbytes, dev, "xattn")
        W = getattr(self, f"{g}_graph_attention_W")[index]
        F3 = getattr(self, f"{g}_graph_attention_ffn3")[index]
        mode = self.resolved_xattn_mode(g)
        if mode == "sparse" and not return_alpha and n > 16 and d <= 1024:
            _lib.check(L.digat_xattn_fwd_mode(X.data_ptr(), adj.data_ptr(), ctx.data_ptr(), W.weight.data_ptr(), W.bias.data_ptr(),
                                              getattr(self, f"{g}_graph_attention_ffn1")[index].weight.data_ptr(),
                                              getattr(self, f"{g}_graph_attention_ffn2")[index].weight.data_ptr(),
                                              F3.weight.data_ptr(), F3.bias.data_ptr(),
                                              getattr(self, f"{g}_graph_attention_a")[index].weight.data_ptr(),
                                              out.data_ptr(), B, n, d, 2, ws.data_ptr(), nbytes, _lib.stream_ptr()),
                       "digat_xattn_fwd_mode")
            return out
        _lib.check(L.digat_xattn_fwd(X.data_ptr(), adj.data_ptr(), ctx.data_ptr(), W.weight.data_ptr(),
                                     W.bias.data_ptr(),
                                     getattr(self, f"{g}_graph_attention_ffn1")[index].weight.data_ptr(),
                                     getattr(self, f"{g}_graph_attention_ffn2")[index].weight.data_ptr(),
                                     F3.weight.data_ptr(), F3.bias.data_ptr(),
                                     getattr(self, f"{g}_graph_attention_a")[index].weight.data_ptr(),
                                     out.data_ptr(), _lib.ptr(alpha), B, n, d, ws.data_ptr(), nbytes,
                                     _lib.stream_ptr()), "digat_xattn_fwd")
        return (out, alpha) if return_alpha else out

    def compute_news_graph_embeddings(self, index, news_graph_embeddings, news_graph, user_graph_context):
        self._eval_only("compute_news_graph_embeddings")
        return self._xattn("news", index, news_graph_embeddings, news_graph, user_graph_context)

    def compute_user_graph_embeddings(self, index, user_graph_embeddings, user_graph, news_graph_context):
        self._eval_only("compute_user_graph_embeddings")
        return self._xattn("user", index, user_graph_embeddings, user_graph, news_graph_context)

    def _encode(self, news_graph_embeddings, news_graph, news_graph_mask, user_news_embedding, user_graph,
                user_category_mask, user_category_indices, news_graph_context, shared: bool = False):
        Xn, ue = _lib.f32(news_graph_embeddings), _lib.f32(user_news_embedding)
        dev = _lib.require_device(Xn, news_graph, news_graph_mask, ue, user_graph, user_category_mask,
                                  user_category_indices)
        B, N, d = Xn.shape
        H, C = self.max_history_num, self.category_num - 1
        if ue.shape != (B, H, d) or user_graph.shape[1] != H + C or N != self.news_graph_size:
            raise _lib.DigatHipError("input shapes do not match the encoder's configuration")
        An, Mn = _lib.as_bytes(news_graph), _lib.as_bytes(news_graph_mask)
        Au, cm = _lib.as_bytes(user_graph), _lib.as_bytes(user_category_mask)
        ci = user_category_indices.to(torch.int64).contiguous()
        c0 = None if news_graph_context is None else _lib.f32(news_graph_context)
        out_n = torch.empty((B, d), dtype=torch.float32, device=dev)
        out_u = torch.empty((B, d), dtype=torch.float32, device=dev)
        if B == 0:
            return out_n, out_u
        L = _lib.lib()
        nbytes = (L.digat_encoder_shared_workspace_bytes if shared else L.digat_encoder_workspace_bytes)(B, N, H, C, d, self.graph_depth)
        ws = _lib.workspace(nbytes, dev, "encoder")
        P = self._params()
        X = _lib.ext()
        if X is not None:
            X.encoder_fwd(_lib.addressof(P), bool(shared), Xn, An, Mn, ue, Au, cm, ci, c0, out_n, out_u, ws)
            return out_n, out_u
        fn, what = (L.digat_encoder_fwd_shared, "digat_encoder_fwd_shared") if shared else (L.digat_encoder_fwd, "digat_encoder_fwd")
        _lib.check(fn(P, Xn.data_ptr(), An.data_ptr(), Mn.data_ptr(), ue.data_ptr(), Au.data_ptr(),
                      cm.data_ptr(), ci.data_ptr(), _lib.ptr(c0), out_n.data_ptr(), out_u.data_ptr(),
                      B, N, H, ws.data_ptr(), nbytes, _lib.stream_ptr()), what)
        return out_n, out_u

    def project_news_layer0(self, news_graph_embeddings):
        X = _lib.f32(news_graph_embeddings)
        dev = _lib.require_device(X)
# ... 349 lines not shown
```

include/digat_hip.h:

```cpp
#ifndef DIGAT_HIP_H
#define DIGAT_HIP_H

#include <stddef.h>
#include <stdint.h>

#ifdef __cplusplus
extern "C" {
#endif

#define DIGAT_ABI_VERSION 4
#define DIGAT_MAX_NODES 128
#define DIGAT_MAX_DEPTH 16

enum {
    DIGAT_OK = 0,
    DIGAT_ERR_ARG = 1,
    DIGAT_ERR_SHAPE = 2,
    DIGAT_ERR_WORKSPACE = 3,
    DIGAT_ERR_LAUNCH = 4
};

int digat_version(void);
const char* digat_error_string(int code);

int digat_linear_f32(const float* x, int64_t ldx, const float* w, const float* b, float* y, int64_t ldy,
                     int M, int N, int K, void* stream);

size_t digat_split_weights_bytes(int rows, int K);
int digat_forget_split_image(const void* wsplit);
int digat_split_proj_weights(const float* W, const float* F1, const float* F2, int d, void* wsplit, int format, void* stream);
int digat_split_weights(const float* W, int N, int K, void* wsplit, int format, void* stream);
int digat_linear_f32x3(const float* x, int64_t ldx, const float* w, const float* b, float* y, int64_t ldy,
                       int M, int N, int K, void* wsplit, int format, void* stream);

size_t digat_xattn_workspace_bytes(int B, int n, int d);
int digat_xattn_fwd(const float* X, const uint8_t* A, const float* ctx,
                    const float* W, const float* bW, const float* F1, const float* F2,
                    const float* F3, const float* b3, const float* a,
                    float* out, float* alpha_out, int B, int n, int d,
                    void* workspace, size_t workspace_bytes, void* stream);
int digat_xattn_fwd_mode(const float* X, const uint8_t* A, const float* ctx,
                         const float* W, const float* bW, const float* F1, const float* F2,
                         const float* F3, const float* b3, const float* a,
                         float* out, int B, int n, int d, int mode,
                         void* workspace, size_t workspace_bytes, void* stream);

int digat_xattn_fwd_lowprec(const float* X, const uint8_t* A, const float* ctx,
                            const float* W, const float* bW, const float* F1, const float* F2,
                            const float* F3, const float* b3, const float* a, const void* wsplit, int format,
                            float* out, int B, int n, int d, int pq,
                            void* workspace, size_t workspace_bytes, void* stream);

int digat_xattn_pairwise_fwd(const float* Pr, const float* Q, const float* h, const float* X,
                             const float* a, const uint8_t* A,
                             float* out, float* alpha, int B, int n, int d, void* stream);

size_t digat_news_ctx_workspace_bytes(int B, int N, int d);
int digat_news_ctx_fwd(const float* X, const uint8_t* mask,
                       const float* Kc, const float* Qc, const float* bQc,
                       const float* Wg, const float* bg,
                       const float* addend, float* out, int B, int N, int d,
                       void* workspace, size_t workspace_bytes, void* stream);

size_t digat_user_ctx_workspace_bytes(int B, int U, int H, int C1, int d);
int digat_user_ctx_fwd(const float* Xu, const uint8_t* cat_mask, const int64_t* cat_idx, const float* c_n,
                       const float* Ku, const float* Qu, const float* bQu,
                       const float* Fa, const float* bFa,
                       const float* Kua, const float* Qua, const float* bQua,
                       const float* addend, float* out, int B, int U, int H, int C1, int d,
                       void* workspace, size_t workspace_bytes, void* stream);

int digat_topic_pool_fwd(const float* Xu, const float* kq, const int64_t* cat_idx, float* out,
                         int B, int U, int H, int C1, int d, void* stream);

enum { DIGAT_XATTN_AUTO = 0, DIGAT_XATTN_DENSE = 1, DIGAT_XATTN_SPARSE = 2 };
enum { DIGAT_PROJ_PQ_X3 = 4 };
enum { DIGAT_NEWS_XATTN_SPARSE = 8 };
enum { DIGAT_PQ_BF16 = 16, DIGAT_PQ_X1 = 32 };
enum { DIGAT_PQ_FP8 = 256 };
enum { DIGAT_PARAMS_GEMM_F16X3 = 64 };
enum { DIGAT_PARAMS_BD_TILED = 128 };

typedef struct digat_layer_params {
    const float *W, *bW;
    const float *F1;
    const float *F2;
    const float *F3, *b3;
    const float *a;
    const void  *wsplit;
    const void  *f3_wsplit;
} digat_layer_params;

typedef struct digat_params {
    int32_t d;
    int32_t depth;
    int32_t category_num;
    int32_t flags;
    const float *topic_node_embedding;
    const float *cand_K, *cand_Q, *cand_bQ;
    const float *news_graph_W, *news_graph_b;
    const float *user_news_K, *user_news_Q, *user_news_bQ;
    const float *featureAffine_W, *featureAffine_b;
    const float *userAtt_K, *userAtt_Q, *userAtt_bQ;
    digat_layer_params news[DIGAT_MAX_DEPTH];
    digat_layer_params user[DIGAT_MAX_DEPTH];
    const float *cand_fold_W, *cand_fold_b;
    const float *user_news_fold_W, *user_news_fold_b;
    const float *userAtt_fold_W, *userAtt_fold_b;
    const void  *featureAffine_wsplit;
    const void  *cand_fold_wsplit, *gate_wsplit;
    const void  *ctx_wsplit[DIGAT_MAX_DEPTH + 1];
    uint32_t    *range_flag;
    const void  *featureAffine_fsplit;
} digat_params;

size_t digat_split_ctx_fused_bytes(int d);
int digat_split_ctx_fused_weights(const float* W, int d, void* image, void* stream);

size_t digat_fold_workspace_bytes(int d);
int digat_fold_attention(const float* K, const float* Q, const float* bQ, float* Wf, float* bf, int d,
                         void* workspace, size_t workspace_bytes, void* stream);

size_t digat_encoder_workspace_bytes(int B, int N, int H, int C, int d, int depth);
int digat_encoder_fwd(const digat_params* params,
                      const float* news_graph_embeddings, const uint8_t* news_graph,
                      const uint8_t* news_graph_mask, const float* user_news_embedding,
                      const uint8_t* user_graph, const uint8_t* user_category_mask,
                      const int64_t* user_category_indices, const float* news_graph_context,
                      float* out_news_context, float* out_user_context,
                      int B, int N, int H,
                      void* workspace, size_t workspace_bytes, void* stream);

enum { DIGAT_PARAMS_SIDE_STREAM_OFF = 512, DIGAT_PARAMS_SIDE_STREAM_ON = 1024, DIGAT_PARAMS_NO_LIVE_ROWS = 2048 };
enum { DIGAT_PARAMS_PROJ_F16F8C = 4096 };

size_t digat_encoder_grouped_workspace_bytes(int B, int N, int H, int C, int d, int depth);
int digat_encoder_fwd_grouped(const digat_params* params,
                              const float* news_graph_embeddings, const uint8_t* news_graph,
                              const uint8_t* news_graph_mask, const float* user_news_embedding_groups,
                              const uint8_t* user_graph_groups, const uint8_t* user_category_mask_groups,
                              const int64_t* user_category_indices_groups, const int32_t* row_group,
                              const float* news_graph_context, float* out_news_context, float* out_user_context,
                              int B, int G, int N, int H, void* workspace, size_t workspace_bytes, void* stream);

int digat_news_project0(const digat_params* params, const float* Xn, float* hpq, int M, int N, void* stream);
int digat_user_project0(const digat_params* params, const float* X, float* hpq, int M, void* stream);
int digat_news_context_queries(const digat_params* params, const float* c_n, float* out, int M, void* stream);
int digat_encoder_fwd_grouped_cached(const digat_params* params,
                                     const float* news_graph_embeddings, const uint8_t* news_graph, const uint8_t* news_graph_mask,
                                     const float* user_news_embedding_g, const uint8_t* user_graph_g,
                                     const uint8_t* user_category_mask_g, const int64_t* user_category_indices_g,
                                     const int32_t* row_group, const float* news_graph_context, const float* news_hpq0,
                                     const float* hist_hpq0, const float* topic_hpq0, const float* ctxq0,
                                     const int64_t* news_index, int64_t news_rows,
                                     float* out_news, float* out_user, int B, int G, int N, int H,
                                     void* workspace, size_t workspace_bytes, void* stream);

int digat_row_logits(const float* news_ctx, const float* user_ctx, float* logits, int B, int d, void* stream);

int digat_linear_bwd_input(const float* dy, int64_t lddy, const float* w, float* dx, int64_t lddx,
                           int M, int N, int K, int accumulate, void* stream);
int digat_linear_bwd_input_x3(const float* dy, int64_t lddy, const float* w, float* dx, int64_t lddx,
                              int M, int N, int K, int accumulate, void* wsplit, void* stream);
size_t digat_linear_bwd_weight_workspace(int M, int No, int Ni);
int digat_linear_bwd_weight(const float* dy, int64_t lddy, const float* x, int64_t ldx, float* dW, float* db,
                            int M, int No, int Ni, int accumulate, void* workspace, size_t workspace_bytes,
                            void* stream);
int digat_colsum(const float* x, int64_t ldx, float* out, int M, int N, int accumulate, void* stream);
int digat_dropout_fwd(const float* x, float* y, uint8_t* mask, int64_t n, float p, uint32_t seed, void* stream);
int digat_dropout_bwd(const float* dy, const uint8_t* mask, float* dx, int64_t n, float p, void* stream);
int digat_gate_fwd(const float* z, const float* l, int64_t ldl, const float* g, float* out, int B, int d, void* stream);
int digat_gate_bwd(const float* dout, const float* z, const float* l, int64_t ldl, const float* g,
                   float* dz, float* dl, float* dg, int B, int d, void* stream);
int digat_relu_res_fwd(const float* y, const float* t, float* out, int64_t n, void* stream);
int digat_relu_mask(const float* dout, const float* y, float* dy, int64_t n, void* stream);
int digat_attn_pool_fwd(const float* feat, int64_t ld_b, const float* kq, const uint8_t* mask, float* out,
                        float* alpha_out, int B, int n, int d, void* stream);
int digat_attn_pool_bwd(const float* feat, int64_t ld_b, const float* kq, const uint8_t* mask, const float* alpha,
                        const float* dout, float* dfeat, int64_t ldd_b, float* dkq, int B, int n, int d,
                        int accumulate_dfeat, void* stream);
int digat_topic_pool_fwd_train(const float* Xu, const float* kq, const int64_t* cat_idx, float* out, float* alpha_out,
                               int B, int U, int H, int C1, int d, void* stream);
int digat_topic_pool_bwd(const float* Xu, const float* kq, const int64_t* cat_idx, const float* alpha, const float* dT,
                         float* dXu, float* dkq, int B, int U, int H, int C1, int d, void* stream);
int digat_xattn_project(const float* X, const float* r, const float* W, const float* bW, const float* F1,
                        const float* F2, float* h, float* Pr, float* Q, int B, int n, int d, void* stream);
int digat_xattn_project_x3(const float* X, const float* r, const float* W, const float* bW, const float* F1, const float* F2,
                           float* h, float* Pr, float* Q, int B, int n, int d, void* wsplit, void* stream);
int digat_xattn_pairwise_fwd_train(const float* Pr, const float* Q, const float* h, const float* X, const float* a,
                                   const uint8_t* A, float* out, float* alpha, float* s_pre, float* alpha_drop,
                                   uint8_t* amask, float p, uint32_t seed, int B, int n, int d, void* stream);
size_t digat_xattn_pairwise_bwd_workspace(int B, int n, int d);
int digat_xattn_pairwise_bwd(const float* dOut, const float* out, const float* Xres, const float* Pr, const float* Q,
                             const float* h, const float* a, const uint8_t* A, const float* alpha, const float* s_pre,
                             const uint8_t* amask, float p, float* dPr, float* dQ, float* dh, float* da,
                             int accumulate_da, int B, int n, int d, void* workspace, size_t workspace_bytes,
                             void* stream);
int digat_sum_nodes(const float* dP, float* dr, int B, int n, int d, void* stream);

int digat_set_train_precision(int bf16);

enum { DIGAT_GEMM_BF16X6 = 0, DIGAT_GEMM_F16X3 = 1 };
enum { DIGAT_GEMM_F16F8C = 2 };
size_t digat_split_weights_bytes_format(int rows, int K, int format);

int digat_row_logits_bwd(const float* dlogits, const float* news_ctx, const float* user_ctx, float* dnews, float* duser, int B, int d,
                         void* stream);
int digat_click_loss(const float* logits, int B, int K, float* loss, float* dlogits, void* stream);

typedef struct digat_opt_tensor { float* p; const float* g; float* m; float* v; int64_t n; float weight_decay; int32_t pad; } digat_opt_tensor;
int digat_opt_chunk(void);
int digat_clip_adam_step(const void* tensors, const int32_t* chunk_tensor, const int64_t* chunk_off, int nchunks, float* scratch, float max_norm,
                         float lr, float beta1, float beta2, float eps, int step, void* stream);

typedef struct digat_split_job {
    const float *w0, *w1, *w2;
    int32_t rows, cols, layout, reserved;
    void* image;
} digat_split_job;
size_t digat_split_job_bytes(int rows, int cols, int layout, int matrices);
int digat_split_jobs(const digat_split_job* jobs, int njobs, void* stream);

size_t digat_xattn_train_save_bytes(int B, int n, int d);
size_t digat_xattn_train_workspace_bytes(int B, int n, int d);
enum { DIGAT_TRAIN_XATTN_AUTO = 0, DIGAT_TRAIN_XATTN_SPARSE = 1, DIGAT_TRAIN_XATTN_DENSE = 2 };
int digat_xattn_fwd_train(const float* X, const uint8_t* A, const float* ctx, const float* W, const float* bW, const float* F1,
                          const float* F2, const float* F3, const float* b3, const float* a, float* out, float p_alpha,
                          uint32_t seed, float p_in, uint32_t seed_in, int B, int n, int d, void* save, size_t save_bytes, void* workspace,
                          size_t workspace_bytes, const void* proj_image, int xattn_mode, void* stream);
int digat_xattn_bwd(const float* dOut, const float* out, const float* X, const uint8_t* A, const float* ctx, const float* W,
                    const float* F1, const float* F2, const float* F3, const float* a, float p_alpha, float p_in, const void* save,
                    size_t save_bytes, float* dX, float* dctx, float* dW, float* dbW, float* dF1, float* dF2, float* dF3,
                    float* db3, float* da, int B, int n, int d, void* workspace, size_t workspace_bytes, const void* bwd_image,
                    int xattn_mode, void* stream);
size_t digat_news_ctx_train_save_bytes(int B, int N, int d);
size_t digat_news_ctx_train_workspace_bytes(int B, int N, int d);
int digat_news_ctx_fwd_train(const float* X, const uint8_t* mask, const float* Kc, const float* Qc, const float* bQc,
                             const float* Wg, const float* bg, float* out, float p_gate, uint32_t seed, int B, int N, int d,
                             void* save, size_t save_bytes, void* workspace, size_t workspace_bytes,
                             const float* prev , void* stream);
int digat_news_ctx_bwd(const float* dout, const float* X, const uint8_t* mask, const float* Kc, const float* Qc, const float* Wg,
                       float p_gate, const void* save, size_t save_bytes, float* dX, float* dKc, float* dQc, float* dbQc,
                       float* dWg, float* dbg, int B, int N, int d, int accumulate_params, void* workspace, size_t workspace_bytes,
                       void* stream);
size_t digat_user_ctx_train_save_bytes(int B, int U, int H, int C1, int d);
size_t digat_user_ctx_train_workspace_bytes(int B, int U, int H, int C1, int d);
int digat_user_ctx_fwd_train(const float* Xu, const uint8_t* cat_mask, const int64_t* cat_idx, const float* c_n, const float* Ku,
                             const float* Qu, const float* bQu, const float* Fa, const float* bFa, const float* Kua,
                             const float* Qua, const float* bQua, float* out, float p_topic, uint32_t seed, int B, int U, int H,
                             int C1, int d, void* save, size_t save_bytes, void* workspace, size_t workspace_bytes,
                             const void* fa_image ,
                             const float* prev , void* stream);
int digat_user_ctx_bwd(const float* dout, const float* Xu, const uint8_t* cat_mask, const int64_t* cat_idx, const float* c_n,
                       const float* Ku, const float* Qu, const float* Fa, const float* Kua, const float* Qua, float p_topic,
                       const void* save, size_t save_bytes, float* dXu, float* dc_n, float* dKu, float* dQu, float* dbQu,
                       float* dFa, float* dbFa, float* dKua, float* dQua, float* dbQua, int B, int U, int H, int C1, int d,
                       int accumulate_params ,
                       void* workspace, size_t workspace_bytes, const void* fa_bwd_image , void* stream);

int digat_rank_metrics(const float* scores, const uint8_t* labels, const int64_t* impression_start, int num_impressions,
                       int32_t* ranks, double* per_impression, double* mean4, void* stream);

int64_t digat_format_rank_file(const int64_t* ranks, const int64_t* starts, int64_t impressions, char* out, int64_t cap);

size_t digat_gat_workspace_bytes(int B, int n, int d);
int digat_gat_fwd(const float* X, const uint8_t* A, const float* W, const float* bW, const float* a1, const float* a2,
                  float* out, int B, int n, int d, void* workspace, size_t workspace_bytes, void* stream);
size_t digat_gat_train_save_bytes(int B, int n, int d);
size_t digat_gat_train_workspace_bytes(int B, int n, int d);
int digat_gat_fwd_train(const float* X, const uint8_t* A, const float* W, const float* bW, const float* a1, const float* a2, float* out,
                        float p_alpha, uint32_t seed, int B, int n, int d, void* save, size_t save_bytes, void* workspace,
                        size_t workspace_bytes, void* stream);
int digat_gat_bwd(const float* dOut, const float* out, const float* X, const uint8_t* A, const float* W, const float* a1, const float* a2,
                  float p_alpha, const void* save, size_t save_bytes, float* dX, float* dW, float* dbW, float* da1, float* da2,
                  int B, int n, int d, void* workspace, size_t workspace_bytes, void* stream);

size_t digat_sag_cos_topk_workspace_bytes(int64_t n, int64_t m, int dim);
int digat_sag_cos_topk(const float* title, const float* content, int64_t n, const float* corpus_title, const float* corpus_content,
                       int64_t m, int dim, int k, float* values, int32_t* indices, void* workspace, size_t workspace_bytes,
                       void* stream);
int digat_sag_news_graph(const int32_t* sim_index, const float* sim_cos, const int32_t* sim_len, int64_t news_num, int top_M, int hop,
                         int news_node_num, float threshold, int32_t* news_node_ID, uint8_t* news_graph, uint8_t* news_graph_mask,
                         int32_t* overflow, void* stream);

typedef struct digat_msa_params {
    int32_t word_embedding_dim, head_num, head_dim, attention_dim;
    const float *word_embedding;
// ... 93 lines not shown
```

Before: 38410 impressions/s.

## Pre-split topic-pool output to fp16x3 and run live-row scan before context tail

Adds an optional path where the topic-pool kernel writes its output already split into fp16 hi/lo pieces, so the featureAffine GEMM can load the pieces directly instead of splitting A in its inner loop (a new presplit strip kernel). This path is off by default. It also moves the live-row scan ahead of the first user-context tail, so that tail's GEMM can use the compacted row list and skip dead rows. The row list is adopted only when it keeps the same kernel choice. The tradeoff is extra write traffic from the split output, plus an earlier scan on the critical path.

```diff
diff --git a/digat_amd/_lib.py b/digat_amd/_lib.py
--- a/digat_amd/_lib.py
+++ b/digat_amd/_lib.py
@@ -18,6 +18,8 @@
 PARAMS_SIDE_STREAM_OFF, PARAMS_SIDE_STREAM_ON = 512, 1024
 PARAMS_NO_LIVE_ROWS = 2048
 PARAMS_PROJ_F16F8C = 4096
+PARAMS_CTX_TAIL_PLAIN = 8192
+PARAMS_CTX_PRESPLIT = 16384
 
 _f = C.c_void_p
 
diff --git a/digat_amd/csrc/digat_context.inc b/digat_amd/csrc/digat_context.inc
--- a/digat_amd/csrc/digat_context.inc
+++ b/digat_amd/csrc/digat_context.inc
@@ -160,6 +160,8 @@
     const int* group;
     const uint8_t* live; int live_ld;
     const int* hlast;
+    unsigned* out_split;
+    unsigned* range_flag;
 };
 constexpr int TOPIC_MAX_H = 256;
 constexpr int TOPIC_MAX_CT = 4;
@@ -272,7 +274,7 @@
 }
 
 
-template <int TOPIC_RES_STEPS>
+template <int TOPIC_RES_STEPS, bool SPLIT = false>
 __global__ void __launch_bounds__(TOPIC_RES_STEPS > 13 ? 512 : 1024) topic_pool_resident_kernel(const TopicArgs g) {
     extern __shared__ __attribute__((aligned(16))) unsigned char smem[];
     const int H = g.H, hs = H | 1;
@@ -359,6 +361,18 @@
     const int ct_eff = __builtin_amdgcn_readfirstlane((scat[64] + 15) >> 4);
     const int nslots_all = scat[64];
     float* Ob = g.out + (long)b * g.C1 * g.d;
+    float amax = 0.f;
+    auto store_row = [&](int c, const float4 v) {
+        *reinterpret_cast<float4*>(Ob + (long)c * g.d + ch) = v;
+        if constexpr (SPLIT) {
+            unsigned h0, l0, h1, l1;
+            split_f16x3(v.x, v.y, h0, l0, amax);
+            split_f16x3(v.z, v.w, h1, l1, amax);
+            unsigned* const sp = g.out_split + ((long)b * g.C1 + c) * g.d + (ch & ~7) + ((ch >> 2) & 1) * 2;
+            *reinterpret_cast<uint2*>(sp) = make_uint2(h0, h1);
+            *reinterpret_cast<uint2*>(sp + 4) = make_uint2(l0, l1);
+        }
+    };
     for (int it = 0; it < ct_eff; ++it) {
         v4f acc[4];
 #pragma unroll
@@ -378,13 +392,17 @@
 #pragma unroll
         for (int r = 0; r < 4; ++r) {
             const int sl = it * 16 + 4 * lq + r;
-            if (sl < nslots_all && ch_ok)
-                *reinterpret_cast<float4*>(Ob + (long)scat[sl] * g.d + ch) = make_float4(acc[0][r], acc[1][r], acc[2][r], acc[3][r]);
+            if (sl < nslots_all && ch_ok) store_row(scat[sl], make_float4(acc[0][r], acc[1][r], acc[2][r], acc[3][r]));
         }
     }
     for (int c = lq; c < g.C1; c += 4)
-        if (cslot[c] < 0 && ch_ok) *reinterpret_cast<float4*>(Ob + (long)c * g.d + ch) = f4_zero();
-}
+        if (cslot[c] < 0 && ch_ok) store_row(c, f4_zero());
+    if constexpr (SPLIT) {
+        if (g.range_flag && __builtin_amdgcn_ballot_w64(!(amax < 65504.f)) != 0 && lane == 0) atomicOr(g.range_flag, 1u);
+    }
+}
+
+static bool topic_writes_split(int H, int d) { return H <= 52 && d % 8 == 0 && (d + 63) / 64 <= 16; }
 
 static int launch_topic_args(TopicArgs g, hipStream_t st) {
     const int groups = (g.d + 63) / 64;
@@ -399,9 +417,11 @@
             raised = 1;
         }
     }
+    if (g.out_split && !topic_writes_split(g.H, g.d)) return DIGAT_ERR_ARG;
     if (g.H <= 64 && (g.H <= 52 || groups <= 8)) {
         const size_t ldsr = ((size_t)ct * 16 * (g.H | 1) + (size_t)groups * 64 + 192 + 64 + 68) * 4;
-        if (g.H <= 52) hipLaunchKernelGGL(topic_pool_resident_kernel<13>, dim3(g.B), dim3(64 * groups), ldsr, st, g);
+        if (g.out_split) hipLaunchKernelGGL((topic_pool_resident_kernel<13, true>), dim3(g.B), dim3(64 * groups), ldsr, st, g);
+        else if (g.H <= 52) hipLaunchKernelGGL(topic_pool_resident_kernel<13>, dim3(g.B), dim3(64 * groups), ldsr, st, g);
         else hipLaunchKernelGGL(topic_pool_resident_kernel<16>, dim3(g.B), dim3(64 * groups), ldsr, st, g);
     } else {
         hipLaunchKernelGGL(topic_pool_kernel, dim3(g.B), dim3(64 * groups), lds, st, g);
@@ -412,9 +432,10 @@
 
 static int launch_topic(const float* Xu, long ld_b, const float* kq, const int64_t* idx, float* out,
                         int B, int H, int C1, int d, hipStream_t st, const int* group = nullptr,
-                        const uint8_t* live = nullptr, int live_ld = 0, const int* hlast = nullptr) {
+                        const uint8_t* live = nullptr, int live_ld = 0, const int* hlast = nullptr,
+                        unsigned* out_split = nullptr, unsigned* range_flag = nullptr) {
     if (B == 0) return DIGAT_OK;
-    TopicArgs g{Xu, ld_b, kq, idx, out, B, H, C1, d, sqrtf((float)d), nullptr, group, live, live_ld, hlast};
-    ProfScope prof(DIGAT_KERNEL_TOPIC, (double)B * ((double)H * d * 4 + d * 4.0 + H * 8.0 + (double)C1 * d * 4), st);
+    TopicArgs g{Xu, ld_b, kq, idx, out, B, H, C1, d, sqrtf((float)d), nullptr, group, live, live_ld, hlast, out_split, range_flag};
+    ProfScope prof(DIGAT_KERNEL_TOPIC, (double)B * ((double)H * d * 4 + d * 4.0 + H * 8.0 + (double)C1 * d * (out_split ? 8 : 4)), st);
     return launch_topic_args(g, st);
 }
diff --git a/digat_amd/csrc/digat_gemm.inc b/digat_amd/csrc/digat_gemm.inc
--- a/digat_amd/csrc/digat_gemm.inc
+++ b/digat_amd/csrc/digat_gemm.inc
@@ -219,6 +219,15 @@
     const fp16x2 h = __builtin_bit_cast(fp16x2, bits);
     return (float)h[0];
 }
+__device__ __forceinline__ void split_f16x3(float x0, float x1, unsigned& hi, unsigned& lo, float& amax) {
+    constexpr float xs = F16_ACT_SCALE;
+    const float v0 = x0 * xs, v1 = x1 * xs;
+    amax = fmaxf(fmaxf(amax, fabsf(v0)), fabsf(v1));
+    hi = pack_half_rtz(v0, v1);
+    const fp16x2 h = __builtin_bit_cast(fp16x2, hi);
+    const _Float16 l0 = (_Float16)__builtin_fmaf(x0, xs, -(float)h[0]), l1 = (_Float16)__builtin_fmaf(x1, xs, -(float)h[1]);
+    lo = (unsigned)__builtin_bit_cast(unsigned short, l0) | ((unsigned)__builtin_bit_cast(unsigned short, l1) << 16);
+}
 struct Split3 { unsigned short a, b, c; };
 __device__ __forceinline__ Split3 split3(float v) {
     const Split3f f = split3f(v);
@@ -340,9 +349,10 @@
 #else
 #define GT_NOW() 0ull
 #endif
-template <int NSUB, bool F16, int MT, bool FULL>
-__global__ void __launch_bounds__(256, MT == 1 ? 3 : 2) gemm_bf16x6s_kernel(const GemmArgs g) {
+template <int NSUB, bool F16, int MT, bool FULL, bool PRE>
+__device__ __forceinline__ void gemm_strip_body(const GemmArgs& g) {
     static_assert(MT == 1 || MT == 2, "wave tiles of 16 or 32 rows");
+    static_assert(!PRE || (F16 && NSUB == 1 && !FULL), "pre-split A rows are fp16x3 pieces, read by the one-strip tiles");
     constexpr int NT = 5;
     constexpr int WROWS = 16 * MT, TROWS = 4 * WROWS;
     constexpr int APW = 2 * MT;
@@ -392,7 +402,7 @@
         }
     };
     const long arow0 = g.rowidx ? 0 : (long)(m0 < Mv ? m0 : Mv - 1);
-    const char* const abase = reinterpret_cast<const char*>(g.a0 + arow0 * g.lda0);
+    const char* const abase = reinterpret_cast<const char*>((PRE ? static_cast<const float*>(g.a_split) : g.a0) + arow0 * g.lda0);
     unsigned aoff[APW];
     int ac4[APW];
 #pragma unroll
@@ -425,22 +435,18 @@
     auto split_mt = [&](int mt, int abuf, bf16x8 (&dst)[3][MT]) {
         const int r = wm * WROWS + mt * 16 + lr;
         const int sw = (r >> 1) & 7;
+        if constexpr (PRE) {
+            dst[0][mt] = __builtin_bit_cast(bf16x8, As[abuf][r * 8 + ((kg * 2) ^ sw)]);
+            dst[1][mt] = __builtin_bit_cast(bf16x8, As[abuf][r * 8 + ((kg * 2 + 1) ^ sw)]);
+            return;
+        }
         const float4 v0 = __builtin_bit_cast(float4, As[abuf][r * 8 + ((kg * 2) ^ sw)]);
         const float4 v1 = __builtin_bit_cast(float4, As[abuf][r * 8 + ((kg * 2 + 1) ^ sw)]);
         if constexpr (F16) {
-            constexpr float xs = F16_ACT_SCALE;
             const float raw[8] = {v0.x, v0.y, v0.z, v0.w, v1.x, v1.y, v1.z, v1.w};
-            const float v[8] = {v0.x * xs, v0.y * xs, v0.z * xs, v0.w * xs, v1.x * xs, v1.y * xs, v1.z * xs, v1.w * xs};
-            amax = fmaxf(fmaxf(amax, fabsf(v[0])), fabsf(v[1])); amax = fmaxf(fmaxf(amax, fabsf(v[2])), fabsf(v[3]));
-            amax = fmaxf(fmaxf(amax, fabsf(v[4])), fabsf(v[5])); amax = fmaxf(fmaxf(amax, fabsf(v[6])), fabsf(v[7]));
             unsigned hi[4], lo[4];
 #pragma unroll
-            for (int e = 0; e < 4; ++e) {
-                hi[e] = pack_half_rtz(v[2 * e], v[2 * e + 1]);
-                const fp16x2 h = __builtin_bit_cast(fp16x2, hi[e]);
-                const _Float16 l0 = (_Float16)__builtin_fmaf(raw[2 * e], xs, -(float)h[0]), l1 = (_Float16)__builtin_fmaf(raw[2 * e + 1], xs, -(float)h[1]);
-                lo[e] = (unsigned)__builtin_bit_cast(unsigned short, l0) | ((unsigned)__builtin_bit_cast(unsigned short, l1) << 16);
-            }
+            for (int e = 0; e < 4; ++e) split_f16x3(raw[2 * e], raw[2 * e + 1], hi[e], lo[e], amax);
             dst[0][mt] = __builtin_bit_cast(bf16x8, make_uint4(hi[0], hi[1], hi[2], hi[3]));
             dst[1][mt] = __builtin_bit_cast(bf16x8, make_uint4(lo[0], lo[1], lo[2], lo[3]));
         } else {
@@ -582,7 +588,7 @@
     const unsigned long long gt_loop_end = GT_NOW();
     gt_body += gt_loop_end - gt_last;
 #endif
-    if constexpr (F16) {
+    if constexpr (F16 && !PRE) {
         if (g.range_flag && __builtin_amdgcn_ballot_w64(!(amax < 65504.f)) != 0 && lane == 0) atomicOr(g.range_flag, 1u);
     }
     int gmv[MT];
@@ -704,6 +710,15 @@
         atomicAdd(&g_gemm_timers[6], 1ull); atomicAdd(&g_gemm_timers[7], gt_end - gt_enter);
     }
 #endif
+}
+
+template <int NSUB, bool F16, int MT, bool FULL>
+__global__ void __launch_bounds__(256, MT == 1 ? 3 : 2) gemm_bf16x6s_kernel(const GemmArgs g) {
+    gemm_strip_body<NSUB, F16, MT, FULL, false>(g);
+}
+template <int MT>
+__global__ void __launch_bounds__(256, MT == 1 ? 3 : 2) gemm_f16x3s_presplit_kernel(const GemmArgs g) {
+    gemm_strip_body<1, true, MT, false, true>(g);
 }
 
 template <int MT, bool KTAIL, bool TW = false>
@@ -1326,7 +1341,7 @@
     g.mtiles = p.mtiles; g.ntiles = p.ntiles;
     switch (p.kernel) {
 #define DIGAT_GEMM_LAUNCH(id, ...) case GEMM_##id: hipLaunchKernelGGL((__VA_ARGS__), dim3(p.grid), dim3(p.block), 0, st, g); break;
-        DIGAT_GEMM_KERNELS(DIGAT_GEMM_LAUNCH)
+        DIGAT_GEMM_ALL_KERNELS(DIGAT_GEMM_LAUNCH)
 #undef DIGAT_GEMM_LAUNCH
         default: return DIGAT_ERR_ARG;
     }
diff --git a/digat_amd/csrc/digat_gemm_plan.h b/digat_amd/csrc/digat_gemm_plan.h
--- a/digat_amd/csrc/digat_gemm_plan.h
+++ b/digat_amd/csrc/digat_gemm_plan.h
@@ -27,6 +27,7 @@
     unsigned* range_flag;
     const uint8_t* dmask; long lddm; float dscale;
     int dmask_cols;
+    const void* a_split;
 };
 
 #define DIGAT_GEMM_KERNELS(X)                                        \
@@ -55,18 +56,22 @@
     X(F32_128, gemm_f32_kernel<128, 80, 4, 1, 1, 0>)                 \
     X(F32_64, gemm_f32_kernel<64, 80, 4, 1, 2, 0>)                   \
     X(F32_32, gemm_f32_kernel<32, 64, 1, 4, 2, 0>)
+#define DIGAT_GEMM_PRESPLIT_KERNELS(X)                               \
+    X(PRE_1_F16_64, gemm_f16x3s_presplit_kernel<1>)                  \
+    X(PRE_1_F16, gemm_f16x3s_presplit_kernel<2>)
+#define DIGAT_GEMM_ALL_KERNELS(X) DIGAT_GEMM_KERNELS(X) DIGAT_GEMM_PRESPLIT_KERNELS(X)
 
 enum GemmKernel {
     GEMM_NONE,
     GEMM_PER_SEGMENT,
 #define DIGAT_GEMM_ENUM(id, ...) GEMM_##id,
-    DIGAT_GEMM_KERNELS(DIGAT_GEMM_ENUM)
+    DIGAT_GEMM_ALL_KERNELS(DIGAT_GEMM_ENUM)
 #undef DIGAT_GEMM_ENUM
 };
 
 static inline const char* gemm_kernel_name(int kernel) {
 #define DIGAT_GEMM_NAME(id, ...) if (kernel == GEMM_##id) return #__VA_ARGS__;
-    DIGAT_GEMM_KERNELS(DIGAT_GEMM_NAME)
+    DIGAT_GEMM_ALL_KERNELS(DIGAT_GEMM_NAME)
 #undef DIGAT_GEMM_NAME
     return kernel == GEMM_PER_SEGMENT ? "per segment" : "none";
 }
@@ -80,7 +85,8 @@
 };
 
 static inline bool gemm_kernel_takes_row_list(int kernel) {
-    return kernel == GEMM_F16F8C_3 || kernel == GEMM_F16F8C_1 || (kernel >= GEMM_STRIP_3_F16_64 && kernel <= GEMM_STRIP_1_BF16);
+    return kernel == GEMM_F16F8C_3 || kernel == GEMM_F16F8C_1 || (kernel >= GEMM_STRIP_3_F16_64 && kernel <= GEMM_STRIP_1_BF16) ||
+           kernel == GEMM_PRE_1_F16_64 || kernel == GEMM_PRE_1_F16;
 }
 
 static inline GemmPlan gemm_plan(const GemmArgs& g, int kind = DIGAT_KERNEL_LINEAR) {
@@ -94,6 +100,18 @@
         return p;
     };
 
+    if (g.a_split) {
+        GemmArgs plain = g;
+        plain.a_split = nullptr;
+        const GemmPlan q = gemm_plan(plain, kind);
+        const bool ok = q.status == DIGAT_OK && g.format == DIGAT_GEMM_F16X3 && g.K % 8 == 0 && g.lda0 % 8 == 0 &&
+                        ((uintptr_t)g.a_split & 15) == 0 && !g.x1_segs && !g.x3_segs &&
+                        (q.kernel == GEMM_STRIP_1_F16_64 || q.kernel == GEMM_STRIP_1_F16);
+        if (!ok) { p = q; p.status = q.status ? q.status : DIGAT_ERR_ARG; return p; }
+        p = q;
+        p.kernel = q.kernel == GEMM_STRIP_1_F16 ? GEMM_PRE_1_F16 : GEMM_PRE_1_F16_64;
+        return p;
+    }
     if (g.format == DIGAT_GEMM_F16F8C && g.wsplit) {
         const bool ok = g.nseg % 80 == 0 && g.K % 4 == 0 && g.k0 == g.K && !g.a1 && !g.transW && g.lda0 % 4 == 0 &&
                         ((uintptr_t)g.a0 & 15) == 0 && g.ldy % 4 == 0 && g.lde0 % 4 == 0 &&
@@ -155,3 +173,8 @@
 }
 
 static inline bool gemm_takes_row_list(const GemmArgs& g) { return gemm_kernel_takes_row_list(gemm_plan(g).kernel); }
+static inline bool gemm_takes_presplit(GemmArgs g) {
+    if (!g.a_split) g.a_split = g.a0;
+    const GemmPlan p = gemm_plan(g);
+    return p.status == DIGAT_OK && (p.kernel == GEMM_PRE_1_F16_64 || p.kernel == GEMM_PRE_1_F16);
+}
diff --git a/digat_amd/csrc/digat_kernels.hip b/digat_amd/csrc/digat_kernels.hip
--- a/digat_amd/csrc/digat_kernels.hip
+++ b/digat_amd/csrc/digat_kernels.hip
@@ -590,7 +590,7 @@
 
 
 enum { ENC_PLAIN, ENC_GROUPED, ENC_SHARED };
-struct FoldCtxWs { float *T, *T2, *glob; };
+struct FoldCtxWs { float *T, *T2, *glob; unsigned* Ts; };
 struct EncoderWs {
     float *Xu[2], *Xn[2];
     char* xws; size_t xws_bytes;
@@ -622,7 +622,7 @@
     e.xu = xattn_carve(xa, B, U, d);
     Arena ca = a.sub(max_sz(digat_news_ctx_workspace_bytes(B, N, d), digat_user_ctx_workspace_bytes(B, U, H, C1, d)));
     e.cws = ca.base; e.cws_bytes = ca.cap;
-    e.fc = FoldCtxWs{ca.take<float>(b * C1 * d), ca.take<float>(b * C1 * d), ca.take<float>(bd)};
+    e.fc = FoldCtxWs{ca.take<float>(b * C1 * d), ca.take<float>(b * C1 * d), ca.take<float>(bd), nullptr};
     e.kq_t = a.take<float>(bd); e.kq_u = a.take<float>(bd);
     e.r_user[0] = a.take<float>(bd); e.r_news = a.take<float>(bd); e.r_user[1] = a.take<float>(bd);
     Arena na = a.sub(digat_xattn_workspace_bytes(B, N, d));
@@ -638,6 +638,7 @@
     e.tw_cnt = a.take<int>(b + 64); e.tw_off = a.take<int>(b + 64);
     e.gl_off = a.take<int>(b + 64); e.gl_idx = a.take<int>(bu);
     e.idx32 = a.take<int>(b);
+    e.fc.Ts = C1 <= U ? reinterpret_cast<unsigned*>(e.xu.P) : nullptr;
     if (variant == ENC_GROUPED) {
         const size_t g = b / 4 + 1;
         e.Au = a.take<uint8_t>(bu * U); e.cm = a.take<uint8_t>(b * C1); e.ci = a.take<int64_t>(b * H);
@@ -708,6 +709,9 @@
     const int lfmt = (p->flags & DIGAT_PARAMS_PROJ_F16F8C) ? DIGAT_GEMM_F16F8C : fmt;
     const int bd_disp = (p->flags & DIGAT_PARAMS_BD_TILED) ? (1 << 30) : 1;
     float *T = w.fc.T, *T2 = w.fc.T2, *glob = w.fc.glob;
+    const bool tail_plain = (p->flags & DIGAT_PARAMS_CTX_TAIL_PLAIN) != 0;
+    const bool want_presplit = !tail_plain && (p->flags & DIGAT_PARAMS_CTX_PRESPLIT) != 0;
+    bool ts_free = false;
     const int* bucket_idx = nullptr;
     const int* nbuckets_dev = nullptr;
     const int* hist_last = nullptr;
@@ -724,6 +728,7 @@
         g.m_dispatch = bd_disp;
         return launch_gemm(g, sq);
     };
+    bool initial_tail = true;
     auto user_ctx_tail = [&](const float* Xu_cur, const float* addend, hipStream_t sq, const int* xgroup = nullptr,
                              const uint8_t* live = nullptr, const float* kq_topic = nullptr, const float* kq_user = nullptr) -> int {
         if (!kq_topic) { kq_topic = w.kq_t; kq_user = w.kq_u; }
@@ -732,13 +737,21 @@
                                   (const uint4*)p->featureAffine_fsplit, p->featureAffine_b, rflag, B, H, C1, d, sqrtf((float)d)};
             return launch_user_ctx_fused(fa, sq);
         }
-        int e = launch_topic(Xu_cur, (long)U * d, kq_topic, cat_idx, T, B, H, C1, d, sq, xgroup, live, U, live ? hist_last : nullptr);
-        if (e) return e;
         GemmArgs g = gemm_plain(T, d, p->featureAffine_W, p->featureAffine_b, T2, d, B * C1, d, d, 0);
         g.epi = EPI_RELU_RES; g.e0 = T; g.lde0 = d;
         g.wsplit = (const unsigned short*)p->featureAffine_wsplit;
         g.format = fmt; g.range_flag = rflag;
-        if (bucket_idx && gemm_takes_row_list(g)) { g.rowidx = bucket_idx; g.nrows_dev = nbuckets_dev; }
+        const bool presplit = ts_free && fmt == 1 && topic_writes_split(H, d) && gemm_takes_presplit(g);
+        int e = launch_topic(Xu_cur, (long)U * d, kq_topic, cat_idx, T, B, H, C1, d, sq, xgroup, live, U, live ? hist_last : nullptr,
+                             presplit ? w.fc.Ts : nullptr, presplit ? rflag : nullptr);
+        if (e) return e;
+        if (presplit) g.a_split = w.fc.Ts;
+        if (bucket_idx && gemm_takes_row_list(g)) {
+            GemmArgs gl = g;
+            gl.rowidx = bucket_idx; gl.nrows_dev = nbuckets_dev;
+            if (!initial_tail || gemm_plan(gl).kernel == gemm_plan(g).kernel) g = gl;
+        }
+        initial_tail = false;
         e = launch_gemm(g, sq);
         if (e) return e;
         return launch_pool(T2, (long)C1 * d, kq_user, cat_mask, addend, c_u, B, C1, d, sq);
@@ -860,6 +873,7 @@
     };
     const int side_mode = (p->flags & DIGAT_PARAMS_SIDE_STREAM_OFF) ? 0 : ((p->flags & DIGAT_PARAMS_SIDE_STREAM_ON) ? 1 : 2);
     SideStream* side = (side_mode == 0 || (side_mode == 2 && B >= 2048)) ? nullptr : side_stream(st);
+    ts_free = !side && want_presplit && w.fc.Ts != nullptr;
     const bool news_early = L > 0 && N <= 16 && d / 4 <= 256;
     const bool news_lists_on = L > 0 && d / 4 <= 256 && !(p->flags & DIGAT_PARAMS_NO_LIVE_ROWS);
     const bool news_lists = news_lists_on && ((!news_early && (p->flags & DIGAT_NEWS_XATTN_SPARSE) && N > 16) || (news_early && L > 1 && B >= 2048));
@@ -953,6 +967,12 @@
         if (rc) return rc;
     }
     const bool xu0_shared = shared && sparse_mode == DIGAT_XATTN_SPARSE;
+    const bool lists_first = !side && want_live && !tail_plain;
+    if (lists_first) {
+        rc = find_live_rows(st);
+        if (rc) return rc;
+        publish_live_rows();
+    }
     rc = user_ctx_tail(xu0_grouped ? Xg0 : w.Xu[0], nullptr, st, (xu0_grouped || xu0_shared) ? row_group : nullptr, nullptr,
                        ctxq0 ? ctxq0 : nullptr, ctxq0 ? ctxq0 + bd : nullptr);
     if (rc) return rc;
@@ -970,7 +990,7 @@
         if (side && i > 0) {
             if (hipStreamWaitEvent(st, side->join, 0) != hipSuccess) return DIGAT_ERR_LAUNCH;
         }
-        if (i == 0 && want_scan && !live_early) {
+        if (i == 0 && want_scan && !live_early && !lists_first) {
             rc = find_live_rows(st);
             if (rc) return rc;
         }
diff --git a/digat_amd/graphEncoders.py b/digat_amd/graphEncoders.py
--- a/digat_amd/graphEncoders.py
+++ b/digat_amd/graphEncoders.py
@@ -71,6 +71,8 @@
         self.corpus_xattn_hint = {}
         self.side_stream = "auto"
         self.live_rows = True
+        self.ctx_lists_first = True
+        self.ctx_presplit = False
         self.fused_user_context = False
 
     def initialize(self):
@@ -96,7 +98,7 @@
         self.userAttention.initialize()
 
     @contextlib.contextmanager
-    def launch_options(self, side_stream=None, live_rows=None, shared_users=None):
+    def launch_options(self, side_stream=None, live_rows=None, shared_users=None, ctx_lists_first=None, ctx_presplit=None):
         table = _TLS.__dict__.setdefault("opts", {})
         prev = table.get(id(self))
         cur = dict(prev or {})
@@ -106,6 +108,10 @@
             cur["side_stream"] = side_stream
         if live_rows is not None:
             cur["live_rows"] = bool(live_rows)
+        if ctx_lists_first is not None:
+            cur["ctx_lists_first"] = bool(ctx_lists_first)
+        if ctx_presplit is not None:
+            cur["ctx_presplit"] = bool(ctx_presplit)
         if shared_users is not None:
             cur["detect_shared_users"] = bool(shared_users)
         table[id(self)] = cur
@@ -274,7 +280,9 @@
                 | (_lib.PARAMS_PROJ_F16F8C if pm == "fp16-fp8c" else 0)
                 | (_lib.PARAMS_BD_TILED if self.pass_rows >= 2048 else 0)
                 | {"auto": 0, "off": _lib.PARAMS_SIDE_STREAM_OFF, "on": _lib.PARAMS_SIDE_STREAM_ON}[self._launch_option("side_stream")]
-                | (0 if self._launch_option("live_rows") else _lib.PARAMS_NO_LIVE_ROWS))
+                | (0 if self._launch_option("live_rows") else _lib.PARAMS_NO_LIVE_ROWS)
+                | (0 if self._launch_option("ctx_lists_first") else _lib.PARAMS_CTX_TAIL_PLAIN)
+                | (_lib.PARAMS_CTX_PRESPLIT if self._launch_option("ctx_presplit") else 0))
 
     def _fold_sources(self):
         ca, ua = self.candidate_attention, self.userAttention
diff --git a/include/digat_hip.h b/include/digat_hip.h
--- a/include/digat_hip.h
+++ b/include/digat_hip.h
@@ -133,6 +133,7 @@
 
 enum { DIGAT_PARAMS_SIDE_STREAM_OFF = 512, DIGAT_PARAMS_SIDE_STREAM_ON = 1024, DIGAT_PARAMS_NO_LIVE_ROWS = 2048 };
 enum { DIGAT_PARAMS_PROJ_F16F8C = 4096 };
+enum { DIGAT_PARAMS_CTX_TAIL_PLAIN = 8192, DIGAT_PARAMS_CTX_PRESPLIT = 16384 };
 
 size_t digat_encoder_grouped_workspace_bytes(int B, int N, int H, int C, int d, int depth);
 int digat_encoder_fwd_grouped(const digat_params* params,
```

Result: no change. 38340 impressions/s, median of 3 (-0.2%).
